# Kateridge/TransMF_AD

Hardware: AMD Instinct MI355X
Metric: volume-pairs/sec fwd+bwd(+Adam), 96^3 MRI+PET batch=8 per GPU (higher is better)
Workload: dtype f32

## Files before the change

include/tmf_hip.h:

```cpp
#ifndef TMF_HIP_H
#define TMF_HIP_H

#include <stddef.h>
#include <stdint.h>

#ifdef __cplusplus
extern "C" {
#endif

#define TMF_OK              0
#define TMF_E_NULL         -1
#define TMF_E_SHAPE        -2
#define TMF_E_ALIGN        -3
#define TMF_E_WORKSPACE    -4
#define TMF_E_ARG          -5

#define TMF_DW_TAPMAJOR  0
#define TMF_DW_REFERENCE 1

#define TMF_POOL_NONE 0
#define TMF_POOL_MAX2 1
#define TMF_POOL_AVG2 2

int         tmf_version(void);
const char* tmf_last_error_string(void);
int         tmf_set_option(const char* name, int value);

int  tmf_conv3d_fwd(const float* x, const float* w, float* z, float* stat_partial,
                    int B, int D, int H, int W, int cin, int cout, int ksize, void* stream);
int  tmf_conv3d_stat_blocks(int B, int D, int H, int W, int cin, int cout, int ksize);
const char* tmf_conv3d_fwd_kernel_name(int B, int D, int H, int W, int cin, int cout, int ksize);
const char* tmf_conv3d_wgrad_kernel_name(int B, int D, int H, int W, int cin, int cout, int ksize);
int  tmf_conv3d_fwd_affine(const float* x, const float* w, const float* scale, const float* shift, float* y,
                           int B, int D, int H, int W, int cin, int cout, int ksize, int pool, float slope, void* stream);

size_t tmf_conv3d_wgrad_workspace_bytes(int B, int D, int H, int W, int cin, int cout, int ksize);
int    tmf_conv3d_wgrad(const float* x, const float* dz, float* dw, void* workspace, size_t workspace_bytes,
                        int B, int D, int H, int W, int cin, int cout, int ksize, int dw_layout, void* stream);

int  tmf_conv3d_fwd_bf16(const float* x, const void* w_bf16, float* z, float* stat_partial,
                         int B, int D, int H, int W, int cin, int cout, void* stream);
int  tmf_conv3d_bf16_stat_blocks(int B, int D, int H, int W);
size_t tmf_conv3d_wgrad_bf16_workspace_bytes(int B, int D, int H, int W, int cin, int cout);
int    tmf_conv3d_wgrad_bf16(const float* x, const float* dz, float* dw, void* workspace, size_t workspace_bytes,
                             int B, int D, int H, int W, int cin, int cout, void* stream);
int    tmf_conv3d_fwd_bf16_t(const void* x, const void* w_bf16, void* z, float* stat_partial,
                             int B, int D, int H, int W, int cin, int cout, int io, void* stream);
const char* tmf_conv3d_fwd_bf16_kernel_name(int B, int D, int H, int W, int cin, int cout, int io);
const char* tmf_conv3d_wgrad_bf16_kernel_name(int B, int D, int H, int W, int cin, int cout, int io);
int    tmf_conv3d_wgrad_bf16_plan(int B, int D, int H, int W, int cin, int cout, int io, int* nsplit, int* tiles_per_split);
int    tmf_conv3d_wgrad_bf16_t(const void* x, const void* dz, float* dw, void* workspace, size_t workspace_bytes,
                               int B, int D, int H, int W, int cin, int cout, int io, int dw_layout, void* stream);
int  tmf_conv3d_fwd_split(const float* x, const void* w3_bf16, float* z, float* stat_partial,
                          int B, int D, int H, int W, int cin, int cout, void* stream);
int  tmf_conv3d_split_stat_blocks(int B, int D, int H, int W);
int    tmf_conv3d_fwd_wino(const float* x, const float* u, float* z, float* stat_partial,
                           int B, int D, int H, int W, int cin, int cout, void* stream);
int    tmf_conv3d_wino_ok(int cin, int cout);
int    tmf_conv3d_fwd_wino_affine(const float* x, const float* u, const float* scale, const float* shift, float* y,
                                  int B, int D, int H, int W, int cin, int cout, int pool, float slope, void* stream);
int    tmf_conv3d_wino_stat_blocks(int B, int D, int H, int W);
int    tmf_conv3d_wino_bricks(int B, int D, int H, int W);
int    tmf_conv3d_wino_bricks2(int B, int D, int H, int W, int cin, int cout);
int    tmf_conv3d_wino_grid(int B, int D, int H, int W, int cin, int cout);
int    tmf_xcd_slot(int block, int grid);
const char* tmf_conv3d_wino_kernel_name(int B, int D, int H, int W, int stats);
const char* tmf_conv3d_wgrad_wino_kernel_name(int B, int D, int H, int W, int cin, int cout);
long   tmf_conv3d_wgrad_wino_tiles(int B, int D, int H, int W, int cin, int cout);
const char* tmf_conv3d_wino_kernel_name2(int B, int D, int H, int W, int cin, int cout, int stats);
size_t tmf_conv3d_wino_weight_bytes(int cin, int cout);
int    tmf_wino_x_mode(void);
int    tmf_conv_wino_mode(void);
int    tmf_wino_p_mode(void);
int    tmf_conv3d_wgrad_wino_ok(int cin, int cout);
size_t tmf_conv3d_wgrad_wino_workspace_bytes(int B, int D, int H, int W, int cin, int cout);
int    tmf_conv3d_wgrad_wino(const float* x, const float* dz, float* dw, void* workspace, size_t workspace_bytes,
                             int B, int D, int H, int W, int cin, int cout, int dw_layout, void* stream);

int    tmf_conv3d_c1_fwd(const float* x, const float* w, float* z, float* stat_partial,
                         int B, int D, int H, int W, int cout, void* stream);
int    tmf_conv3d_c1_stat_blocks(int B, int D, int H, int W, int cout);
size_t tmf_conv3d_c1_wgrad_workspace_bytes(int B, int D, int H, int W, int cout);
int    tmf_conv3d_c1_wgrad(const float* x, const float* dz, float* dw, void* workspace, size_t workspace_bytes,
                           int B, int D, int H, int W, int cout, int dw_layout, void* stream);

int    tmf_c1_blocks(int B, int D, int H, int W, int C);
int    tmf_c1_stats(const float* x, const float* w, float* stat_partial, int B, int D, int H, int W, int C, void* stream);
size_t tmf_c1_gram_bytes(int B, int D, int H, int W, int C);
size_t tmf_c1_gram_bytes_bf16(int B, int D, int H, int W, int C);
int    tmf_c1_stats_g(const float* x, const float* w, float* stat_partial, void* gram, size_t gram_bytes,
                      int B, int D, int H, int W, int C, void* stream);
size_t tmf_c1_bwd_fused_workspace_bytes(int B, int D, int H, int W, int C);
int    tmf_c1_bwd_fused(const float* x, const float* w, const float* scale, const float* shift, const float* mean,
                        const float* invstd, const float* dpool, const void* gram, float* dw, float* dgamma, float* dbeta,
                        void* workspace, size_t workspace_bytes, int B, int D, int H, int W, int C, float slope,
                        int dw_layout, void* stream);
int    tmf_c1_stats_g_bf16(const float* x, const float* w, float* stat_partial, void* gram, size_t gram_bytes,
                           int B, int D, int H, int W, int C, void* stream);
int    tmf_c1_bwd_fused_bf16(const float* x, const float* w, const float* scale, const float* shift, const float* mean,
                             const float* invstd, const void* dpool, const void* gram, float* dw, float* dgamma, float* dbeta,
                             void* workspace, size_t workspace_bytes, int B, int D, int H, int W, int C, float slope,
                             int pooled_bf16, int dw_layout, void* stream);
int    tmf_c1_bn_pool_fwd(const float* x, const float* w, const float* scale, const float* shift, float* pooled,
                          int B, int D, int H, int W, int C, float slope, void* stream);
int    tmf_c1_bn_pool_fwd_route(const float* x, const float* w, const float* scale, const float* shift, float* pooled,
                                float* z_sel, unsigned char* arg, int B, int D, int H, int W, int C, float slope, void* stream);
int    tmf_c1_bwd_fused_route(const float* x, const float* w, const float* scale, const float* shift, const float* mean,
                              const float* invstd, const float* dpool, const float* z_sel, const unsigned char* arg,
                              const void* gram, float* dw, float* dgamma, float* dbeta, void* workspace, size_t workspace_bytes,
                              int B, int D, int H, int W, int C, float slope, int dw_layout, void* stream);
int    tmf_c1_bwd_fused_coef(const float* x, const float* w, const float* scale, const float* shift, const float* mean,
                             const float* invstd, const float* dpool, const float* z_sel, const unsigned char* arg,
                             const void* gram, float* dw, float* dgamma, float* dbeta, float* coef, void* workspace,
                             size_t workspace_bytes, int B, int D, int H, int W, int C, float slope, int dw_layout, void* stream);
int    tmf_c1_bwd_reduce(const float* x, const float* w, const float* scale, const float* shift,
                         const float* mean, const float* invstd, const float* dpool, float* partial,
                         int B, int D, int H, int W, int C, float slope, void* stream);
size_t tmf_c1_bwd_wgrad_workspace_bytes(int B, int D, int H, int W, int C);
int    tmf_c1_bwd_wgrad(const float* x, const float* w, const float* scale, const float* shift,
                        const float* mean, const float* invstd, const float* coef, const float* dpool,
                        float* dw, void* workspace, size_t workspace_bytes,
                        int B, int D, int H, int W, int C, float slope, int dw_layout, void* stream);
size_t tmf_c1_bwd_dgrad_workspace_bytes(int B, int D, int H, int W, int C);
int    tmf_c1_bwd_dgrad(const float* x, const float* w, const float* scale, const float* shift, const float* mean,
                        const float* invstd, const float* coef, const float* dpool, float* dx,
                        void* workspace, size_t workspace_bytes, int B, int D, int H, int W, int C, float slope, void* stream);
int    tmf_c1_stats_bf16(const float* x, const float* w, float* stat_partial, int B, int D, int H, int W, int C, void* stream);
int    tmf_c1_bn_pool_fwd_bf16(const float* x, const float* w, const float* scale, const float* shift, void* pooled,
                               int B, int D, int H, int W, int C, float slope, int pooled_bf16, void* stream);
int    tmf_c1_bwd_reduce_bf16(const float* x, const float* w, const float* scale, const float* shift,
                              const float* mean, const float* invstd, const void* dpool, float* partial,
                              int B, int D, int H, int W, int C, float slope, int pooled_bf16, void* stream);
int    tmf_c1_bwd_wgrad_bf16(const float* x, const float* w, const float* scale, const float* shift,
                             const float* mean, const float* invstd, const float* coef, const void* dpool,
                             float* dw, void* workspace, size_t workspace_bytes,
                             int B, int D, int H, int W, int C, float slope, int pooled_bf16, int dw_layout, void* stream);


int tmf_bn_finalize(const float* stat_partial, int nblk, int C, double count,
                    const float* gamma, const float* beta, const float* conv_bias,
                    float* running_mean, float* running_var, float momentum, float eps,
                    float* mean, float* invstd, float* scale, float* shift, void* stream);

int tmf_bn_eval_coeffs(const float* gamma, const float* beta, const float* conv_bias,
                       const float* running_mean, const float* running_var, float eps, int C,
                       float* scale, float* shift, void* stream);

int tmf_bn_act_pool_fwd(const float* z, const float* scale, const float* shift, float* out,
                        int B, int D, int H, int W, int C, int pool, float slope, void* stream);

int tmf_bn_act_pool_bwd_blocks(int B, int D, int H, int W, int C, int pool);
int tmf_bn_act_pool_bwd_reduce(const float* z, const float* dout, const float* scale, const float* shift,
                               const float* mean, const float* invstd, float* partial,
                               int B, int D, int H, int W, int C, int pool, float slope, void* stream);
int tmf_bn_bwd_finalize(const float* partial, int nblk, int C, double count,
                        float* dgamma, float* dbeta, float* coef, void* stream);
int tmf_bn_act_pool_bwd_apply(const float* z, const float* dout, const float* scale, const float* shift,
                              const float* mean, const float* invstd, const float* coef, float* dz,
                              int B, int D, int H, int W, int C, int pool, float slope, void* stream);

int tmf_bn_act_pool_fwd_t(const void* z, const float* scale, const float* shift, void* out,
                          int B, int D, int H, int W, int C, int pool, float slope, int io, void* stream);
int tmf_bn_act_pool_bwd_reduce_t(const void* z, const void* dout, const float* scale, const float* shift,
                                 const float* mean, const float* invstd, float* partial,
                                 int B, int D, int H, int W, int C, int pool, float slope, int io, void* stream);
int tmf_bn_act_pool_bwd_apply_t(const void* z, const void* dout, const float* scale, const float* shift,
                                const float* mean, const float* invstd, const float* coef, void* dz,
                                int B, int D, int H, int W, int C, int pool, float slope, int io, void* stream);

int tmf_bn_act_pool_fwd_route(const float* z, const float* scale, const float* shift, float* out, float* z_sel,
                              int B, int D, int H, int W, int C, float slope, void* stream);
int tmf_bn_act_pool_bwd_reduce_route(const float* z_sel, const float* dout, const float* scale, const float* shift,
                                     const float* mean, const float* invstd, float* partial,
                                     int B, int D, int H, int W, int C, float slope, void* stream);

int tmf_colsum_finalize(const float* partial, int nblk, int ncol, float* out, void* stream);

int tmf_xattn_fwd(const float* q, const float* k, const float* v, float* out, float* lse,
                  int B, int heads, int N, int M, int dh, int q_stride, int kv_stride, float scale,
                  void* stream);
int tmf_xattn_bwd(const float* q, const float* k, const float* v, const float* out, const float* lse,
                  const float* dout, float* dq, float* dk, float* dv,
                  int B, int heads, int N, int M, int dh, int q_stride, int kv_stride, int dkv_stride,
                  float scale, void* stream);
int tmf_xattn_fwd_cat(const float* q, const float* k1, const float* v1, const float* k2, const float* v2, float* out,
                      float* lse, int B, int heads, int N, int M1, int M2, int dh, int q_stride, int kv_stride, float scale,
                      void* stream);
int tmf_xattn_bwd_cat(const float* q, const float* k1, const float* v1, const float* k2, const float* v2, const float* out,
                      const float* lse, const float* dout, float* dq, float* dk1, float* dv1, float* dk2, float* dv2,
                      int B, int heads, int N, int M1, int M2, int dh, int q_stride, int kv_stride, int dkv_stride,
                      float scale, void* stream);
int tmf_xattn_probs(const float* q, const float* k1, const float* k2, const float* lse,
                    float* probs, float* recv, int B, int heads, int N, int M1, int M2, int dh,
                    int q_stride, int kv_stride, float scale, void* stream);

int tmf_layernorm_fwd(const float* x, const float* gamma, const float* beta, const float* residual, float* y,
                      float* mean, float* rstd, int rows, int dim, float eps, void* stream);
int tmf_layernorm_bwd_blocks(int rows, int dim);
int tmf_layernorm_bwd(const float* x, const float* gamma, const float* mean, const float* rstd,
                      const float* dy, float* dx, float* partial, int rows, int dim, void* stream);
int tmf_layernorm_bwd_masked(const float* x, const float* gamma, const float* mean, const float* rstd,
                             const float* dy, float* dx, float* partial, int rows, int dim,
                             const float* mask, float* dx_masked, void* stream);
int tmf_mask_mul(const float* x, const float* mask, float* y, long n, void* stream);

int tmf_tok_row_blocks(int R);
int tmf_tok_linear_fwd(const float* x, const float* w, const float* bias, const float* residual, float* y,
                       int R, int K, int Nout, const float* ln_gamma, const float* ln_beta, float eps,
                       float* ln_mean, float* ln_rstd, float* ln_out, float* gelu_pre, void* stream);
int tmf_tok_linear_bwd_input(const float* dy, const float* w, float* dx, int R, int Nout, int K,
                             const float* gelu_pre, const float* ln_x, const float* ln_mean, const float* ln_rstd,
                             const float* ln_gamma, const float* add1, const float* add2, float* ln_partial,
                             float* bias_partial, int partial_stride, void* stream);
int tmf_tok_linear_fwd_masked(const float* x, const float* w, const float* bias, const float* residual, float* y,
                              int R, int K, int Nout, const float* ln_gamma, const float* ln_beta, float eps,
                              float* ln_mean, float* ln_rstd, float* ln_out, float* gelu_pre, const float* mask, void* stream);
int tmf_tok_linear_bwd_input_masked(const float* dy, const float* w, float* dx, int R, int Nout, int K,
                                    const float* gelu_pre, const float* ln_x, const float* ln_mean, const float* ln_rstd,
                                    const float* ln_gamma, const float* add1, const float* add2, float* ln_partial,
                                    float* bias_partial, int partial_stride, const float* mask, float* dx_masked,
                                    void* stream);

int tmf_pack_conv_weights(const float* w, float* w_fwd, float* w_dgrad, int cout, int cin, int taps, void* stream);
int tmf_pack_conv_weights_bf16(const float* w, void* w_fwd_bf16, void* w_dgrad_bf16, int cout, int cin, int taps, void* stream);
int tmf_pack_conv_weights_split3(const float* w, void* w3_fwd, void* w3_dgrad, int cout, int cin, int taps, void* stream);
int tmf_pack_conv_weights_wino(const float* w, float* u_fwd, float* u_dgrad, int cout, int cin, void* stream);
int tmf_pack_conv_weights_wino_multi(int n, const float* const* w, float* const* u_fwd, float* const* u_dgrad,
                                     const int* cout, const int* cin, void* stream);

int tmf_layout_ncdhw_to_ndhwc(const float* src, float* dst, int B, int C, long voxels, void* stream);
int tmf_layout_ndhwc_to_ncdhw(const float* src, float* dst, int B, int C, long voxels, void* stream);

size_t tmf_tok_wgrad_multi_workspace_bytes(int nprob, const int* N, const int* K);
int    tmf_tok_wgrad_multi(int nprob, const float* const* dy, const float* const* x, float* const* dw,
                           const int* R, const int* N, const int* K, void* workspace, size_t workspace_bytes, void* stream);

int tmf_token_pool_fwd(const float* mri, const float* pet, float* cls, int32_t* argmax,
                       int B, int N, int dim, void* stream);
int tmf_token_pool_bwd(const float* dcls, const int32_t* argmax, float* dmri, float* dpet,
                       int B, int N, int dim, void* stream);

size_t tmf_scale_intensity_workspace_bytes(int B);
int    tmf_rotate_x(const float* src, float* dst, const float* cos_sin, const unsigned char* do_rot,
                    int B, int D, int H, int W, void* stream);
int    tmf_zoom_area(const float* src, float* dst, const int* out_size, const unsigned char* do_zoom,
                     int B, int D, int H, int W, void* stream);
int    tmf_volume_minmax(const float* vol, float* minmax, void* workspace, size_t workspace_bytes, int B, long voxels,
                         void* stream);
int    tmf_scale_flip(const float* src, float* dst, const float* minmax, const unsigned char* flip_d,
                      int B, int D, int H, int W, void* stream);

typedef struct tmf_augment_decision {
    int32_t index;
    int32_t flip;
    int32_t do_rot;
    float   cos_a, sin_a;
    int32_t od, oh, ow;
} tmf_augment_decision;
int    tmf_batch_augment(const float* store_mri, const float* store_pet, const int64_t* labels,
                         const tmf_augment_decision* decisions, float* out_mri, float* out_pet, int64_t* out_label,
                         int N, int B, int D, int H, int W, void* stream);

#define TMF_SNET_BLOCKS 7
#define TMF_PREC_FP32 0
#define TMF_PREC_BF16 1
#define TMF_PREC_FP32X 2
#define TMF_SNET_ALONE 1
#define TMF_SNET_ALGO          0x100
#define TMF_SNET_ALGO_WINO(m)  (((m) & 3) << 9)
#define TMF_SNET_ALGO_WINO_P   0x800
#define TMF_SNET_ALGO_WINO_X   0x1000
#define TMF_SNET_ALGO_C1_GRAM  0x2000
#define TMF_SNET_ALGO_C1_GRAM_BF16 0x4000
#define TMF_SNET_ALGO_C1_SPLIT 0x8000
#define TMF_SNET_ALGO_POOL_REC_C1 0x10000
#define TMF_SNET_ALGO_POOL_REC_BN 0x20000
int  tmf_snet_algo_flags(void);
int  tmf_c1_split_mode(void);
#define TMF_CONV_DIRECT 0
#define TMF_CONV_WINO   1
#define TMF_CONV_BF16   2
#define TMF_CONV_SPLIT  3
int  tmf_conv_block_algo(int precision, int cin, int cout, int ksize);
typedef struct tmf_snet_desc {
    int   B, D, H, W;
    int   dim;
    int   precision;
    int   storage_bf16;
    float momentum[TMF_SNET_BLOCKS];
    float eps[TMF_SNET_BLOCKS];
    float slope[TMF_SNET_BLOCKS];
    int   flags;
} tmf_snet_desc;
typedef struct tmf_snet_params {
    const float* weight[TMF_SNET_BLOCKS];
    const float* bias[TMF_SNET_BLOCKS];
    const float* gamma[TMF_SNET_BLOCKS];
    const float* beta[TMF_SNET_BLOCKS];
    float*       running_mean[TMF_SNET_BLOCKS];
    float*       running_var[TMF_SNET_BLOCKS];
} tmf_snet_params;
#define TMF_SNET_DEEP_FROM 3
typedef struct tmf_snet_grads {
    float* dweight[TMF_SNET_BLOCKS];
    float* dbias[TMF_SNET_BLOCKS];
    float* dgamma[TMF_SNET_BLOCKS];
    float* dbeta[TMF_SNET_BLOCKS];
    void*  deep_event;
} tmf_snet_grads;
size_t tmf_snet_saved_bytes(const tmf_snet_desc* d);
size_t tmf_snet_bwd_scratch_bytes(const tmf_snet_desc* d);
int    tmf_snet_train_fwd(const tmf_snet_desc* d, const float* vol, const tmf_snet_params* params,
                          void* saved, size_t saved_bytes, float* out, void* stream);
int    tmf_snet_train_bwd(const tmf_snet_desc* d, const float* vol, const void* saved, size_t saved_bytes,
                          const float* dout, const tmf_snet_grads* grads, void* scratch, size_t scratch_bytes, void* stream);
int    tmf_snet_train_bwd_input(const tmf_snet_desc* d, const float* vol, const void* saved, size_t saved_bytes,
                                const float* dout, const tmf_snet_grads* grads, void* scratch, size_t scratch_bytes, void* stream,
                                float* dvol);
size_t tmf_snet_eval_workspace_bytes(const tmf_snet_desc* d);
int    tmf_snet_eval_fwd(const tmf_snet_desc* d, const float* vol, const tmf_snet_params* params,
                         void* workspace, size_t workspace_bytes, float* out, void* stream);

#define TMF_FUSION_MAX_DEPTH 16
#define TMF_FUSION_PER_OP 1
typedef struct tmf_fusion_desc { int B, N, dim, heads, dim_head, mlp, depth, flags; } tmf_fusion_desc;
typedef struct tmf_xformer_params {
    const float *ln1_g, *ln1_b;
    const float *wq, *wkv, *wo, *bo;
    const float *ln2_g, *ln2_b;
    const float *w1, *b1, *w2, *b2;
    const float *lnf_g, *lnf_b;
    float eps1, eps2, epsf;
    const float *mask_o, *mask_g, *mask_f;
} tmf_xformer_params;
typedef struct tmf_xformer_grads {
    float *small, *lnf, *dwq, *dwkv, *dwo, *dw1, *dw2;
} tmf_xformer_grads;
void   tmf_debug_xf_trace(void* fwd, void* bwd_q, void* bwd_kv);
size_t tmf_fusion_saved_bytes(const tmf_fusion_desc* d);
int    tmf_fusion_uses_fused(const tmf_fusion_desc* d);
int    tmf_fusion_takes_masks(const tmf_fusion_desc* d);
size_t tmf_fusion_bwd_scratch_bytes(const tmf_fusion_desc* d);
int    tmf_fusion_train_fwd(const tmf_fusion_desc* d, const float* mri_tok, const float* pet_tok,
                            const tmf_xformer_params* inst, void* saved, size_t saved_bytes, float* cls, void* stream);
int    tmf_fusion_train_bwd(const tmf_fusion_desc* d, const float* mri_tok, const float* pet_tok,
                            const tmf_xformer_params* inst, const void* saved, size_t saved_bytes, const float* dcls,
                            const tmf_xformer_grads* grads, float* dmri_tok, float* dpet_tok,
                            void* scratch, size_t scratch_bytes, void* stream);
size_t tmf_fusion_infer_workspace_bytes(const tmf_fusion_desc* d);
int    tmf_fusion_infer_fwd(const tmf_fusion_desc* d, const float* mri_tok, const float* pet_tok,
                            const tmf_xformer_params* inst, void* workspace, size_t workspace_bytes,
                            float* cls, void* stream);
size_t tmf_fusion_attn_maps_workspace_bytes(const tmf_fusion_desc* d);
int    tmf_fusion_attn_maps(const tmf_fusion_desc* d, const float* mri_tok, const float* pet_tok,
                            const tmf_xformer_params* inst, void* workspace, size_t workspace_bytes,
                            float* cls, float* probs, float* recv, void* stream);

typedef struct tmf_heads_desc { int B, N, dim, H1, H2, HD, NC, training; float momentum[3], eps[3]; } tmf_heads_desc;
typedef struct tmf_heads_params {
    const float *fc0_w, *fc0_b, *bn1_g, *bn1_b, *fc4_w, *fc4_b, *bn5_g, *bn5_b, *fc8_w, *fc8_b;
    const float *d0_w, *d0_b, *dbn_g, *dbn_b, *d3_w, *d3_b;
    float *bn1_rm, *bn1_rv, *bn5_rm, *bn5_rv, *dbn_rm, *dbn_rv;
} tmf_heads_params;
typedef struct tmf_heads_grads {
    float *fc0_w, *fc0_b, *bn1_g, *bn1_b, *fc4_w, *fc4_b, *bn5_g, *bn5_b, *fc8_w, *fc8_b, *d0_w, *d0_b, *dbn_g, *dbn_b, *d3_w, *d3_b;
} tmf_heads_grads;
size_t tmf_heads_saved_bytes(const tmf_heads_desc* d);
size_t tmf_heads_bwd_scratch_bytes(const tmf_heads_desc* d);
int    tmf_heads_fwd(const tmf_heads_desc* d, const float* cls, const float* mri_tok, const float* pet_tok,
                     const float* mask1, const float* mask2, const tmf_heads_params* params, float* logits,
                     float* d_mri_logits, float* d_pet_logits, void* saved, size_t saved_bytes, void* stream);
int    tmf_heads_bwd(const tmf_heads_desc* d, const float* cls, const float* mask1, const float* mask2,
                     const tmf_heads_params* params, const void* saved, size_t saved_bytes, const float* d_logits,
                     const float* d_d_mri_logits, const float* d_d_pet_logits, const tmf_heads_grads* grads,
                     float* d_cls, float* d_mri_tok, float* d_pet_tok, float revgrad_alpha,
                     void* scratch, size_t scratch_bytes, void* stream);

#define TMF_MASK_SEGMENTS 20
int    tmf_dropout_keep_masks(int nseg, float* const* out, const long* numel, const float* keep,
                              unsigned long long seed, unsigned long long offset, void* stream);

typedef struct tmf_heads_cnn_desc { int B, N, dim, M, H, HD, NC, training; float momentum, eps; } tmf_heads_cnn_desc;
typedef struct tmf_heads_cnn_params {
    const float *fc0_w, *fc0_b, *fc2_w, *fc2_b;
    const float *d0_w, *d0_b, *dbn_g, *dbn_b;
    float *dbn_rm, *dbn_rv;
    const float *d3_w, *d3_b;
} tmf_heads_cnn_params;
typedef struct tmf_heads_cnn_grads { float *fc0_w, *fc0_b, *fc2_w, *fc2_b, *d0_w, *d0_b, *dbn_g, *dbn_b, *d3_w, *d3_b; } tmf_heads_cnn_grads;
size_t tmf_heads_cnn_saved_bytes(const tmf_heads_cnn_desc* d);
size_t tmf_heads_cnn_bwd_scratch_bytes(const tmf_heads_cnn_desc* d);
int    tmf_heads_cnn_fwd(const tmf_heads_cnn_desc* d, const float* mri_tok, const float* pet_tok,
                         const tmf_heads_cnn_params* params, float* logits, float* d_mri_logits, float* d_pet_logits,
                         void* saved, size_t saved_bytes, void* stream);
// ... 94 lines not shown
```

transmf_ad_amd/csrc/conv1_fused.hip:

```cpp
#include <type_traits>
#include "conv1_z.h"

namespace {
using namespace c1z;

enum { MODE_STATS = 0, MODE_FWD = 1, MODE_REDUCE = 2, MODE_WGRAD = 3, MODE_RD = 4 };
#ifndef TMF_C1X_LAZY
#define TMF_C1X_LAZY 0x12
#endif

struct Args {
    const float* x;
    const float* w;
    const float* scale;
    const float* shift;
    const float* mean;
    const float* invstd;
    const float* coef;
    const void* dpool;
    void* pooled;
    float* zsel;
    unsigned char* parg;
    float* partial;
    float* partial2;
// ... 400 lines not shown
}
extern "C" int tmf_c1_stats(const float* x, const float* w, float* stat_partial,
                            int B, int D, int H, int W, int C, void* stream) {
    return c1_stats(false, x, w, stat_partial, B, D, H, W, C, stream);
}
extern "C" int tmf_c1_stats_bf16(const float* x, const float* w, float* stat_partial,
                                 int B, int D, int H, int W, int C, void* stream) {
    return c1_stats(true, x, w, stat_partial, B, D, H, W, C, stream);
}

static int c1_bn_pool_fwd(bool bf16, bool p16, const float* x, const float* w, const float* scale, const float* shift,
                          void* pooled, int B, int D, int H, int W, int C, float slope, void* stream,
                          float* z_sel = nullptr, unsigned char* arg = nullptr) {
    TMF_REQUIRE_PTR(x); TMF_REQUIRE_PTR(w); TMF_REQUIRE_PTR(scale); TMF_REQUIRE_PTR(shift); TMF_REQUIRE_PTR(pooled);
    int rc = check("tmf_c1_bn_pool_fwd", B, D, H, W, C);
    if (rc) return rc;
    const Plan p = make_plan(B, D, H, W, C, tmf_opt(TMF_OPT_C1_FWD_MULT) * SLAB_BLOCKS);
    Args a = base_args(x, w, D, H, W, C, p, slope);
    a.scale = scale; a.shift = shift; a.pooled = pooled; a.zsel = z_sel; a.parg = arg;
    TMF_REQUIRE(bf16 || !p16, TMF_E_ARG, "tmf_c1_bn_pool_fwd: bf16 tensors only with the bf16 kernels");
    if (z_sel != nullptr) {
        if (c1_split_mode()) hipLaunchKernelGGL((conv1_fused_kernel<MODE_FWD, false, false, true, true>), dim3(p.nblk, p.nby), dim3(256), 0, (hipStream_t)stream, a);
        else                 hipLaunchKernelGGL((conv1_fused_kernel<MODE_FWD, false, false, false, true>), dim3(p.nblk, p.nby), dim3(256), 0, (hipStream_t)stream, a);
        return tmf_launch_result("tmf_c1_bn_pool_fwd_route");
    }
    if (bf16 && p16) hipLaunchKernelGGL((conv1_fused_kernel<MODE_FWD, true, true>), dim3(p.nblk, p.nby), dim3(256), 0, (hipStream_t)stream, a);
    else if (bf16)   hipLaunchKernelGGL((conv1_fused_kernel<MODE_FWD, true>), dim3(p.nblk, p.nby), dim3(256), 0, (hipStream_t)stream, a);
    else if (c1_split_mode()) hipLaunchKernelGGL((conv1_fused_kernel<MODE_FWD, false, false, true>), dim3(p.nblk, p.nby), dim3(256), 0, (hipStream_t)stream, a);
    else             hipLaunchKernelGGL((conv1_fused_kernel<MODE_FWD, false>), dim3(p.nblk, p.nby), dim3(256), 0, (hipStream_t)stream, a);
    return tmf_launch_result("tmf_c1_bn_pool_fwd");
}
extern "C" int tmf_c1_bn_pool_fwd(const float* x, const float* w, const float* scale, const float* shift,
                                  float* pooled, int B, int D, int H, int W, int C, float slope, void* stream) {
    return c1_bn_pool_fwd(false, false, x, w, scale, shift, pooled, B, D, H, W, C, slope, stream);
}
extern "C" int tmf_c1_bn_pool_fwd_route(const float* x, const float* w, const float* scale, const float* shift, float* pooled,
                                        float* z_sel, unsigned char* arg, int B, int D, int H, int W, int C, float slope, void* stream) {
    TMF_REQUIRE_PTR(z_sel); TMF_REQUIRE_PTR(arg);
    return c1_bn_pool_fwd(false, false, x, w, scale, shift, pooled, B, D, H, W, C, slope, stream, z_sel, arg);
}
extern "C" int tmf_c1_bn_pool_fwd_bf16(const float* x, const float* w, const float* scale, const float* shift,
                                       void* pooled, int B, int D, int H, int W, int C, float slope, int pooled_bf16,
                                       void* stream) {
    return c1_bn_pool_fwd(true, pooled_bf16 != 0, x, w, scale, shift, pooled, B, D, H, W, C, slope, stream);
}

static int c1_bwd_reduce(bool bf16, bool p16, const float* x, const float* w, const float* scale, const float* shift,
                         const float* mean, const float* invstd, const void* dpool, float* partial,
                         int B, int D, int H, int W, int C, float slope, void* stream) {
    TMF_REQUIRE_PTR(x); TMF_REQUIRE_PTR(w); TMF_REQUIRE_PTR(scale); TMF_REQUIRE_PTR(shift);
    TMF_REQUIRE_PTR(mean); TMF_REQUIRE_PTR(invstd); TMF_REQUIRE_PTR(dpool); TMF_REQUIRE_PTR(partial);
    int rc = check("tmf_c1_bwd_reduce", B, D, H, W, C);
    if (rc) return rc;
    const Plan p = make_plan(B, D, H, W, C, SLAB_BLOCKS);
    Args a = base_args(x, w, D, H, W, C, p, slope);
    a.scale = scale; a.shift = shift; a.mean = mean; a.invstd = invstd; a.dpool = dpool; a.partial = partial;
    TMF_REQUIRE(bf16 || !p16, TMF_E_ARG, "tmf_c1_bwd_reduce: bf16 tensors only with the bf16 kernels");
    if (bf16 && p16) hipLaunchKernelGGL((conv1_fused_kernel<MODE_REDUCE, true, true>), dim3(p.nblk, p.nby), dim3(256), 0, (hipStream_t)stream, a);
    else if (bf16)   hipLaunchKernelGGL((conv1_fused_kernel<MODE_REDUCE, true>), dim3(p.nblk, p.nby), dim3(256), 0, (hipStream_t)stream, a);
    else if (c1_split_mode()) hipLaunchKernelGGL((conv1_fused_kernel<MODE_REDUCE, false, false, true>), dim3(p.nblk, p.nby), dim3(256), 0, (hipStream_t)stream, a);
    else             hipLaunchKernelGGL((conv1_fused_kernel<MODE_REDUCE, false>), dim3(p.nblk, p.nby), dim3(256), 0, (hipStream_t)stream, a);
    return tmf_launch_result("tmf_c1_bwd_reduce");
}
extern "C" int tmf_c1_bwd_reduce(const float* x, const float* w, const float* scale, const float* shift,
                                 const float* mean, const float* invstd, const float* dpool, float* partial,
                                 int B, int D, int H, int W, int C, float slope, void* stream) {
    return c1_bwd_reduce(false, false, x, w, scale, shift, mean, invstd, dpool, partial, B, D, H, W, C, slope, stream);
}
extern "C" int tmf_c1_bwd_reduce_bf16(const float* x, const float* w, const float* scale, const float* shift,
                                      const float* mean, const float* invstd, const void* dpool, float* partial,
                                      int B, int D, int H, int W, int C, float slope, int pooled_bf16, void* stream) {
    return c1_bwd_reduce(true, pooled_bf16 != 0, x, w, scale, shift, mean, invstd, dpool, partial, B, D, H, W, C, slope, stream);
}

extern "C" size_t tmf_c1_bwd_wgrad_workspace_bytes(int B, int D, int H, int W, int C) {
    if (B <= 0 || D <= 0 || H <= 0 || W <= 0 || C <= 0) return 0;
    const Plan p = make_plan(B, D, H, W, C, SLAB_BLOCKS);
    return (size_t)(p.nblk + tmf_reduce_groups(p.nblk)) * 27 * C * 4;
}

static int c1_bwd_wgrad(bool bf16, bool p16, const float* x, const float* w, const float* scale, const float* shift,
                        const float* mean, const float* invstd, const float* coef, const void* dpool,
                        float* dw, void* workspace, size_t workspace_bytes,
                        int B, int D, int H, int W, int C, float slope, int dw_layout, void* stream) {
    TMF_REQUIRE(dw_layout == TMF_DW_TAPMAJOR || dw_layout == TMF_DW_REFERENCE, TMF_E_ARG,
                "tmf_c1_bwd_wgrad: unknown dw_layout %d", dw_layout);
    TMF_REQUIRE_PTR(x); TMF_REQUIRE_PTR(w); TMF_REQUIRE_PTR(scale); TMF_REQUIRE_PTR(shift); TMF_REQUIRE_PTR(mean);
    TMF_REQUIRE_PTR(invstd); TMF_REQUIRE_PTR(coef); TMF_REQUIRE_PTR(dpool); TMF_REQUIRE_PTR(dw); TMF_REQUIRE_PTR(workspace);
    int rc = check("tmf_c1_bwd_wgrad", B, D, H, W, C);
    if (rc) return rc;
    const size_t need = tmf_c1_bwd_wgrad_workspace_bytes(B, D, H, W, C);
    TMF_REQUIRE(workspace_bytes >= need, TMF_E_WORKSPACE, "tmf_c1_bwd_wgrad: workspace %zu B < required %zu B",
                workspace_bytes, need);
    const Plan p = make_plan(B, D, H, W, C, SLAB_BLOCKS);
    Args a = base_args(x, w, D, H, W, C, p, slope);
    a.scale = scale; a.shift = shift; a.mean = mean; a.invstd = invstd; a.coef = coef; a.dpool = dpool;
    a.partial = (float*)workspace;
    hipStream_t s = (hipStream_t)stream;
    TMF_REQUIRE(bf16 || !p16, TMF_E_ARG, "tmf_c1_bwd_wgrad: bf16 tensors only with the bf16 kernels");
    if (bf16 && p16) hipLaunchKernelGGL((conv1_fused_kernel<MODE_WGRAD, true, true>), dim3(p.nblk, p.nby), dim3(256), 0, s, a);
    else if (bf16)   hipLaunchKernelGGL((conv1_fused_kernel<MODE_WGRAD, true>), dim3(p.nblk, p.nby), dim3(256), 0, s, a);
    else if (c1_split_mode()) hipLaunchKernelGGL((conv1_fused_kernel<MODE_WGRAD, false, false, true>), dim3(p.nblk, p.nby), dim3(256), 0, s, a);
    else             hipLaunchKernelGGL((conv1_fused_kernel<MODE_WGRAD, false>), dim3(p.nblk, p.nby), dim3(256), 0, s, a);
    if ((rc = tmf_launch_result("tmf_c1_bwd_wgrad"))) return rc;
    const long n = 27L * C;
    return tmf_reduce_slabs((const float*)workspace, p.nblk, n, (float*)workspace + (size_t)p.nblk * n, dw, s,
                            "tmf_c1_bwd_wgrad(reduce)", dw_layout == TMF_DW_REFERENCE ? 1 : 0, C);
}

extern "C" int tmf_c1_bwd_wgrad(const float* x, const float* w, const float* scale, const float* shift,
                                const float* mean, const float* invstd, const float* coef, const float* dpool,
                                float* dw, void* workspace, size_t workspace_bytes,
                                int B, int D, int H, int W, int C, float slope, int dw_layout, void* stream) {
    return c1_bwd_wgrad(false, false, x, w, scale, shift, mean, invstd, coef, dpool, dw, workspace, workspace_bytes, B, D, H, W,
                        C, slope, dw_layout, stream);
}
extern "C" int tmf_c1_bwd_wgrad_bf16(const float* x, const float* w, const float* scale, const float* shift,
                                     const float* mean, const float* invstd, const float* coef, const void* dpool,
                                     float* dw, void* workspace, size_t workspace_bytes,
                                     int B, int D, int H, int W, int C, float slope, int pooled_bf16, int dw_layout,
                                     void* stream) {
    return c1_bwd_wgrad(true, pooled_bf16 != 0, x, w, scale, shift, mean, invstd, coef, dpool, dw, workspace, workspace_bytes,
                        B, D, H, W, C, slope, dw_layout, stream);
}

int tmf_c1_bwd_fused_finish(const float* part, int nblk, const float* dred, const float* w, const void* gram, const float* scale,
                            const float* mean, const float* invstd, double count, float* dgamma, float* dbeta, float* dw, int C,
                            int dw_ref, int round16, void* stream, float* coef);
extern "C" size_t tmf_c1_bwd_fused_workspace_bytes(int B, int D, int H, int W, int C) {
    if (B <= 0 || D <= 0 || H <= 0 || W <= 0 || C <= 0) return 0;
    const Plan p = make_plan(B, D, H, W, C, SLAB_BLOCKS);
    return ((size_t)p.nblk * 2 * C + (size_t)(p.nblk + tmf_reduce_groups(p.nblk) + 1) * 27 * C) * 4;
}
static int c1_bwd_fused(bool bf16, bool p16, const float* x, const float* w, const float* scale, const float* shift, const float* mean,
                        const float* invstd, const void* dpool, const void* gram, float* dw, float* dgamma, float* dbeta,
                        void* workspace, size_t workspace_bytes, int B, int D, int H, int W, int C, float slope,
                        int dw_layout, void* stream, const float* z_sel = nullptr, const unsigned char* arg = nullptr,
                        float* coef = nullptr) {
    TMF_REQUIRE(dw_layout == TMF_DW_TAPMAJOR || dw_layout == TMF_DW_REFERENCE, TMF_E_ARG, "tmf_c1_bwd_fused: unknown dw_layout %d", dw_layout);
    TMF_REQUIRE_PTR(x); TMF_REQUIRE_PTR(w); TMF_REQUIRE_PTR(scale); TMF_REQUIRE_PTR(shift); TMF_REQUIRE_PTR(mean); TMF_REQUIRE_PTR(invstd);
    TMF_REQUIRE_PTR(dpool); TMF_REQUIRE_PTR(gram); TMF_REQUIRE_PTR(dw); TMF_REQUIRE_PTR(workspace);
    int rc = check("tmf_c1_bwd_fused", B, D, H, W, C);
    if (rc) return rc;
    TMF_REQUIRE(C <= 64, TMF_E_SHAPE, "tmf_c1_bwd_fused: C = %d > 64", C);
    const size_t need = tmf_c1_bwd_fused_workspace_bytes(B, D, H, W, C);
    TMF_REQUIRE(workspace_bytes >= need, TMF_E_WORKSPACE, "tmf_c1_bwd_fused: workspace %zu B < required %zu B", workspace_bytes, need);
    const Plan p = make_plan(B, D, H, W, C, SLAB_BLOCKS);
    Args a = base_args(x, w, D, H, W, C, p, slope);
    a.scale = scale; a.shift = shift; a.mean = mean; a.invstd = invstd; a.dpool = dpool;
    float* part = (float*)workspace;
    float* slabs = part + (size_t)p.nblk * 2 * C;
    const long n = 27L * C;
    float* scratch = slabs + (size_t)p.nblk * n;
    float* dred = scratch + (size_t)tmf_reduce_groups(p.nblk) * n;
    a.partial = part; a.partial2 = slabs;
    a.zsel = const_cast<float*>(z_sel); a.parg = const_cast<unsigned char*>(arg);
    hipStream_t s = (hipStream_t)stream;
    TMF_REQUIRE(bf16 || !p16, TMF_E_ARG, "tmf_c1_bwd_fused: bf16 tensors only with the bf16 kernels");
    if (z_sel != nullptr) hipLaunchKernelGGL((conv1_fused_kernel<MODE_RD, false, false, false, true>), dim3(p.nblk, p.nby), dim3(256), 0, s, a);
    else if (bf16 && p16) hipLaunchKernelGGL((conv1_fused_kernel<MODE_RD, true, true>), dim3(p.nblk, p.nby), dim3(256), 0, s, a);
    else if (bf16)   hipLaunchKernelGGL((conv1_fused_kernel<MODE_RD, true>), dim3(p.nblk, p.nby), dim3(256), 0, s, a);
    else if (c1_split_mode()) hipLaunchKernelGGL((conv1_fused_kernel<MODE_RD, false, false, true>), dim3(p.nblk, p.nby), dim3(256), 0, s, a);
    else             hipLaunchKernelGGL((conv1_fused_kernel<MODE_RD, false>), dim3(p.nblk, p.nby), dim3(256), 0, s, a);
    if ((rc = tmf_launch_result("tmf_c1_bwd_fused"))) return rc;
    if ((rc = tmf_reduce_slabs(slabs, p.nblk, n, scratch, dred, s, "tmf_c1_bwd_fused(reduce)"))) return rc;
    return tmf_c1_bwd_fused_finish(part, p.nblk, dred, w, gram, scale, mean, invstd, (double)B * D * H * W, dgamma, dbeta, dw, C,
                                   dw_layout == TMF_DW_REFERENCE ? 1 : 0, bf16 ? 1 : 0, stream, coef);
}
extern "C" int tmf_c1_bwd_fused(const float* x, const float* w, const float* scale, const float* shift, const float* mean,
                                const float* invstd, const float* dpool, const void* gram, float* dw, float* dgamma, float* dbeta,
                                void* workspace, size_t workspace_bytes, int B, int D, int H, int W, int C, float slope,
                                int dw_layout, void* stream) {
    return c1_bwd_fused(false, false, x, w, scale, shift, mean, invstd, dpool, gram, dw, dgamma, dbeta, workspace, workspace_bytes,
                        B, D, H, W, C, slope, dw_layout, stream);
}
extern "C" int tmf_c1_bwd_fused_route(const float* x, const float* w, const float* scale, const float* shift, const float* mean,
                                      const float* invstd, const float* dpool, const float* z_sel, const unsigned char* arg,
                                      const void* gram, float* dw, float* dgamma, float* dbeta, void* workspace, size_t workspace_bytes,
                                      int B, int D, int H, int W, int C, float slope, int dw_layout, void* stream) {
    TMF_REQUIRE_PTR(z_sel); TMF_REQUIRE_PTR(arg);
    return c1_bwd_fused(false, false, x, w, scale, shift, mean, invstd, dpool, gram, dw, dgamma, dbeta, workspace, workspace_bytes,
                        B, D, H, W, C, slope, dw_layout, stream, z_sel, arg);
}
extern "C" int tmf_c1_bwd_fused_coef(const float* x, const float* w, const float* scale, const float* shift, const float* mean,
                                     const float* invstd, const float* dpool, const float* z_sel, const unsigned char* arg,
                                     const void* gram, float* dw, float* dgamma, float* dbeta, float* coef, void* workspace,
                                     size_t workspace_bytes, int B, int D, int H, int W, int C, float slope, int dw_layout, void* stream) {
    TMF_REQUIRE_PTR(coef);
    TMF_REQUIRE((z_sel == nullptr) == (arg == nullptr), TMF_E_NULL, "tmf_c1_bwd_fused_coef: z_sel and arg go together");
    return c1_bwd_fused(false, false, x, w, scale, shift, mean, invstd, dpool, gram, dw, dgamma, dbeta, workspace, workspace_bytes,
// ... 10 lines not shown
```

transmf_ad_amd/csrc/conv3d_mfma.hip:

```cpp
#include <type_traits>
#include "tmf_device.h"

#ifndef TMF_CONV_ACC
#define TMF_CONV_ACC 1
#endif
#ifndef TMF_CONV_BUF
#define TMF_CONV_BUF 1
#endif

namespace {

template <int KS_, int CINC_, int MT_, int NT_, int WM_, int WN_, int TD_, int TH_, int TW_, int TPS_>
struct FwdCfg {
    static constexpr int KS = KS_, CINC = CINC_, MT = MT_, NT = NT_, WM = WM_, WN = WN_;
    static constexpr int TD = TD_, TH = TH_, TW = TW_, TPS = TPS_;
    static constexpr int PAD = KS / 2;
    static constexpr int HD = TD + 2 * PAD, HH = TH + 2 * PAD, HW = TW + 2 * PAD;
    static constexpr int NHALO = HD * HH * HW;
    static constexpr int CP = CINC + 4;
    static constexpr int NPOS = TD * TH * TW;
    static constexpr int NB = 32 * NT * WN;
    static constexpr int NTAPS = KS * KS * KS;
    static constexpr int NSTAGES = NTAPS / TPS;
    static constexpr int BSTAGE = TPS * CINC * NB;
// ... 1402 lines not shown
}

extern "C" const char* tmf_conv3d_fwd_kernel_name(int B, int D, int H, int W, int cin, int cout, int ksize) {
    if (B <= 0 || D <= 0 || H <= 0 || W <= 0 || cin <= 0 || cout <= 0 || (ksize != 1 && ksize != 3)) return "?";
    const FwdPlan p = plan_fwd(B, D, H, W, cin, cout, ksize);
    return ksize == 3 ? fwd_kernel_name<3>(p) : fwd_kernel_name<1>(p);
}

extern "C" const char* tmf_conv3d_wgrad_kernel_name(int B, int D, int H, int W, int cin, int cout, int ksize) {
    if (B <= 0 || D <= 0 || H <= 0 || W <= 0 || cin <= 0 || cout <= 0) return "?";
    if (ksize != 3) return "conv1x1_wgrad_kernel";
    const WgPlan p = plan_wgrad(B, D, H, W, cin, cout);
    const bool vec = (cin % 4 == 0) && (cout % 4 == 0);
    const bool w8 = vec && conv_waves() >= 8;
    static thread_local char buf[64];
    const int edge = p.small ? 4 : 8;
    const int nt = (w8 && p.pack) ? 1 : p.nt;
    snprintf(buf, sizeof buf, "WgCfg<%d, 4, %d, %d, %d, %d>", nt, edge, edge, w8 ? 8 : 4, (w8 && p.pack) ? 16 : 32);
    return buf;
}

extern "C" int tmf_conv3d_stat_blocks(int B, int D, int H, int W, int cin, int cout, int ksize) {
    return tmf_conv3d_stat_blocks_mode(B, D, H, W, cin, cout, ksize, 0);
}
int tmf_conv3d_stat_blocks_mode(int B, int D, int H, int W, int cin, int cout, int ksize, int rt_min) {
    if (B <= 0 || D <= 0 || H <= 0 || W <= 0 || cin <= 0 || cout <= 0) return 0;
    return plan_fwd(B, D, H, W, cin, cout, ksize, true, rt_min).ntiles;
}

extern "C" int tmf_conv3d_fwd(const float* x, const float* w, float* z, float* stat_partial,
                              int B, int D, int H, int W, int cin, int cout, int ksize, void* stream) {
    return tmf_conv3d_fwd_mode(x, w, z, stat_partial, B, D, H, W, cin, cout, ksize, 0, stream);
}
int tmf_conv3d_fwd_mode(const float* x, const float* w, float* z, float* stat_partial,
                        int B, int D, int H, int W, int cin, int cout, int ksize, int rt_min, void* stream) {
    TMF_REQUIRE_PTR(x); TMF_REQUIRE_PTR(w); TMF_REQUIRE_PTR(z);
    TMF_REQUIRE(B > 0 && D > 0 && H > 0 && W > 0 && cin > 0 && cout > 0, TMF_E_SHAPE,
                "tmf_conv3d_fwd: non-positive dimension (B=%d D=%d H=%d W=%d cin=%d cout=%d)", B, D, H, W, cin, cout);
    TMF_REQUIRE(ksize == 1 || ksize == 3, TMF_E_ARG, "tmf_conv3d_fwd: ksize must be 1 or 3, got %d", ksize);
    TMF_REQUIRE((long)D * H * W * (cin > cout ? cin : cout) < (1L << 29), TMF_E_SHAPE,
                "tmf_conv3d_fwd: one sample exceeds 2^29 elements (32-bit byte offsets inside a sample)");
    TMF_REQUIRE((long)ksize * ksize * ksize * cin * cout < (1L << 29), TMF_E_SHAPE, "tmf_conv3d_fwd: weight tensor exceeds 2^29 elements");
    TMF_REQUIRE_ALIGNED(x); TMF_REQUIRE_ALIGNED(w); TMF_REQUIRE_ALIGNED(z);
    const FwdPlan p = plan_fwd(B, D, H, W, cin, cout, ksize, true, rt_min);
    hipStream_t s = (hipStream_t)stream;
    return ksize == 3 ? launch_fwd<3>(p, x, w, z, stat_partial, D, H, W, cin, cout, s)
                      : launch_fwd<1>(p, x, w, z, stat_partial, D, H, W, cin, cout, s);
}

extern "C" int tmf_conv3d_fwd_affine(const float* x, const float* w, const float* scale, const float* shift, float* y,
                                     int B, int D, int H, int W, int cin, int cout, int ksize, int pool, float slope,
                                     void* stream) {
    TMF_REQUIRE_PTR(x); TMF_REQUIRE_PTR(w); TMF_REQUIRE_PTR(scale); TMF_REQUIRE_PTR(shift); TMF_REQUIRE_PTR(y);
    TMF_REQUIRE(B > 0 && D > 0 && H > 0 && W > 0 && cin > 0 && cout > 0, TMF_E_SHAPE,
                "tmf_conv3d_fwd_affine: non-positive dimension (B=%d D=%d H=%d W=%d cin=%d cout=%d)", B, D, H, W, cin, cout);
    TMF_REQUIRE(ksize == 1 || ksize == 3, TMF_E_ARG, "tmf_conv3d_fwd_affine: ksize must be 1 or 3, got %d", ksize);
    TMF_REQUIRE(pool == TMF_POOL_NONE || pool == TMF_POOL_MAX2 || pool == TMF_POOL_AVG2, TMF_E_ARG,
                "tmf_conv3d_fwd_affine: unknown pool mode %d", pool);
    TMF_REQUIRE((long)D * H * W * (cin > cout ? cin : cout) < (1L << 29), TMF_E_SHAPE,
                "tmf_conv3d_fwd_affine: one sample exceeds 2^29 elements (32-bit byte offsets inside a sample)");
    TMF_REQUIRE((long)ksize * ksize * ksize * cin * cout < (1L << 29), TMF_E_SHAPE, "tmf_conv3d_fwd_affine: weight tensor exceeds 2^29 elements");
    TMF_REQUIRE_ALIGNED(x); TMF_REQUIRE_ALIGNED(w); TMF_REQUIRE_ALIGNED(y);
    if (pool != TMF_POOL_NONE && (D / 2 == 0 || H / 2 == 0 || W / 2 == 0)) return TMF_OK;
    const FwdPlan p = plan_fwd(B, D, H, W, cin, cout, ksize, false);
    const Affine aff = {scale, shift, slope, pool};
    hipStream_t s = (hipStream_t)stream;
    return ksize == 3 ? launch_fwd<3>(p, x, w, y, nullptr, D, H, W, cin, cout, s, &aff)
                      : launch_fwd<1>(p, x, w, y, nullptr, D, H, W, cin, cout, s, &aff);
}

extern "C" size_t tmf_conv3d_wgrad_workspace_bytes(int B, int D, int H, int W, int cin, int cout, int ksize) {
    if (B <= 0 || D <= 0 || H <= 0 || W <= 0 || cin <= 0 || cout <= 0) return 0;
    if (ksize == 3) {
        const WgPlan p = plan_wgrad(B, D, H, W, cin, cout);
        return (size_t)(p.nsplit + tmf_reduce_groups(p.nsplit)) * 27 * cin * cout * 4;
    }
    const Wg1Plan p = plan_wgrad1((long)B * D * H * W, cin, cout);
    return (size_t)(p.nsplit + tmf_reduce_groups(p.nsplit)) * cin * cout * 4;
}

extern "C" int tmf_conv3d_wgrad(const float* x, const float* dz, float* dw, void* workspace,
                                size_t workspace_bytes, int B, int D, int H, int W, int cin, int cout,
                                int ksize, int dw_layout, void* stream) {
    TMF_REQUIRE(dw_layout == TMF_DW_TAPMAJOR || dw_layout == TMF_DW_REFERENCE, TMF_E_ARG,
                "tmf_conv3d_wgrad: unknown dw_layout %d", dw_layout);
    TMF_REQUIRE_PTR(x); TMF_REQUIRE_PTR(dz); TMF_REQUIRE_PTR(dw); TMF_REQUIRE_PTR(workspace);
    TMF_REQUIRE(B > 0 && D > 0 && H > 0 && W > 0 && cin > 0 && cout > 0, TMF_E_SHAPE,
                "tmf_conv3d_wgrad: non-positive dimension");
    TMF_REQUIRE(ksize == 1 || ksize == 3, TMF_E_ARG, "tmf_conv3d_wgrad: ksize must be 1 or 3, got %d", ksize);
    TMF_REQUIRE((long)(D > 6 ? D : 6) * H * W * (cin > cout ? cin : cout) < (1L << 29), TMF_E_SHAPE,
                "tmf_conv3d_wgrad: one sample exceeds 2^29 elements (32-bit byte offsets inside a sample)");
    TMF_REQUIRE_ALIGNED(x); TMF_REQUIRE_ALIGNED(dz); TMF_REQUIRE_ALIGNED(dw); TMF_REQUIRE_ALIGNED(workspace);
    const size_t need = tmf_conv3d_wgrad_workspace_bytes(B, D, H, W, cin, cout, ksize);
    TMF_REQUIRE(workspace_bytes >= need, TMF_E_WORKSPACE, "tmf_conv3d_wgrad: workspace %zu B < required %zu B",
                workspace_bytes, need);
    hipStream_t s = (hipStream_t)stream;
    float* partial = (float*)workspace;
    const bool vec = (cin % 4 == 0) && (cout % 4 == 0);
    int rc;
    long nelem;
    int nsplit;
    if (ksize == 3) {
        const WgPlan p = plan_wgrad(B, D, H, W, cin, cout);
        dim3 grid(p.nsplit, p.gy, p.gz);
#define TMF_WG_LAUNCH(CFG, V)                                                                       \
    do {                                                                                            \
        auto k = conv3d_wgrad_kernel<CFG, V>;                                                       \
        if ((rc = tmf_allow_lds(k, CFG::LDS_BYTES, "tmf_conv3d_wgrad"))) return rc;                 \
        hipLaunchKernelGGL(k, grid, dim3(CFG::NTHR), CFG::LDS_BYTES, s, x, dz, partial, D, H, W, cin, cout,   \
                           p.tilesD, p.tilesH, p.tilesW, p.ntiles, p.tps, tmf_opt(TMF_OPT_DEBUG));  \
    } while (0)
        using L1 = WgCfg<1, 4, 8, 8>;
        using L2 = WgCfg<2, 4, 8, 8>;
        using S1 = WgCfg<1, 4, 4, 4>;
        using S2 = WgCfg<2, 4, 4, 4>;
        using L1w8 = WgCfg<1, 4, 8, 8, 8>;
        using L2w8 = WgCfg<2, 4, 8, 8, 8>;
        using S1w8 = WgCfg<1, 4, 4, 4, 8>;
        using S2w8 = WgCfg<2, 4, 4, 4, 8>;
        using L1w8p = WgCfg<1, 4, 8, 8, 8, 16>;
        using S1w8p = WgCfg<1, 4, 4, 4, 8, 16>;
        const bool w8 = vec && conv_waves() >= 8;
        if (w8 && p.pack) {
            if (!p.small) TMF_WG_LAUNCH(L1w8p, true);
            else          TMF_WG_LAUNCH(S1w8p, true);
        } else if (w8) {
            if (!p.small && p.nt == 1) TMF_WG_LAUNCH(L1w8, true);
            else if (!p.small)         TMF_WG_LAUNCH(L2w8, true);
            else if (p.nt == 1)        TMF_WG_LAUNCH(S1w8, true);
            else                       TMF_WG_LAUNCH(S2w8, true);
        }
        else if (!p.small && p.nt == 1) { if (vec) TMF_WG_LAUNCH(L1, true); else TMF_WG_LAUNCH(L1, false); }
        else if (!p.small)         { if (vec) TMF_WG_LAUNCH(L2, true); else TMF_WG_LAUNCH(L2, false); }
        else if (p.nt == 1)        { if (vec) TMF_WG_LAUNCH(S1, true); else TMF_WG_LAUNCH(S1, false); }
        else                       { if (vec) TMF_WG_LAUNCH(S2, true); else TMF_WG_LAUNCH(S2, false); }
#undef TMF_WG_LAUNCH
        if ((rc = tmf_launch_result("tmf_conv3d_wgrad"))) return rc;
        nelem = 27L * cin * cout;
        nsplit = p.nsplit;
    } else {
        const long npos = (long)B * D * H * W;
        const Wg1Plan p = plan_wgrad1(npos, cin, cout);
        dim3 grid(p.nblk, p.gy, p.gz), block(256);
        if (p.nt == 1) hipLaunchKernelGGL(conv1x1_wgrad_kernel<1>, grid, block, 0, s, x, dz, partial, npos, cin, cout, p.spb);
        else           hipLaunchKernelGGL(conv1x1_wgrad_kernel<2>, grid, block, 0, s, x, dz, partial, npos, cin, cout, p.spb);
        if ((rc = tmf_launch_result("tmf_conv3d_wgrad(1x1)"))) return rc;
        nelem = (long)cin * cout;
        nsplit = p.nsplit;
    }
    return tmf_reduce_slabs(partial, nsplit, nelem, partial + (size_t)nsplit * nelem, dw, s, "tmf_conv3d_wgrad(reduce)",
                            dw_layout == TMF_DW_REFERENCE ? cin : 0, cout);
}

extern "C" int tmf_conv3d_c1_stat_blocks(int B, int D, int H, int W, int cout) {
    if (B <= 0 || D <= 0 || H <= 0 || W <= 0 || cout <= 0) return 0;
    return plan_c1(B, D, H, W, cout).ntiles;
}

extern "C" int tmf_conv3d_c1_fwd(const float* x, const float* w, float* z, float* stat_partial,
                                 int B, int D, int H, int W, int cout, void* stream) {
    TMF_REQUIRE_PTR(x); TMF_REQUIRE_PTR(w); TMF_REQUIRE_PTR(z);
    TMF_REQUIRE(B > 0 && D > 0 && H > 0 && W > 0 && cout > 0, TMF_E_SHAPE, "tmf_conv3d_c1_fwd: non-positive dimension");
    TMF_REQUIRE((long)D * H * W * cout < (1L << 31), TMF_E_SHAPE, "tmf_conv3d_c1_fwd: one sample exceeds 2^31 elements");
    const C1Plan p = plan_c1(B, D, H, W, cout);
    hipLaunchKernelGGL(conv3d_c1_fwd_kernel, dim3(p.ntiles, p.nby), dim3(256), 0, (hipStream_t)stream,
                       x, w, z, stat_partial, D, H, W, cout, p.tilesD, p.tilesH, p.tilesW, p.ntiles);
    return tmf_launch_result("tmf_conv3d_c1_fwd");
}

extern "C" size_t tmf_conv3d_c1_wgrad_workspace_bytes(int B, int D, int H, int W, int cout) {
    if (B <= 0 || D <= 0 || H <= 0 || W <= 0 || cout <= 0) return 0;
    const C1Plan p = plan_c1(B, D, H, W, cout);
    return (size_t)(p.nblk * 4 + tmf_reduce_groups(p.nblk * 4)) * 27 * cout * 4;
}

extern "C" int tmf_conv3d_c1_wgrad(const float* x, const float* dz, float* dw, void* workspace,
                                   size_t workspace_bytes, int B, int D, int H, int W, int cout, int dw_layout,
                                   void* stream) {
    TMF_REQUIRE(dw_layout == TMF_DW_TAPMAJOR || dw_layout == TMF_DW_REFERENCE, TMF_E_ARG,
                "tmf_conv3d_c1_wgrad: unknown dw_layout %d", dw_layout);
    TMF_REQUIRE_PTR(x); TMF_REQUIRE_PTR(dz); TMF_REQUIRE_PTR(dw); TMF_REQUIRE_PTR(workspace);
    TMF_REQUIRE(B > 0 && D > 0 && H > 0 && W > 0 && cout > 0, TMF_E_SHAPE, "tmf_conv3d_c1_wgrad: non-positive dimension");
    const size_t need = tmf_conv3d_c1_wgrad_workspace_bytes(B, D, H, W, cout);
    TMF_REQUIRE(workspace_bytes >= need, TMF_E_WORKSPACE, "tmf_conv3d_c1_wgrad: workspace %zu B < required %zu B",
                workspace_bytes, need);
    const C1Plan p = plan_c1(B, D, H, W, cout);
    hipStream_t s = (hipStream_t)stream;
    float* partial = (float*)workspace;
    const size_t lds = (size_t)C1_TD * C1_TH * C1_TW * 32 * 4;
    hipLaunchKernelGGL(conv3d_c1_wgrad_kernel, dim3(p.nblk, p.nby), dim3(256), lds, s, x, dz, partial,
                       D, H, W, cout, p.tilesD, p.tilesH, p.tilesW, p.ntiles, p.tps);
    int rc;
    if ((rc = tmf_launch_result("tmf_conv3d_c1_wgrad"))) return rc;
    const long nelem = 27L * cout;
    return tmf_reduce_slabs(partial, p.nblk * 4, nelem, partial + (size_t)p.nblk * 4 * nelem, dw, s,
                            "tmf_conv3d_c1_wgrad(reduce)", dw_layout == TMF_DW_REFERENCE ? 1 : 0, cout);
}
```

transmf_ad_amd/csrc/conv3d_wino.hip:

```cpp
#include <type_traits>
#include "tmf_device.h"

namespace {

constexpr int TD = 4, TH = 8, TW = 8;
constexpr int CK = 8;
constexpr int NTHR = 512;
constexpr int GROUPS = 768, SLOTS = 2 * GROUPS;
constexpr int RAW_BYTES = SLOTS * 16;
constexpr int NDMA = SLOTS / NTHR;
constexpr int B_OFF = 2 * RAW_BYTES;
constexpr int B_BYTES = 8 * 8 * 64 * 16;
constexpr int EX_FLOATS = 8 * 8 * 2 * 64 * 4;
constexpr int RED_OFF = EX_FLOATS;
constexpr int LDS_FLOATS = RED_OFF + 8 * 32 * 2;
constexpr size_t LDS_BYTES = (size_t)LDS_FLOATS * 4;
static_assert(B_OFF + B_BYTES <= EX_FLOATS * 4, "LDS carving");

__device__ __forceinline__ constexpr int ogd(int dd) { return (dd & 1) * 384 + (dd >> 1) * 32; }
__device__ __forceinline__ constexpr int ogh(int i) { return (i & 1) * 192 + (i >> 1) * 6; }
__device__ __forceinline__ constexpr int ogw(int k) { return (k & 1) * 96 + (k >> 1); }

#ifdef TMF_WINO_TRACE
__device__ long long g_wino_blocks[8192 * 4];
// ... 1628 lines not shown
    if (B <= 0 || D <= 0 || H <= 0 || W <= 0) return "conv3d_wino_wgrad_p_kernel<0>";
    return plan_wino_wgrad(B, D, H, W, cin, cout).geom ? "conv3d_wino_wgrad_p_kernel<1>" : "conv3d_wino_wgrad_p_kernel<0>";
}

extern "C" size_t tmf_conv3d_wino_weight_bytes(int cin, int cout) { return (size_t)64 * cin * cout * (4 + 6); }

extern "C" int tmf_pack_conv_weights_wino(const float* w, float* u_fwd, float* u_dgrad, int cout, int cin, void* stream) {
    TMF_REQUIRE_PTR(w);
    TMF_REQUIRE(u_fwd != nullptr || u_dgrad != nullptr, TMF_E_NULL, "tmf_pack_conv_weights_wino: both outputs are NULL");
    TMF_REQUIRE(cout > 0 && cin > 0, TMF_E_SHAPE, "tmf_pack_conv_weights_wino: cout=%d cin=%d", cout, cin);
    TMF_REQUIRE(u_fwd == nullptr || tmf_conv3d_wino_ok(cin, cout), TMF_E_SHAPE,
                "tmf_pack_conv_weights_wino: forward form needs cin %% 8 == 0 and cout %% 32 == 0 (cin=%d cout=%d)", cin, cout);
    TMF_REQUIRE(u_dgrad == nullptr || tmf_conv3d_wino_ok(cout, cin), TMF_E_SHAPE,
                "tmf_pack_conv_weights_wino: data-gradient form needs cout %% 8 == 0 and cin %% 32 == 0 (cin=%d cout=%d)", cin, cout);
    hipLaunchKernelGGL(wino_pack_kernel, dim3((unsigned)tmf_cdiv((long)cout * cin, 256L)), dim3(256), 0, (hipStream_t)stream,
                       w, u_fwd, u_dgrad, cout, cin);
    return tmf_launch_result("tmf_pack_conv_weights_wino");
}

extern "C" int tmf_pack_conv_weights_wino_multi(int n, const float* const* w, float* const* u_fwd, float* const* u_dgrad,
                                                const int* cout, const int* cin, void* stream) {
    TMF_REQUIRE(n > 0 && n <= 8, TMF_E_ARG, "tmf_pack_conv_weights_wino_multi: %d layers (1 .. 8)", n);
    TMF_REQUIRE_PTR(w); TMF_REQUIRE_PTR(u_fwd); TMF_REQUIRE_PTR(u_dgrad); TMF_REQUIRE_PTR(cout); TMF_REQUIRE_PTR(cin);
    WinoPackMulti a;
    long most = 0;
    for (int l = 0; l < n; ++l) {
        TMF_REQUIRE(w[l] != nullptr && (u_fwd[l] != nullptr || u_dgrad[l] != nullptr), TMF_E_NULL,
                    "tmf_pack_conv_weights_wino_multi: layer %d: weight or both outputs NULL", l);
        TMF_REQUIRE(cout[l] > 0 && cin[l] > 0 && (u_fwd[l] == nullptr || tmf_conv3d_wino_ok(cin[l], cout[l])) &&
                    (u_dgrad[l] == nullptr || tmf_conv3d_wino_ok(cout[l], cin[l])), TMF_E_SHAPE,
                    "tmf_pack_conv_weights_wino_multi: layer %d: cin=%d cout=%d", l, cin[l], cout[l]);
        a.w[l] = w[l]; a.fwd[l] = u_fwd[l]; a.dgrad[l] = u_dgrad[l]; a.cout[l] = cout[l]; a.cin[l] = cin[l];
        if ((long)cout[l] * cin[l] > most) most = (long)cout[l] * cin[l];
    }
    for (int l = n; l < 8; ++l) { a.w[l] = nullptr; a.fwd[l] = nullptr; a.dgrad[l] = nullptr; a.cout[l] = 0; a.cin[l] = 0; }
    hipLaunchKernelGGL(wino_pack_multi_kernel, dim3((unsigned)tmf_cdiv(most, 256L), n), dim3(256), 0, (hipStream_t)stream, a);
    return tmf_launch_result("tmf_pack_conv_weights_wino_multi");
}

extern "C" int tmf_conv3d_fwd_wino(const float* x, const float* u, float* z, float* stat_partial,
                                   int B, int D, int H, int W, int cin, int cout, void* stream) {
    TMF_REQUIRE_PTR(x); TMF_REQUIRE_PTR(u); TMF_REQUIRE_PTR(z);
    TMF_REQUIRE(B > 0 && D > 0 && H > 0 && W > 0, TMF_E_SHAPE, "tmf_conv3d_fwd_wino: non-positive dimension (B=%d D=%d H=%d W=%d)", B, D, H, W);
    TMF_REQUIRE(tmf_conv3d_wino_ok(cin, cout), TMF_E_SHAPE,
                "tmf_conv3d_fwd_wino: needs cin %% 8 == 0 and cout %% 32 == 0 (cin=%d cout=%d)", cin, cout);
    TMF_REQUIRE((long)D * H * W * (cin > cout ? cin : cout) < (1L << 29), TMF_E_SHAPE,
                "tmf_conv3d_fwd_wino: one sample exceeds 2^29 elements (32-bit byte offsets inside a sample)");
    TMF_REQUIRE((long)64 * cin * cout < (1L << 29), TMF_E_SHAPE, "tmf_conv3d_fwd_wino: weight tensor exceeds 2^29 elements");
    TMF_REQUIRE_ALIGNED(x); TMF_REQUIRE_ALIGNED(u); TMF_REQUIRE_ALIGNED(z);
    if (wino_p_mode()) {
        if (stat_partial != nullptr)
            return launch_wino_p<1>("tmf_conv3d_fwd_wino", x, u, z, stat_partial, B, D, H, W, cin, cout, nullptr, nullptr, 0.f, 0, (hipStream_t)stream);
        return launch_wino_p<0>("tmf_conv3d_fwd_wino", x, u, z, nullptr, B, D, H, W, cin, cout, nullptr, nullptr, 0.f, 0, (hipStream_t)stream);
    }
    const int tilesD = tmf_cdiv(D, TD), tilesH = tmf_cdiv(H, TH), tilesW = tmf_cdiv(W, TW);
    const int ntiles = B * tilesD * tilesH * tilesW;
    dim3 grid(ntiles, cout / 32), block(NTHR);
    int rc;
    if (stat_partial != nullptr) {
        auto k = conv3d_wino_kernel<1>;
        if ((rc = tmf_allow_lds(k, LDS_BYTES, "tmf_conv3d_fwd_wino"))) return rc;
        hipLaunchKernelGGL(k, grid, block, LDS_BYTES, (hipStream_t)stream, x, u, z, stat_partial, D, H, W, cin, cout,
                           tilesD, tilesH, tilesW, ntiles, (const float*)nullptr, (const float*)nullptr, 0.f, 0);
    } else {
        auto k = conv3d_wino_kernel<0>;
        if ((rc = tmf_allow_lds(k, LDS_BYTES, "tmf_conv3d_fwd_wino"))) return rc;
        hipLaunchKernelGGL(k, grid, block, LDS_BYTES, (hipStream_t)stream, x, u, z, stat_partial, D, H, W, cin, cout,
                           tilesD, tilesH, tilesW, ntiles, (const float*)nullptr, (const float*)nullptr, 0.f, 0);
    }
    return tmf_launch_result("tmf_conv3d_fwd_wino");
}

extern "C" int tmf_conv3d_wgrad_wino_ok(int cin, int cout) { return cin > 0 && cout > 0 && cin % 32 == 0 && cout % 32 == 0; }

extern "C" size_t tmf_conv3d_wgrad_wino_workspace_bytes(int B, int D, int H, int W, int cin, int cout) {
    if (B <= 0 || D <= 0 || H <= 0 || W <= 0 || !tmf_conv3d_wgrad_wino_ok(cin, cout)) return 0;
    const WinoWgPlan p = plan_wino_wgrad(B, D, H, W, cin, cout);
    if (wino_p_mode())
        return (size_t)(p.nsplit + tmf_reduce_groups(p.nsplit)) * 27 * cin * cout * 4;
    const size_t n = (size_t)p.nblk * 64 * 1024;
    return (size_t)(p.nsplit + tmf_reduce_groups(p.nsplit) + 1) * n * 4;
}

extern "C" int tmf_conv3d_wgrad_wino(const float* x, const float* dz, float* dw, void* workspace, size_t workspace_bytes,
                                     int B, int D, int H, int W, int cin, int cout, int dw_layout, void* stream) {
    TMF_REQUIRE(dw_layout == TMF_DW_TAPMAJOR || dw_layout == TMF_DW_REFERENCE, TMF_E_ARG,
                "tmf_conv3d_wgrad_wino: unknown dw_layout %d", dw_layout);
    TMF_REQUIRE_PTR(x); TMF_REQUIRE_PTR(dz); TMF_REQUIRE_PTR(dw); TMF_REQUIRE_PTR(workspace);
    TMF_REQUIRE(B > 0 && D > 0 && H > 0 && W > 0, TMF_E_SHAPE, "tmf_conv3d_wgrad_wino: non-positive dimension");
    TMF_REQUIRE(tmf_conv3d_wgrad_wino_ok(cin, cout), TMF_E_SHAPE,
                "tmf_conv3d_wgrad_wino: needs cin %% 32 == 0 and cout %% 32 == 0 (cin=%d cout=%d)", cin, cout);
    TMF_REQUIRE((long)(D + 2) * (H + 2) * (W + 2) * (cin > cout ? cin : cout) < (1L << 29), TMF_E_SHAPE,
                "tmf_conv3d_wgrad_wino: one sample exceeds 2^29 elements (32-bit byte offsets inside a sample)");
    TMF_REQUIRE_ALIGNED(x); TMF_REQUIRE_ALIGNED(dz); TMF_REQUIRE_ALIGNED(dw); TMF_REQUIRE_ALIGNED(workspace);
    const size_t need = tmf_conv3d_wgrad_wino_workspace_bytes(B, D, H, W, cin, cout);
    TMF_REQUIRE(workspace_bytes >= need, TMF_E_WORKSPACE, "tmf_conv3d_wgrad_wino: workspace %zu B < required %zu B", workspace_bytes, need);
    const WinoWgPlan p = plan_wino_wgrad(B, D, H, W, cin, cout);
    hipStream_t s = (hipStream_t)stream;
    float* partial = (float*)workspace;
    const long n = (long)p.nblk * 64 * 1024;
    int rc;
    if (wino_p_mode()) {
        auto k = p.geom ? conv3d_wino_wgrad_p_kernel<1> : conv3d_wino_wgrad_p_kernel<0>;
        const size_t lds = p.geom ? WGeomP<1>::LDS_BYTES : WGeomP<0>::LDS_BYTES;
        if ((rc = tmf_allow_lds(k, lds, "tmf_conv3d_wgrad_wino"))) return rc;
        hipLaunchKernelGGL(k, dim3(p.nsplit, p.nblk), dim3(WPN), lds, s, x, dz, partial, B, D, H, W, cin, cout,
                           p.tilesD, p.tilesH, p.tilesW, p.nbricks, p.per, p.ncob);
        if ((rc = tmf_launch_result("tmf_conv3d_wgrad_wino"))) return rc;
        const long nw = (long)27 * cin * cout;
        const bool ref = dw_layout == TMF_DW_REFERENCE;
        return tmf_reduce_slabs(partial, p.nsplit, nw, partial + (size_t)p.nsplit * nw, dw, s, "tmf_conv3d_wgrad_wino(reduce)",
                                ref ? cin : 0, ref ? cout : 0);
    }
    auto k = conv3d_wino_wgrad_kernel;
    if ((rc = tmf_allow_lds(k, WG_LDS_BYTES, "tmf_conv3d_wgrad_wino"))) return rc;
    hipLaunchKernelGGL(k, dim3(p.nsplit, p.nblk), dim3(NTHR), WG_LDS_BYTES, s, x, dz, partial, D, H, W, cin, cout,
                       p.tilesD, p.tilesH, p.tilesW, p.nbricks, p.per, p.ncob);
    if ((rc = tmf_launch_result("tmf_conv3d_wgrad_wino"))) return rc;
    float* scratch = partial + (size_t)p.nsplit * n;
    float* du = scratch + (size_t)tmf_reduce_groups(p.nsplit) * n;
    if ((rc = tmf_reduce_slabs(partial, p.nsplit, n, scratch, du, s, "tmf_conv3d_wgrad_wino(reduce)"))) return rc;
    hipLaunchKernelGGL(wino_wgrad_finish_kernel, dim3((unsigned)tmf_cdiv((long)cin * cout, 256L)), dim3(256), 0, s,
                       (const float*)du, dw, cin, cout, p.ncob, dw_layout == TMF_DW_REFERENCE ? 1 : 0);
    return tmf_launch_result("tmf_conv3d_wgrad_wino(finish)");
}

extern "C" int tmf_conv3d_fwd_wino_affine(const float* x, const float* u, const float* scale, const float* shift, float* y,
                                          int B, int D, int H, int W, int cin, int cout, int pool, float slope, void* stream) {
    TMF_REQUIRE_PTR(x); TMF_REQUIRE_PTR(u); TMF_REQUIRE_PTR(scale); TMF_REQUIRE_PTR(shift); TMF_REQUIRE_PTR(y);
    TMF_REQUIRE(B > 0 && D > 0 && H > 0 && W > 0, TMF_E_SHAPE, "tmf_conv3d_fwd_wino_affine: non-positive dimension");
    TMF_REQUIRE(tmf_conv3d_wino_ok(cin, cout), TMF_E_SHAPE,
                "tmf_conv3d_fwd_wino_affine: needs cin %% 8 == 0 and cout %% 32 == 0 (cin=%d cout=%d)", cin, cout);
    TMF_REQUIRE(pool == TMF_POOL_NONE || pool == TMF_POOL_MAX2, TMF_E_ARG, "tmf_conv3d_fwd_wino_affine: pool must be none or max, got %d", pool);
    TMF_REQUIRE((long)D * H * W * (cin > cout ? cin : cout) < (1L << 29), TMF_E_SHAPE,
                "tmf_conv3d_fwd_wino_affine: one sample exceeds 2^29 elements (32-bit byte offsets inside a sample)");
    TMF_REQUIRE((long)64 * cin * cout < (1L << 29), TMF_E_SHAPE, "tmf_conv3d_fwd_wino_affine: weight tensor exceeds 2^29 elements");
    TMF_REQUIRE_ALIGNED(x); TMF_REQUIRE_ALIGNED(u); TMF_REQUIRE_ALIGNED(y);
    if (pool != TMF_POOL_NONE && (D / 2 == 0 || H / 2 == 0 || W / 2 == 0)) return TMF_OK;
    if (wino_p_mode())
        return launch_wino_p<2>("tmf_conv3d_fwd_wino_affine", x, u, y, nullptr, B, D, H, W, cin, cout, scale, shift, slope, pool, (hipStream_t)stream);
    const int tilesD = tmf_cdiv(D, TD), tilesH = tmf_cdiv(H, TH), tilesW = tmf_cdiv(W, TW);
    const int ntiles = B * tilesD * tilesH * tilesW;
    auto k = conv3d_wino_kernel<2>;
    int rc;
    if ((rc = tmf_allow_lds(k, LDS_BYTES, "tmf_conv3d_fwd_wino_affine"))) return rc;
    hipLaunchKernelGGL(k, dim3(ntiles, cout / 32), dim3(NTHR), LDS_BYTES, (hipStream_t)stream, x, u, y, (float*)nullptr, D, H, W, cin, cout,
                       tilesD, tilesH, tilesW, ntiles, scale, shift, slope, pool);
    return tmf_launch_result("tmf_conv3d_fwd_wino_affine");
}
```

transmf_ad_amd/csrc/options.hip:

```cpp
#include "tmf_common.h"
#include <atomic>
#include <climits>

namespace {

constexpr int UNSET = INT_MIN;

int nonzero(int v) { return v != 0; }
int clamp02(int v) { return v <= 0 ? 0 : (v >= 2 ? 2 : 1); }
bool in02(int v) { return v >= 0 && v <= 2; }

struct Row {
    TmfOpt opt;
    const char* name;
    const char* env;
    int def;
    const char* accepts;
    bool (*ok)(int);
    int (*set)(int);
    int (*from_env)(int);
    int call[3];
};

constexpr Row kRows[] = {
    {TMF_OPT_CONV_WINO, "conv_wino", "TMF_CONV_WINO", 3, "0, 1, 2 or 3", [](int v) { return v >= 0 && v <= 3; }, nullptr,
     [](int v) { return v >= 0 && v <= 2 ? v : 3; }, {TMF_SNET_ALGO_WINO(1), TMF_SNET_ALGO_WINO(2), TMF_SNET_ALGO_WINO(3)}},
    {TMF_OPT_WINO_P, "wino_p", "TMF_WINO_P", 1, nullptr, nullptr, nonzero, nonzero, {TMF_SNET_ALGO_WINO_P}},
    {TMF_OPT_WINO_X, "wino_x", "TMF_WINO_X", 1, nullptr, nullptr, nonzero, nonzero, {TMF_SNET_ALGO_WINO_X}},
    {TMF_OPT_C1_GRAM, "c1_gram", "TMF_C1_GRAM", 1, nullptr, nullptr, clamp02, clamp02,
     {TMF_SNET_ALGO_C1_GRAM, TMF_SNET_ALGO_C1_GRAM | TMF_SNET_ALGO_C1_GRAM_BF16}},
    {TMF_OPT_C1_SPLIT, "c1_split", "TMF_C1_SPLIT", 1, nullptr, nullptr, nonzero, nonzero, {TMF_SNET_ALGO_C1_SPLIT}},
    {TMF_OPT_POOL_RECOMPUTE, "pool_recompute", "TMF_POOL_RECOMPUTE", 0, "0, 1, 2 or 3", [](int v) { return v >= 0 && v <= 3; }, nullptr,
     [](int v) { return v >= 0 && v <= 3 ? v : 0; },
     {TMF_SNET_ALGO_POOL_REC_C1 | TMF_SNET_ALGO_POOL_REC_BN, TMF_SNET_ALGO_POOL_REC_C1, TMF_SNET_ALGO_POOL_REC_BN}},
    {TMF_OPT_WINO_CUS, "wino_cus", "TMF_WINO_CUS", 0, ">= 0", [](int v) { return v >= 0; }, [](int v) { return v ? v : UNSET; },
     nullptr, {}},
    {TMF_OPT_CONV_RT, "conv_rt", "TMF_CONV_RT", 0, "0, 1 or 2", in02, nullptr, [](int v) { return v == 1 || v == 2 ? v : 0; }, {}},
    {TMF_OPT_CONV_WAVES, "conv_waves", "TMF_CONV_WAVES", 16, "2, 4, 8 or 16", [](int v) { return v == 2 || v == 4 || v == 8 || v == 16; },
     nullptr, [](int v) { return v == 2 || v == 4 || v == 8 ? v : 16; }, {}},
    {TMF_OPT_BF16_V2, "bf16_v2", "TMF_BF_V2", 1, "0, 1 or 2", in02, nullptr, [](int v) { return v == 0 || v == 2 ? v : 1; }, {}},
    {TMF_OPT_BF16_DMA, "bf16_dma", nullptr, 1, "0 or 1", [](int v) { return v == 0 || v == 1; }, nullptr, nullptr, {}},
    {TMF_OPT_WGRAD_TR, "wgrad_tr", nullptr, 1, "0, 1 or 2", in02, nullptr, nullptr, {}},
    {TMF_OPT_DEBUG, "debug", nullptr, 0, nullptr, nullptr, nullptr, nullptr, {}},
    {TMF_OPT_WINO_EVEN, nullptr, "TMF_WINO_EVEN", 1, nullptr, nullptr, nullptr, nonzero, {}},
    {TMF_OPT_WINOX_SWAP, nullptr, "TMF_WINOX_SWAP", 1, nullptr, nullptr, nullptr, nonzero, {}},
    {TMF_OPT_BF_NT2, nullptr, "TMF_BF_NT2", 1, nullptr, nullptr, nullptr, nonzero, {}},
    {TMF_OPT_CONV_AUTO, nullptr, "TMF_CONV_AUTO", 1, nullptr, nullptr, nullptr, nonzero, {}},
    {TMF_OPT_C1_BLOCKS, nullptr, "TMF_C1_BLOCKS", 1024, nullptr, nullptr, nullptr, [](int v) { return v < 64 ? 1024 : v; }, {}},
    {TMF_OPT_C1_FWD_MULT, nullptr, "TMF_C1_FWD_MULT", 4, nullptr, nullptr, nullptr, nullptr, {}},
};
constexpr bool rows_in_order() {
    for (int o = 0; o < TMF_OPT_COUNT; ++o)
        if (kRows[o].opt != o) return false;
    return sizeof kRows / sizeof kRows[0] == TMF_OPT_COUNT;
}
static_assert(rows_in_order(), "kRows: one row per TmfOpt, in the enum's order");

struct Values {
    int env[TMF_OPT_COUNT];
    std::atomic<int> set[TMF_OPT_COUNT];
    Values() {
        for (const Row& r : kRows) {
            const char* e = r.env ? getenv(r.env) : nullptr;
            env[r.opt] = e == nullptr ? r.def : (r.from_env ? r.from_env(atoi(e)) : atoi(e));
            set[r.opt].store(UNSET, std::memory_order_relaxed);
        }
    }
};
Values& values() {
    static Values v;
    return v;
}

thread_local int t_algo = 0;

}

TmfAlgoScope::TmfAlgoScope(int flags) : prev(t_algo) { if (flags & TMF_SNET_ALGO) t_algo = flags; }
TmfAlgoScope::~TmfAlgoScope() { t_algo = prev; }

int tmf_opt(TmfOpt o) {
    const Row& r = kRows[o];
    if (r.call[0]) {
        if (const int f = t_algo) {
            const int bits = f & (r.call[0] | r.call[1] | r.call[2]);
            for (int i = 0; i < 3; ++i)
                if (r.call[i] && bits == r.call[i]) return i + 1;
            return 0;
        }
    }
    Values& v = values();
    const int s = v.set[o].load(std::memory_order_relaxed);
    return s != UNSET ? s : v.env[o];
}

extern "C" int tmf_set_option(const char* name, int value) {
    TMF_REQUIRE_PTR(name);
    for (const Row& r : kRows) {
        if (r.name == nullptr || strcmp(name, r.name) != 0) continue;
        TMF_REQUIRE(r.ok == nullptr || r.ok(value), TMF_E_ARG, "tmf_set_option: %s must be %s, got %d", r.name, r.accepts, value);
        values().set[r.opt].store(r.set ? r.set(value) : value, std::memory_order_relaxed);
        return TMF_OK;
    }
    tmf_set_error("tmf_set_option: unknown option '%s'", name);
    return TMF_E_ARG;
}

extern "C" int tmf_snet_algo_flags(void) {
    int flags = TMF_SNET_ALGO;
    for (const Row& r : kRows)
        if (const int v = r.call[0] ? tmf_opt(r.opt) : 0) flags |= r.call[v - 1];
    return flags;
}

extern "C" int tmf_conv_wino_mode(void) { return tmf_opt(TMF_OPT_CONV_WINO); }
extern "C" int tmf_wino_p_mode(void) { return tmf_opt(TMF_OPT_WINO_P); }
extern "C" int tmf_wino_x_mode(void) { return tmf_opt(TMF_OPT_WINO_X); }
extern "C" int tmf_c1_split_mode(void) { return tmf_opt(TMF_OPT_C1_SPLIT); }
```

transmf_ad_amd/csrc/reduce.hip:

```cpp
#include "tmf_common.h"

#define TMF_RED_LANES 16
static __global__ __launch_bounds__(64 * TMF_RED_LANES) void tmf_slab_reduce_kernel(
    const float* __restrict__ partial, float* __restrict__ out, int nsplit, long n, int slabs_per_group,
    int tcin = 0, int tcout = 0) {
    __shared__ double red[TMF_RED_LANES][64];
    const int tx = threadIdx.x & 63, ty = threadIdx.x >> 6;
    const long e = (long)blockIdx.x * 64 + tx;
    const int g = blockIdx.y;
    const int s0 = g * slabs_per_group;
    int s1 = s0 + slabs_per_group;
    if (s1 > nsplit) s1 = nsplit;
    double a = 0.0;
    if (e < n) {
        int s = s0 + ty;
        for (; s + 3 * TMF_RED_LANES < s1; s += 4 * TMF_RED_LANES) {
            const float v0 = partial[(size_t)s * n + e];
            const float v1 = partial[(size_t)(s + TMF_RED_LANES) * n + e];
            const float v2 = partial[(size_t)(s + 2 * TMF_RED_LANES) * n + e];
            const float v3 = partial[(size_t)(s + 3 * TMF_RED_LANES) * n + e];
            a += ((double)v0 + (double)v1) + ((double)v2 + (double)v3);
        }
        for (; s < s1; s += TMF_RED_LANES) a += (double)partial[(size_t)s * n + e];
    }
    red[ty][tx] = a;
    __syncthreads();
    if (ty == 0 && e < n) {
#pragma unroll
        for (int k = 1; k < TMF_RED_LANES; ++k) a += red[k][tx];
        size_t o = (size_t)g * n + e;
        if (tcin > 0) {
            const int co = (int)(e % tcout), ci = (int)((e / tcout) % tcin), t = (int)(e / ((long)tcout * tcin));
            const int T = (int)(n / ((long)tcin * tcout));
            o = ((size_t)co * tcin + ci) * T + t;
        }
        out[o] = (float)a;
    }
}

static __global__ __launch_bounds__(64 * TMF_RED_LANES) void tmf_slab_reduce4_kernel(
    const float* __restrict__ partial, float* __restrict__ out, int nsplit, long n, int slabs_per_group,
    int tcin = 0, int tcout = 0) {
    typedef float f4 __attribute__((ext_vector_type(4)));
    __shared__ double red[TMF_RED_LANES][64][4];
    const int tx = threadIdx.x & 63, ty = threadIdx.x >> 6;
    const long e = ((long)blockIdx.x * 64 + tx) * 4;
    const int g = blockIdx.y;
    const int s0 = g * slabs_per_group;
    int s1 = s0 + slabs_per_group;
    if (s1 > nsplit) s1 = nsplit;
    double a[4] = {0.0, 0.0, 0.0, 0.0};
    if (e < n) {
        int s = s0 + ty;
        for (; s + 3 * TMF_RED_LANES < s1; s += 4 * TMF_RED_LANES) {
            const f4 v0 = *reinterpret_cast<const f4*>(partial + (size_t)s * n + e);
            const f4 v1 = *reinterpret_cast<const f4*>(partial + (size_t)(s + TMF_RED_LANES) * n + e);
            const f4 v2 = *reinterpret_cast<const f4*>(partial + (size_t)(s + 2 * TMF_RED_LANES) * n + e);
            const f4 v3 = *reinterpret_cast<const f4*>(partial + (size_t)(s + 3 * TMF_RED_LANES) * n + e);
#pragma unroll
            for (int c = 0; c < 4; ++c) a[c] += ((double)v0[c] + (double)v1[c]) + ((double)v2[c] + (double)v3[c]);
        }
        for (; s < s1; s += TMF_RED_LANES) {
            const f4 v = *reinterpret_cast<const f4*>(partial + (size_t)s * n + e);
#pragma unroll
            for (int c = 0; c < 4; ++c) a[c] += (double)v[c];
        }
    }
#pragma unroll
    for (int c = 0; c < 4; ++c) red[ty][tx][c] = a[c];
    __syncthreads();
    if (ty == 0 && e < n) {
#pragma unroll
        for (int k = 1; k < TMF_RED_LANES; ++k)
#pragma unroll
            for (int c = 0; c < 4; ++c) a[c] += red[k][tx][c];
        if (tcin > 0) {
            const int T = (int)(n / ((long)tcin * tcout));
#pragma unroll
            for (int c = 0; c < 4; ++c) {
                const long ec = e + c;
                const int co = (int)(ec % tcout), ci = (int)((ec / tcout) % tcin), t = (int)(ec / ((long)tcout * tcin));
                out[((size_t)co * tcin + ci) * T + t] = (float)a[c];
            }
        } else {
            *reinterpret_cast<f4*>(out + (size_t)g * n + e) = f4{(float)a[0], (float)a[1], (float)a[2], (float)a[3]};
        }
    }
}

int tmf_reduce_slabs(const float* partial, int nsplit, long n, float* scratch, float* out, hipStream_t s, const char* what,
                     int tcin, int tcout) {
    const int G = tmf_reduce_groups(nsplit);
    const dim3 block(64 * TMF_RED_LANES);
    const bool v4 = n % 4 == 0 && n >= 1024 && ((size_t)partial & 15) == 0 && ((size_t)out & 15) == 0 &&
                    (G == 1 || ((size_t)scratch & 15) == 0);
    const int gx = v4 ? (int)((n / 4 + 63) / 64) : (int)((n + 63) / 64);
    auto k = v4 ? tmf_slab_reduce4_kernel : tmf_slab_reduce_kernel;
    if (G == 1) {
        hipLaunchKernelGGL(k, dim3(gx, 1), block, 0, s, partial, out, nsplit, n, nsplit, tcin, tcout);
        return tmf_launch_result(what);
    }
    const int spg = (nsplit + G - 1) / G;
    hipLaunchKernelGGL(k, dim3(gx, G), block, 0, s, partial, scratch, nsplit, n, spg, 0, 0);
    int rc = tmf_launch_result(what);
    if (rc) return rc;
    hipLaunchKernelGGL(k, dim3(gx, 1), block, 0, s, (const float*)scratch, out, G, n, G, tcin, tcout);
    return tmf_launch_result(what);
}

extern "C" int tmf_colsum_finalize(const float* partial, int nblk, int ncol, float* out, void* stream) {
    TMF_REQUIRE_PTR(partial); TMF_REQUIRE_PTR(out);
    TMF_REQUIRE(nblk > 0 && ncol > 0, TMF_E_SHAPE, "tmf_colsum_finalize: nblk=%d ncol=%d", nblk, ncol);
    const dim3 block(64 * TMF_RED_LANES);
    hipLaunchKernelGGL(tmf_slab_reduce_kernel, dim3(tmf_cdiv(ncol, 64), 1), block, 0, (hipStream_t)stream,
                       partial, out, nblk, (long)ncol, nblk, 0, 0);
    return tmf_launch_result("tmf_colsum_finalize");
}
```

transmf_ad_amd/csrc/snet_path.hip:

```cpp
#include "tmf_common.h"

namespace {

constexpr int NL = TMF_SNET_BLOCKS;

struct LayerPlan {
    int cin, cout, k, pool;
    int D, H, W;
    int oD, oH, oW;
    int fwd, dgr, wgr;
    bool x16, z16, o16;
    size_t off_z, off_out, off_vec, off_wf, off_wd;
    bool route;
    size_t off_zsel, off_arg;
    size_t x_bytes, z_bytes, out_bytes;
    int cpad;
};

struct Plan {
    LayerPlan L[NL];
    size_t off_part;
    size_t off_c1gram = 0, c1gram_bytes = 0;
    size_t saved_bytes;
    size_t off_bpart, off_coef, off_dz, off_gA, off_gB, off_ws, scratch_bytes, ws_bytes;
    size_t off_dgws, dgws_bytes;
};

int check_desc(const char* fn, const tmf_snet_desc* d) {
    TMF_REQUIRE_PTR(d);
    TMF_REQUIRE(d->B > 0 && d->D >= 16 && d->H >= 16 && d->W >= 16, TMF_E_SHAPE,
                "%s: volume %dx%dx%d (batch %d): every edge must be >= 16 (four 2x2x2 pools)", fn, d->D, d->H, d->W, d->B);
    TMF_REQUIRE(d->dim >= 32 && d->dim % 32 == 0, TMF_E_SHAPE, "%s: dim=%d must be a positive multiple of 32", fn, d->dim);
    TMF_REQUIRE(d->precision == TMF_PREC_FP32 || d->precision == TMF_PREC_BF16 || d->precision == TMF_PREC_FP32X, TMF_E_ARG,
                "%s: unknown precision %d", fn, d->precision);
    TMF_REQUIRE(!d->storage_bf16 || d->precision == TMF_PREC_BF16, TMF_E_ARG,
                "%s: bf16 activation storage needs the bf16 precision", fn);
    return TMF_OK;
}


inline int rt_min_of(const tmf_snet_desc& d) { return (d.flags & TMF_SNET_ALONE) ? 1 : 0; }

int stat_rows(const tmf_snet_desc& d, const LayerPlan& L) {
    switch (L.fwd) {
    case TMF_CONV_BF16:  return tmf_conv3d_bf16_stat_blocks(d.B, L.D, L.H, L.W);
    case TMF_CONV_SPLIT: return tmf_conv3d_split_stat_blocks(d.B, L.D, L.H, L.W);
    case TMF_CONV_WINO:  return tmf_conv3d_wino_stat_blocks(d.B, L.D, L.H, L.W);
    default:             return tmf_conv3d_stat_blocks_mode(d.B, L.D, L.H, L.W, L.cin, L.cout, L.k, rt_min_of(d));
    }
}

size_t wgrad_workspace_bytes(const tmf_snet_desc& d, const LayerPlan& L) {
    switch (L.wgr) {
    case TMF_CONV_BF16: return tmf_conv3d_wgrad_bf16_workspace_bytes(d.B, L.D, L.H, L.W, L.cin, L.cout);
    case TMF_CONV_WINO: return tmf_conv3d_wgrad_wino_workspace_bytes(d.B, L.D, L.H, L.W, L.cin, L.cout);
    default:            return tmf_conv3d_wgrad_workspace_bytes(d.B, L.D, L.H, L.W, L.cin, L.cout, L.k);
    }
}

size_t weight_bytes(const LayerPlan& L, int family) {
    const size_t wn = (size_t)L.k * L.k * L.k * L.cin * L.cout;
    switch (family) {
    case TMF_CONV_WINO:  return tmf_conv3d_wino_weight_bytes(L.cin, L.cout);
    case TMF_CONV_SPLIT: return wn * 6;
    case TMF_CONV_BF16:  return wn * 2;
    default:             return wn * 4;
    }
}

int pack_weights(const LayerPlan& L, const float* w, void* wf, void* wd, void* stream) {
    const bool uf = L.fwd == TMF_CONV_WINO, ud = L.dgr == TMF_CONV_WINO;
    switch (L.fwd) {
    case TMF_CONV_BF16:  return tmf_pack_conv_weights_bf16(w, wf, wd, L.cout, L.cin, 27, stream);
    case TMF_CONV_SPLIT: return tmf_pack_conv_weights_split3(w, wf, wd, L.cout, L.cin, 27, stream);
    default:
        if (uf && ud) return TMF_OK;
        return tmf_pack_conv_weights(w, uf ? nullptr : (float*)wf, ud ? nullptr : (float*)wd, L.cout, L.cin, L.k * L.k * L.k, stream);
    }
}

int launch_fwd(const tmf_snet_desc& d, const LayerPlan& L, const void* x, const void* wf, void* z, float* part, void* stream) {
    switch (L.fwd) {
    case TMF_CONV_BF16:
        return tmf_conv3d_fwd_bf16_t(x, wf, z, part, d.B, L.D, L.H, L.W, L.cin, L.cout, (L.x16 ? 1 : 0) | (L.z16 ? 2 : 0), stream);
    case TMF_CONV_SPLIT:
        return tmf_conv3d_fwd_split((const float*)x, wf, (float*)z, part, d.B, L.D, L.H, L.W, L.cin, L.cout, stream);
    case TMF_CONV_WINO:
        return tmf_conv3d_fwd_wino((const float*)x, (const float*)wf, (float*)z, part, d.B, L.D, L.H, L.W, L.cin, L.cout, stream);
    default:
        return tmf_conv3d_fwd_mode((const float*)x, (const float*)wf, (float*)z, part, d.B, L.D, L.H, L.W, L.cin, L.cout, L.k,
                                   rt_min_of(d), stream);
    }
}

int launch_dgrad(const tmf_snet_desc& d, const LayerPlan& L, const void* dz, const void* wd, void* dx, void* stream) {
    switch (L.dgr) {
    case TMF_CONV_BF16:
        return tmf_conv3d_fwd_bf16_t(dz, wd, dx, nullptr, d.B, L.D, L.H, L.W, L.cout, L.cin, (L.z16 ? 1 : 0) | (L.x16 ? 2 : 0), stream);
    case TMF_CONV_SPLIT:
        return tmf_conv3d_fwd_split((const float*)dz, wd, (float*)dx, nullptr, d.B, L.D, L.H, L.W, L.cout, L.cin, stream);
    case TMF_CONV_WINO:
        return tmf_conv3d_fwd_wino((const float*)dz, (const float*)wd, (float*)dx, nullptr, d.B, L.D, L.H, L.W, L.cout, L.cin, stream);
    default:
        return tmf_conv3d_fwd_mode((const float*)dz, (const float*)wd, (float*)dx, nullptr, d.B, L.D, L.H, L.W, L.cout, L.cin, L.k,
                                   rt_min_of(d), stream);
    }
}

int launch_wgrad(const tmf_snet_desc& d, const LayerPlan& L, const void* x, const void* dz, float* dw, void* ws, size_t ws_bytes,
                 void* stream) {
    switch (L.wgr) {
    case TMF_CONV_BF16:
        return tmf_conv3d_wgrad_bf16_t(x, dz, dw, ws, ws_bytes, d.B, L.D, L.H, L.W, L.cin, L.cout, L.x16 ? 1 : 0, TMF_DW_REFERENCE, stream);
    case TMF_CONV_WINO:
        return tmf_conv3d_wgrad_wino((const float*)x, (const float*)dz, dw, ws, ws_bytes, d.B, L.D, L.H, L.W, L.cin, L.cout,
                                     TMF_DW_REFERENCE, stream);
    default:
        return tmf_conv3d_wgrad((const float*)x, (const float*)dz, dw, ws, ws_bytes, d.B, L.D, L.H, L.W, L.cin, L.cout, L.k,
                                TMF_DW_REFERENCE, stream);
    }
}

Plan make_plan(const tmf_snet_desc& d, bool train = true) {
    Plan p;
    const int rec = tmf_opt(TMF_OPT_POOL_RECOMPUTE);
    const int q = d.dim / 4, h = d.dim / 2, dm = d.dim, d2 = d.dim * 2;
    const int cin[NL] = {1, q, q, h, h, dm, d2}, cout[NL] = {q, q, h, h, dm, d2, dm};
    const int ks[NL] = {3, 3, 3, 3, 3, 3, 1};
    const int pool[NL] = {TMF_POOL_MAX2, TMF_POOL_NONE, TMF_POOL_MAX2, TMF_POOL_NONE, TMF_POOL_MAX2, TMF_POOL_NONE, TMF_POOL_AVG2};
    const bool b16 = d.precision == TMF_PREC_BF16, s16 = b16 && d.storage_bf16;
    int D = d.D, H = d.H, W = d.W;
    size_t off = 0;
    size_t part_max = 0, bpart_max = 0, z_max = 0, x_max = 0, ws_max = 0;
    for (int l = 0; l < NL; ++l) {
        LayerPlan& L = p.L[l];
        L.cin = cin[l]; L.cout = cout[l]; L.k = ks[l]; L.pool = pool[l];
        L.D = D; L.H = H; L.W = W;
        if (pool[l] != TMF_POOL_NONE) { D /= 2; H /= 2; W /= 2; }
        L.oD = D; L.oH = H; L.oW = W;
        const int algo = tmf_conv_block_algo(d.precision, cin[l], cout[l], ks[l]);
        L.fwd = algo & 15; L.dgr = (algo >> 4) & 15; L.wgr = (algo >> 8) & 15;
    }
    for (int l = 0; l < NL; ++l) {
        LayerPlan& L = p.L[l];
        const bool mine = l == 0 ? b16 : L.fwd == TMF_CONV_BF16;
        L.o16 = s16 && l + 1 < NL && mine && p.L[l + 1].fwd == TMF_CONV_BF16;
        L.z16 = s16 && L.fwd == TMF_CONV_BF16;
        L.x16 = l > 0 && p.L[l - 1].o16;
        const size_t vox = (size_t)d.B * L.D * L.H * L.W, ovox = (size_t)d.B * L.oD * L.oH * L.oW;
        L.x_bytes = vox * L.cin * (L.x16 ? 2 : 4);
        L.z_bytes = l == 0 ? 0 : vox * L.cout * (L.z16 ? 2 : 4);
        L.out_bytes = l == NL - 1 ? 0 : ovox * L.cout * (L.o16 ? 2 : 4);
        L.cpad = (int)(up256((size_t)L.cout * 4) / 4);
        L.off_z = off; off += up256(L.z_bytes);
        L.off_out = off; off += up256(L.out_bytes);
        L.route = train && d.precision == TMF_PREC_FP32 && L.pool == TMF_POOL_MAX2 && ovox > 0 &&
                  (l == 0 ? rec != 1 && rec != 2 && tmf_c1_gram_bytes(d.B, L.D, L.H, L.W, L.cout) > 0 : rec != 1 && rec != 3);
        L.off_zsel = off; off += L.route ? up256(ovox * L.cout * 4) : 0;
        L.off_arg = off; off += L.route && l == 0 ? up256(ovox * L.cout) : 0;
        L.off_vec = off; off += (size_t)4 * L.cpad * 4;
        L.off_wf = off; off += up256(weight_bytes(L, L.fwd));
        L.off_wd = off; off += l == 0 ? 0 : up256(weight_bytes(L, L.dgr));
        int nblk, nb2;
        size_t ws;
        if (l == 0) {
            nblk = tmf_c1_blocks(d.B, L.D, L.H, L.W, L.cout);
            nb2 = nblk;
            ws = tmf_c1_bwd_wgrad_workspace_bytes(d.B, L.D, L.H, L.W, L.cout);
            p.c1gram_bytes = d.precision == TMF_PREC_FP32 ? tmf_c1_gram_bytes(d.B, L.D, L.H, L.W, L.cout)
                             : b16 ? tmf_c1_gram_bytes_bf16(d.B, L.D, L.H, L.W, L.cout) : 0;
            if (p.c1gram_bytes) {
                const size_t wf_ = tmf_c1_bwd_fused_workspace_bytes(d.B, L.D, L.H, L.W, L.cout);
                if (wf_ > ws) ws = wf_;
            }
        } else {
            nblk = stat_rows(d, L);
            nb2 = tmf_bn_act_pool_bwd_blocks(d.B, L.D, L.H, L.W, L.cout, L.pool);
            ws = wgrad_workspace_bytes(d, L);
        }
        const size_t pb = (size_t)nblk * 2 * L.cout * 4, pb2 = (size_t)nb2 * 2 * L.cout * 4;
        if (pb > part_max) part_max = pb;
        if (pb2 > bpart_max) bpart_max = pb2;
        if (L.z_bytes > z_max) z_max = L.z_bytes;
        if (l > 0 && L.x_bytes > x_max) x_max = L.x_bytes;
        if (ws > ws_max) ws_max = ws;
    }
    p.off_part = off; off += up256(part_max);
    p.off_c1gram = off; off += up256(p.c1gram_bytes);
    p.saved_bytes = off;
    size_t so = 0;
    p.off_bpart = so; so += up256(bpart_max);
    p.off_coef = so; so += up256((size_t)2 * 2 * d.dim * 4);
    p.off_dz = so; so += up256(z_max);
    p.off_gA = so; so += up256(x_max);
    p.off_gB = so; so += up256(x_max);
    p.off_ws = so; so += up256(ws_max > 16 ? ws_max : 16);
    p.ws_bytes = ws_max > 16 ? ws_max : 16;
    p.dgws_bytes = tmf_c1_bwd_dgrad_workspace_bytes(d.B, p.L[0].D, p.L[0].H, p.L[0].W, p.L[0].cout);
    p.off_dgws = so; so += up256(p.dgws_bytes);
    p.scratch_bytes = so;
    return p;
}

struct Vecs { float *mean, *invstd, *scale, *shift; };
inline Vecs vecs_of(char* base, const LayerPlan& L) {
    float* v = (float*)(base + L.off_vec);
    return Vecs{v, v + L.cpad, v + 2 * L.cpad, v + 3 * L.cpad};
}

}

extern "C" int tmf_conv_block_algo(int precision, int cin, int cout, int ksize) {
    if (precision != TMF_PREC_FP32 && precision != TMF_PREC_BF16 && precision != TMF_PREC_FP32X) return -1;
    int fwd = TMF_CONV_DIRECT, dgr = TMF_CONV_DIRECT, wgr = TMF_CONV_DIRECT;
    if (ksize == 3 && cin > 1) {
        if (precision == TMF_PREC_FP32) {
            const int wino = tmf_opt(TMF_OPT_CONV_WINO);
            if (wino >= 2 && tmf_conv3d_wino_ok(cin, cout)) fwd = TMF_CONV_WINO;
            if (wino >= 1 && tmf_conv3d_wino_ok(cout, cin)) dgr = TMF_CONV_WINO;
            if (wino >= 3 && tmf_conv3d_wgrad_wino_ok(cin, cout)) wgr = TMF_CONV_WINO;
        } else if (cin % 8 == 0) {
            fwd = precision == TMF_PREC_BF16 ? TMF_CONV_BF16 : TMF_CONV_SPLIT;
            if (cout % 8 == 0) dgr = fwd;
            if (precision == TMF_PREC_BF16) wgr = TMF_CONV_BF16;
        }
    }
    return fwd | (dgr << 4) | (wgr << 8);
}

extern "C" size_t tmf_snet_saved_bytes(const tmf_snet_desc* d) {
    if (check_desc("tmf_snet_saved_bytes", d) != TMF_OK) return 0;
    const TmfAlgoScope algo_scope(d->flags);
    return make_plan(*d).saved_bytes;
}

extern "C" size_t tmf_snet_bwd_scratch_bytes(const tmf_snet_desc* d) {
    if (check_desc("tmf_snet_bwd_scratch_bytes", d) != TMF_OK) return 0;
    const TmfAlgoScope algo_scope(d->flags);
    return make_plan(*d).scratch_bytes;
}

extern "C" int tmf_snet_train_fwd(const tmf_snet_desc* d, const float* vol, const tmf_snet_params* prm,
                                  void* saved, size_t saved_bytes, float* out, void* stream) {
    TMF_TRY(check_desc("tmf_snet_train_fwd", d));
    const TmfAlgoScope algo_scope(d->flags);
    TMF_REQUIRE_PTR(vol); TMF_REQUIRE_PTR(prm); TMF_REQUIRE_PTR(saved); TMF_REQUIRE_PTR(out);
    TMF_REQUIRE_ALIGNED(vol); TMF_REQUIRE_ALIGNED(saved); TMF_REQUIRE_ALIGNED(out);
    const Plan p = make_plan(*d);
    TMF_REQUIRE(saved_bytes >= p.saved_bytes, TMF_E_WORKSPACE, "tmf_snet_train_fwd: saved workspace %zu B < required %zu B",
                saved_bytes, p.saved_bytes);
    for (int l = 0; l < NL; ++l) {
        TMF_REQUIRE(prm->weight[l] && prm->gamma[l] && prm->beta[l], TMF_E_NULL,
                    "tmf_snet_train_fwd: weight / gamma / beta of block %d is NULL", l);
    }
    char* base = (char*)saved;
    float* part = (float*)(base + p.off_part);
    const bool b16 = d->precision == TMF_PREC_BF16;
    const void* x = vol;
    {
        const float* pw[8]; float* pf[8]; float* pd[8]; int pco[8], pci[8];
        int n = 0;
        for (int l = 0; l < NL; ++l) {
            const LayerPlan& L = p.L[l];
            const bool uf = L.fwd == TMF_CONV_WINO, ud = L.dgr == TMF_CONV_WINO;
            if (!(uf || ud)) continue;
            pw[n] = prm->weight[l]; pf[n] = uf ? (float*)(base + L.off_wf) : nullptr; pd[n] = ud ? (float*)(base + L.off_wd) : nullptr;
            pco[n] = L.cout; pci[n] = L.cin; ++n;
        }
        if (n > 0) TMF_TRY(tmf_pack_conv_weights_wino_multi(n, pw, pf, pd, pco, pci, stream));
    }
    for (int l = 0; l < NL; ++l) {
        const LayerPlan& L = p.L[l];
        const Vecs v = vecs_of(base, L);
        void* o = l == NL - 1 ? (void*)out : (void*)(base + L.off_out);
        void* wf = base + L.off_wf;
        void* wd = base + L.off_wd;
        void* z = base + L.off_z;
        const double count = (double)d->B * L.D * L.H * L.W;
        const bool has_out = (size_t)L.oD * L.oH * L.oW > 0;
        int nblk;
        if (l == 0) {
            TMF_TRY(tmf_pack_conv_weights(prm->weight[l], (float*)wf, nullptr, L.cout, 1, 27, stream));
            nblk = tmf_c1_blocks(d->B, L.D, L.H, L.W, L.cout);
            if (p.c1gram_bytes) {
                if (b16) TMF_TRY(tmf_c1_stats_g_bf16(vol, (const float*)wf, part, base + p.off_c1gram, p.c1gram_bytes, d->B, L.D, L.H, L.W,
                                                     L.cout, stream));
                else     TMF_TRY(tmf_c1_stats_g(vol, (const float*)wf, part, base + p.off_c1gram, p.c1gram_bytes, d->B, L.D, L.H, L.W, L.cout,
                                                stream));
                nblk = 2;
            } else if (b16) TMF_TRY(tmf_c1_stats_bf16(vol, (const float*)wf, part, d->B, L.D, L.H, L.W, L.cout, stream));
            else     TMF_TRY(tmf_c1_stats(vol, (const float*)wf, part, d->B, L.D, L.H, L.W, L.cout, stream));
        } else {
            TMF_TRY(pack_weights(L, prm->weight[l], wf, wd, stream));
            nblk = stat_rows(*d, L);
            TMF_TRY(launch_fwd(*d, L, x, wf, z, part, stream));
        }
        TMF_TRY(tmf_bn_finalize(part, nblk, L.cout, count, prm->gamma[l], prm->beta[l], prm->bias[l], prm->running_mean[l],
                                prm->running_var[l], d->momentum[l], d->eps[l], v.mean, v.invstd, v.scale, v.shift, stream));
        if (has_out) {
            if (l == 0) {
                if (b16) TMF_TRY(tmf_c1_bn_pool_fwd_bf16(vol, (const float*)wf, v.scale, v.shift, o, d->B, L.D, L.H, L.W, L.cout,
                                                         d->slope[l], L.o16 ? 1 : 0, stream));
                else if (L.route) TMF_TRY(tmf_c1_bn_pool_fwd_route(vol, (const float*)wf, v.scale, v.shift, (float*)o, (float*)(base + L.off_zsel),
                                                                   (unsigned char*)(base + L.off_arg), d->B, L.D, L.H, L.W, L.cout, d->slope[l],
                                                                   stream));
                else     TMF_TRY(tmf_c1_bn_pool_fwd(vol, (const float*)wf, v.scale, v.shift, (float*)o, d->B, L.D, L.H, L.W,
                                                    L.cout, d->slope[l], stream));
            } else if (L.route) {
                TMF_TRY(tmf_bn_act_pool_fwd_route((const float*)z, v.scale, v.shift, (float*)o, (float*)(base + L.off_zsel), d->B, L.D, L.H,
                                                  L.W, L.cout, d->slope[l], stream));
            } else {
                TMF_TRY(tmf_bn_act_pool_fwd_t(z, v.scale, v.shift, o, d->B, L.D, L.H, L.W, L.cout, L.pool, d->slope[l],
                                              (L.z16 ? 1 : 0) | (L.o16 ? 2 : 0), stream));
            }
        }
        x = o;
    }
    return TMF_OK;
}

extern "C" size_t tmf_snet_eval_workspace_bytes(const tmf_snet_desc* d) {
    if (check_desc("tmf_snet_eval_workspace_bytes", d) != TMF_OK) return 0;
// ... 19 lines not shown
                    "tmf_snet_eval_fwd: weight / gamma / beta / running statistics of block %d is NULL", l);
    char* base = (char*)workspace;
    const bool b16 = d->precision == TMF_PREC_BF16;
    const void* x = vol;
    for (int l = 0; l < NL; ++l) {
        const LayerPlan& L = p.L[l];
        const Vecs v = vecs_of(base, L);
        void* o = l == NL - 1 ? (void*)out : (void*)(base + L.off_out);
        void* wf = base + L.off_wf;
        const int fam = (L.fwd == TMF_CONV_WINO && L.pool == TMF_POOL_AVG2) ? TMF_CONV_DIRECT : L.fwd;
        switch (fam) {
        case TMF_CONV_BF16: TMF_TRY(tmf_pack_conv_weights_bf16(prm->weight[l], wf, nullptr, L.cout, L.cin, 27, stream)); break;
        case TMF_CONV_WINO: TMF_TRY(tmf_pack_conv_weights_wino(prm->weight[l], (float*)wf, nullptr, L.cout, L.cin, stream)); break;
        default:            TMF_TRY(tmf_pack_conv_weights(prm->weight[l], (float*)wf, nullptr, L.cout, L.cin, L.k * L.k * L.k, stream));
        }
        TMF_TRY(tmf_bn_eval_coeffs(prm->gamma[l], prm->beta[l], prm->bias[l], prm->running_mean[l], prm->running_var[l],
                                   d->eps[l], L.cout, v.scale, v.shift, stream));
        if ((size_t)L.oD * L.oH * L.oW == 0) continue;
        if (l == 0) {
            if (b16) TMF_TRY(tmf_c1_bn_pool_fwd_bf16(vol, (const float*)wf, v.scale, v.shift, o, d->B, L.D, L.H, L.W, L.cout,
                                                     d->slope[l], L.o16 ? 1 : 0, stream));
            else     TMF_TRY(tmf_c1_bn_pool_fwd(vol, (const float*)wf, v.scale, v.shift, (float*)o, d->B, L.D, L.H, L.W, L.cout,
                                                d->slope[l], stream));
        } else if (b16) {
            void* z = base + L.off_z;
            if (fam == TMF_CONV_BF16) TMF_TRY(launch_fwd(*d, L, x, wf, z, nullptr, stream));
            else TMF_TRY(tmf_conv3d_fwd((const float*)x, (const float*)wf, (float*)z, nullptr, d->B, L.D, L.H, L.W, L.cin, L.cout, L.k, stream));
            TMF_TRY(tmf_bn_act_pool_fwd_t(z, v.scale, v.shift, o, d->B, L.D, L.H, L.W, L.cout, L.pool, d->slope[l],
                                          (L.z16 ? 1 : 0) | (L.o16 ? 2 : 0), stream));
        } else if (fam == TMF_CONV_WINO) {
            TMF_TRY(tmf_conv3d_fwd_wino_affine((const float*)x, (const float*)wf, v.scale, v.shift, (float*)o, d->B, L.D, L.H, L.W,
                                               L.cin, L.cout, L.pool, d->slope[l], stream));
        } else {
            TMF_TRY(tmf_conv3d_fwd_affine((const float*)x, (const float*)wf, v.scale, v.shift, (float*)o, d->B, L.D, L.H, L.W,
                                          L.cin, L.cout, L.k, L.pool, d->slope[l], stream));
        }
        x = o;
    }
    return TMF_OK;
}

extern "C" int tmf_snet_train_bwd_input(const tmf_snet_desc* d, const float* vol, const void* saved, size_t saved_bytes,
                                        const float* dout, const tmf_snet_grads* g, void* scratch, size_t scratch_bytes,
                                        void* stream, float* dvol) {
    TMF_TRY(check_desc("tmf_snet_train_bwd", d));
    TMF_REQUIRE(dvol == nullptr || d->precision != TMF_PREC_BF16, TMF_E_ARG,
                "tmf_snet_train_bwd_input: the input gradient needs the fp32 or fp32x precision");
    if (dvol != nullptr) TMF_REQUIRE_ALIGNED(dvol);
    const TmfAlgoScope algo_scope(d->flags);
    TMF_REQUIRE_PTR(vol); TMF_REQUIRE_PTR(saved); TMF_REQUIRE_PTR(dout); TMF_REQUIRE_PTR(g); TMF_REQUIRE_PTR(scratch);
    TMF_REQUIRE_ALIGNED(vol); TMF_REQUIRE_ALIGNED(saved); TMF_REQUIRE_ALIGNED(dout); TMF_REQUIRE_ALIGNED(scratch);
    const Plan p = make_plan(*d);
    TMF_REQUIRE(saved_bytes >= p.saved_bytes, TMF_E_WORKSPACE, "tmf_snet_train_bwd: saved workspace %zu B < required %zu B",
                saved_bytes, p.saved_bytes);
    TMF_REQUIRE(scratch_bytes >= p.scratch_bytes, TMF_E_WORKSPACE, "tmf_snet_train_bwd: scratch %zu B < required %zu B",
                scratch_bytes, p.scratch_bytes);
    char* base = (char*)saved;
    char* sc = (char*)scratch;
    float* part = (float*)(sc + p.off_bpart);
    float* coef = (float*)(sc + p.off_coef);
    void* dz = sc + p.off_dz;
    void* ws = sc + p.off_ws;
    hipStream_t s = (hipStream_t)stream;
    const bool b16 = d->precision == TMF_PREC_BF16;
    bool bias_filled = false;
    {
        float* first = nullptr;
        const float* expect = nullptr;
        size_t total = 0;
        bool contiguous = true;
        for (int l = 0; l < NL; ++l) {
            if (g->dbias[l] == nullptr) continue;
            if (first == nullptr) first = g->dbias[l];
            else if (g->dbias[l] != expect) contiguous = false;
            expect = g->dbias[l] + p.L[l].cout;
            total += (size_t)p.L[l].cout;
        }
        if (first != nullptr && contiguous) {
            hipError_t e = hipMemsetAsync(first, 0, total * 4, s);
            TMF_REQUIRE(e == hipSuccess, (int)e, "tmf_snet_train_bwd: memset failed: %s", hipGetErrorString(e));
            bias_filled = true;
        }
    }
    const void* go = dout;
    for (int l = NL - 1; l >= 0; --l) {
        const LayerPlan& L = p.L[l];
        const Vecs v = vecs_of(base, L);
        const void* x = l == 0 ? (const void*)vol : (const void*)(base + p.L[l - 1].off_out);
        const void* wf = base + L.off_wf;
        const void* wd = base + L.off_wd;
        const void* z = base + L.off_z;
        const double count = (double)d->B * L.D * L.H * L.W;
        if (g->dbias[l] != nullptr && !bias_filled) {
            hipError_t e = hipMemsetAsync(g->dbias[l], 0, (size_t)L.cout * 4, s);
            TMF_REQUIRE(e == hipSuccess, (int)e, "tmf_snet_train_bwd: memset failed: %s", hipGetErrorString(e));
        }
        if ((size_t)L.oD * L.oH * L.oW == 0) continue;
        if (l == 0 && p.c1gram_bytes && g->dweight[l] != nullptr) {
            if (dvol != nullptr) {
                TMF_TRY(tmf_c1_bwd_fused_coef(vol, (const float*)wf, v.scale, v.shift, v.mean, v.invstd, (const float*)go,
                                              L.route ? (const float*)(base + L.off_zsel) : nullptr,
                                              L.route ? (const unsigned char*)(base + L.off_arg) : nullptr, base + p.off_c1gram,
                                              g->dweight[l], g->dgamma[l], g->dbeta[l], coef, ws, p.ws_bytes, d->B, L.D, L.H, L.W, L.cout,
                                              d->slope[l], TMF_DW_REFERENCE, stream));
                TMF_TRY(tmf_c1_bwd_dgrad(vol, (const float*)wf, v.scale, v.shift, v.mean, v.invstd, coef, (const float*)go, dvol,
                                         sc + p.off_dgws, p.dgws_bytes, d->B, L.D, L.H, L.W, L.cout, d->slope[l], stream));
                break;
            }
            if (b16) TMF_TRY(tmf_c1_bwd_fused_bf16(vol, (const float*)wf, v.scale, v.shift, v.mean, v.invstd, go, base + p.off_c1gram,
                                                   g->dweight[l], g->dgamma[l], g->dbeta[l], ws, p.ws_bytes, d->B, L.D, L.H, L.W, L.cout,
                                                   d->slope[l], L.o16 ? 1 : 0, TMF_DW_REFERENCE, stream));
            else if (L.route) TMF_TRY(tmf_c1_bwd_fused_route(vol, (const float*)wf, v.scale, v.shift, v.mean, v.invstd, (const float*)go,
                                                             (const float*)(base + L.off_zsel), (const unsigned char*)(base + L.off_arg),
                                                             base + p.off_c1gram, g->dweight[l], g->dgamma[l], g->dbeta[l], ws, p.ws_bytes,
                                                             d->B, L.D, L.H, L.W, L.cout, d->slope[l], TMF_DW_REFERENCE, stream));
            else     TMF_TRY(tmf_c1_bwd_fused(vol, (const float*)wf, v.scale, v.shift, v.mean, v.invstd, (const float*)go,
                                              base + p.off_c1gram, g->dweight[l], g->dgamma[l], g->dbeta[l], ws, p.ws_bytes, d->B, L.D,
                                              L.H, L.W, L.cout, d->slope[l], TMF_DW_REFERENCE, stream));
            break;
        }
        if (l == 0) {
            const int nblk = tmf_c1_blocks(d->B, L.D, L.H, L.W, L.cout);
            if (b16) TMF_TRY(tmf_c1_bwd_reduce_bf16(vol, (const float*)wf, v.scale, v.shift, v.mean, v.invstd, go, part, d->B, L.D,
                                                    L.H, L.W, L.cout, d->slope[l], L.o16 ? 1 : 0, stream));
            else     TMF_TRY(tmf_c1_bwd_reduce(vol, (const float*)wf, v.scale, v.shift, v.mean, v.invstd, (const float*)go, part,
                                               d->B, L.D, L.H, L.W, L.cout, d->slope[l], stream));
            TMF_TRY(tmf_bn_bwd_finalize(part, nblk, L.cout, count, g->dgamma[l], g->dbeta[l], coef, stream));
            if (g->dweight[l] != nullptr) {
                if (b16) TMF_TRY(tmf_c1_bwd_wgrad_bf16(vol, (const float*)wf, v.scale, v.shift, v.mean, v.invstd, coef, go,
                                                       g->dweight[l], ws, p.ws_bytes, d->B, L.D, L.H, L.W, L.cout, d->slope[l],
                                                       L.o16 ? 1 : 0, TMF_DW_REFERENCE, stream));
                else     TMF_TRY(tmf_c1_bwd_wgrad(vol, (const float*)wf, v.scale, v.shift, v.mean, v.invstd, coef,
                                                  (const float*)go, g->dweight[l], ws, p.ws_bytes, d->B, L.D, L.H, L.W, L.cout,
                                                  d->slope[l], TMF_DW_REFERENCE, stream));
            }
            if (dvol != nullptr)
                TMF_TRY(tmf_c1_bwd_dgrad(vol, (const float*)wf, v.scale, v.shift, v.mean, v.invstd, coef, (const float*)go, dvol,
                                         sc + p.off_dgws, p.dgws_bytes, d->B, L.D, L.H, L.W, L.cout, d->slope[l], stream));
            break;
        }
        const int io = (L.z16 ? 1 : 0) | (L.o16 ? 2 : 0);
        const int nblk = tmf_bn_act_pool_bwd_blocks(d->B, L.D, L.H, L.W, L.cout, L.pool);
        if (L.route) TMF_TRY(tmf_bn_act_pool_bwd_reduce_route((const float*)(base + L.off_zsel), (const float*)go, v.scale, v.shift, v.mean,
                                                              v.invstd, part, d->B, L.D, L.H, L.W, L.cout, d->slope[l], stream));
        else TMF_TRY(tmf_bn_act_pool_bwd_reduce_t(z, go, v.scale, v.shift, v.mean, v.invstd, part, d->B, L.D, L.H, L.W, L.cout, L.pool,
                                                  d->slope[l], io, stream));
        TMF_TRY(tmf_bn_bwd_finalize(part, nblk, L.cout, count, g->dgamma[l], g->dbeta[l], coef, stream));
        TMF_TRY(tmf_bn_act_pool_bwd_apply_t(z, go, v.scale, v.shift, v.mean, v.invstd, coef, dz, d->B, L.D, L.H, L.W, L.cout,
                                            L.pool, d->slope[l], io, stream));
        void* dx = sc + ((l & 1) ? p.off_gA : p.off_gB);
        if (g->dweight[l] != nullptr) TMF_TRY(launch_wgrad(*d, L, x, dz, g->dweight[l], ws, p.ws_bytes, stream));
        TMF_TRY(launch_dgrad(*d, L, dz, wd, dx, stream));
        go = dx;
        if (l == TMF_SNET_DEEP_FROM && g->deep_event != nullptr) {
            hipError_t e = hipEventRecord((hipEvent_t)g->deep_event, s);
            TMF_REQUIRE(e == hipSuccess, (int)e, "tmf_snet_train_bwd: hipEventRecord failed: %s", hipGetErrorString(e));
        }
    }
    return TMF_OK;
}

extern "C" int tmf_snet_train_bwd(const tmf_snet_desc* d, const float* vol, const void* saved, size_t saved_bytes,
                                  const float* dout, const tmf_snet_grads* g, void* scratch, size_t scratch_bytes,
                                  void* stream) {
    return tmf_snet_train_bwd_input(d, vol, saved, saved_bytes, dout, g, scratch, scratch_bytes, stream, nullptr);
}
```

transmf_ad_amd/csrc/tmf_common.h:

```cpp
#pragma once
#include <hip/hip_runtime.h>
#include <stdarg.h>
#include <stdio.h>
#include <stdlib.h>
#include <string.h>
#include "../../include/tmf_hip.h"

typedef float f32x16 __attribute__((ext_vector_type(16)));
typedef float f32x4 __attribute__((ext_vector_type(4)));
#ifdef __HIPCC__
typedef __bf16 tmf_bf16x2 __attribute__((ext_vector_type(2)));
typedef __bf16 tmf_bf16x8 __attribute__((ext_vector_type(8)));
__device__ __forceinline__ unsigned int tmf_pack_bf16(float a, float b) {
    const tmf_bf16x2 v = {(__bf16)a, (__bf16)b};
    return __builtin_bit_cast(unsigned int, v);
}
typedef unsigned short tmf_bf16_t;
typedef unsigned int tmf_u32x2 __attribute__((ext_vector_type(2)));
typedef float tmf_f32x1 __attribute__((ext_vector_type(1)));
template <typename T, int VEC> struct TmfIO;
template <> struct TmfIO<float, 4> {
    static __device__ __forceinline__ f32x4 ld(const float* p) { return *reinterpret_cast<const f32x4*>(p); }
    static __device__ __forceinline__ void st(float* p, f32x4 v) { *reinterpret_cast<f32x4*>(p) = v; }
    static __device__ __forceinline__ f32x4 ld_nt(const float* p) { return __builtin_nontemporal_load(reinterpret_cast<const f32x4*>(p)); }
    static __device__ __forceinline__ void st_nt(float* p, f32x4 v) { __builtin_nontemporal_store(v, reinterpret_cast<f32x4*>(p)); }
};
template <> struct TmfIO<float, 1> {
    static __device__ __forceinline__ tmf_f32x1 ld(const float* p) { return *reinterpret_cast<const tmf_f32x1*>(p); }
    static __device__ __forceinline__ void st(float* p, tmf_f32x1 v) { *p = v[0]; }
};
template <> struct TmfIO<tmf_bf16_t, 4> {
    static __device__ __forceinline__ f32x4 ld(const tmf_bf16_t* p) {
        const tmf_u32x2 r = *reinterpret_cast<const tmf_u32x2*>(p);
        return f32x4{__builtin_bit_cast(float, r[0] << 16), __builtin_bit_cast(float, r[0] & 0xFFFF0000u),
                     __builtin_bit_cast(float, r[1] << 16), __builtin_bit_cast(float, r[1] & 0xFFFF0000u)};
    }
    static __device__ __forceinline__ void st(tmf_bf16_t* p, f32x4 v) {
        *reinterpret_cast<tmf_u32x2*>(p) = tmf_u32x2{tmf_pack_bf16(v[0], v[1]), tmf_pack_bf16(v[2], v[3])};
    }
};
typedef float tmf_f32x8 __attribute__((ext_vector_type(8)));
typedef unsigned int tmf_u32x4 __attribute__((ext_vector_type(4)));
template <> struct TmfIO<float, 8> {
    static __device__ __forceinline__ tmf_f32x8 ld(const float* p) {
        const f32x4 a = *reinterpret_cast<const f32x4*>(p), b = *reinterpret_cast<const f32x4*>(p + 4);
        return tmf_f32x8{a[0], a[1], a[2], a[3], b[0], b[1], b[2], b[3]};
    }
    static __device__ __forceinline__ void st(float* p, tmf_f32x8 v) {
        *reinterpret_cast<f32x4*>(p) = f32x4{v[0], v[1], v[2], v[3]};
        *reinterpret_cast<f32x4*>(p + 4) = f32x4{v[4], v[5], v[6], v[7]};
    }
};
template <> struct TmfIO<tmf_bf16_t, 8> {
    static __device__ __forceinline__ tmf_f32x8 ld(const tmf_bf16_t* p) {
        const tmf_u32x4 r = *reinterpret_cast<const tmf_u32x4*>(p);
        tmf_f32x8 v;
#pragma unroll
        for (int i = 0; i < 4; ++i) {
            v[2 * i] = __builtin_bit_cast(float, r[i] << 16);
            v[2 * i + 1] = __builtin_bit_cast(float, r[i] & 0xFFFF0000u);
        }
        return v;
    }
    static __device__ __forceinline__ void st(tmf_bf16_t* p, tmf_f32x8 v) {
        *reinterpret_cast<tmf_u32x4*>(p) = tmf_u32x4{tmf_pack_bf16(v[0], v[1]), tmf_pack_bf16(v[2], v[3]),
                                                      tmf_pack_bf16(v[4], v[5]), tmf_pack_bf16(v[6], v[7])};
    }
};
template <> struct TmfIO<tmf_bf16_t, 1> {
    static __device__ __forceinline__ tmf_f32x1 ld(const tmf_bf16_t* p) {
        return tmf_f32x1{__builtin_bit_cast(float, (unsigned int)(*p) << 16)};
    }
    static __device__ __forceinline__ void st(tmf_bf16_t* p, tmf_f32x1 v) {
        *p = (tmf_bf16_t)(tmf_pack_bf16(v[0], 0.f) & 0xFFFFu);
    }
};
#endif

void tmf_set_error(const char* fmt, ...);
int tmf_conv3d_fwd_mode(const float* x, const float* w, float* z, float* stat_partial, int B, int D, int H, int W, int cin,
                        int cout, int ksize, int rt_min, void* stream);
int tmf_conv3d_stat_blocks_mode(int B, int D, int H, int W, int cin, int cout, int ksize, int rt_min);
enum TmfOpt {
    TMF_OPT_CONV_WINO, TMF_OPT_WINO_P, TMF_OPT_WINO_X, TMF_OPT_C1_GRAM, TMF_OPT_C1_SPLIT, TMF_OPT_POOL_RECOMPUTE,
    TMF_OPT_WINO_CUS, TMF_OPT_CONV_RT, TMF_OPT_CONV_WAVES, TMF_OPT_BF16_V2, TMF_OPT_BF16_DMA, TMF_OPT_WGRAD_TR, TMF_OPT_DEBUG,
    TMF_OPT_WINO_EVEN, TMF_OPT_WINOX_SWAP, TMF_OPT_BF_NT2, TMF_OPT_CONV_AUTO, TMF_OPT_C1_BLOCKS, TMF_OPT_C1_FWD_MULT,
    TMF_OPT_COUNT
};
int tmf_opt(TmfOpt o);
struct TmfAlgoScope {
    int prev;
    explicit TmfAlgoScope(int flags);
    ~TmfAlgoScope();
    TmfAlgoScope(const TmfAlgoScope&) = delete;
    TmfAlgoScope& operator=(const TmfAlgoScope&) = delete;
};
int tmf_winox_takes(int B, int D, int H, int W, int cin, int cout, int geom);
long tmf_winox_items(int D, int H, int W, int* swap);
int tmf_winox_first_grid(long nitems, int ncu);
int tmf_winox_launch(const char* what, const float* x, const unsigned short* u3, float* z, float* stat_partial, int B, int D, int H,
                     int W, int cin, int cout, int ncu, hipStream_t stream, const float* scale = nullptr, const float* shift = nullptr,
                     float slope = 0.f, int pool = 0);
#define TMF_INTERNAL __attribute__((visibility("hidden")))
TMF_INTERNAL
int tmf_tok_linear_fwd_impl(const float* x, const float* w, const float* bias, const float* residual, float* y, int R, int K,
                            int Nout, const float* ln_gamma, const float* ln_beta, float eps, float* ln_mean, float* ln_rstd,
                            float* ln_out, float* gelu_pre, const float* mask, void* stream);
TMF_INTERNAL
int tmf_tok_linear_bwd_input_impl(const float* dy, const float* w, float* dx, int R, int Nout, int K, const float* gelu_pre,
                                 const float* ln_x, const float* ln_mean, const float* ln_rstd, const float* ln_gamma,
                                 const float* add1, const float* add2, float* ln_partial, float* bias_partial,
                                 int partial_stride, const float* mask, float* dx_masked, void* stream);
TMF_INTERNAL
int tmf_layernorm_bwd_impl(const float* x, const float* gamma, const float* mean, const float* rstd, const float* dy, float* dx,
                          float* partial, int rows, int dim, const float* mask, float* dx_masked, void* stream);

#define TMF_REQUIRE_PTR(p)                                                     \
    do {                                                                       \
        if ((p) == nullptr) {                                                  \
            tmf_set_error("%s: argument '%s' is NULL", __func__, #p);          \
            return TMF_E_NULL;                                                 \
        }                                                                      \
    } while (0)

#define TMF_REQUIRE_ALIGNED(p)                                                 \
    do {                                                                       \
        if ((reinterpret_cast<uintptr_t>(p) & 15u) != 0) {                     \
            tmf_set_error("%s: argument '%s' is not 16-byte aligned", __func__, #p); \
            return TMF_E_ALIGN;                                                \
        }                                                                      \
    } while (0)

#define TMF_REQUIRE(cond, code, ...)                                           \
    do {                                                                       \
        if (!(cond)) {                                                         \
            tmf_set_error(__VA_ARGS__);                                        \
            return (code);                                                     \
        }                                                                      \
    } while (0)

#define TMF_REQUIRE_PTR_FN(fn, p) TMF_REQUIRE((p) != nullptr, TMF_E_NULL, "%s: argument '%s' is NULL", (fn), #p)
#define TMF_REQUIRE_ALIGNED_FN(fn, p) \
    TMF_REQUIRE((reinterpret_cast<uintptr_t>(p) & 15u) == 0, TMF_E_ALIGN, "%s: argument '%s' is not 16-byte aligned", (fn), #p)

#define TMF_TRY(call) do { int rc__ = (call); if (rc__ != TMF_OK) return rc__; } while (0)

static inline int tmf_launch_result(const char* what, const char* tag = "") {
    hipError_t e = hipGetLastError();
    if (e != hipSuccess) {
        tmf_set_error("%s%s: launch failed: %s", what, tag, hipGetErrorString(e));
        return (int)e;
    }
    return TMF_OK;
}

template <typename K>
static inline int tmf_allow_lds(K kernel, size_t bytes, const char* what) {
    static thread_local const void* last_fn[8] = {};
    static thread_local size_t last_sz[8] = {};
    static thread_local int last_dev[8] = {-1, -1, -1, -1, -1, -1, -1, -1};
    const void* fn = reinterpret_cast<const void*>(kernel);
    const unsigned slot = (unsigned)((reinterpret_cast<uintptr_t>(fn) >> 4) & 7u);
    int dev = 0;
    (void)hipGetDevice(&dev);
    if (last_fn[slot] == fn && last_dev[slot] == dev && last_sz[slot] >= bytes) return TMF_OK;
    hipError_t e = hipFuncSetAttribute(fn, hipFuncAttributeMaxDynamicSharedMemorySize, (int)bytes);
    if (e != hipSuccess) {
        tmf_set_error("%s: cannot reserve %zu B of LDS: %s", what, bytes, hipGetErrorString(e));
        return (int)e;
    }
    last_fn[slot] = fn;
    last_sz[slot] = bytes;
    last_dev[slot] = dev;
    return TMF_OK;
}

static inline int tmf_cdiv(long a, long b) { return (int)((a + b - 1) / b); }
static inline size_t up256(size_t n) { return (n + 255) & ~(size_t)255; }

static inline int tmf_wino_window_grid(long n, int ncu, int even) {
    if (n <= ncu) return (int)n;
    if (!even) return ncu;
    const long rounds = (n + ncu - 1) / ncu;
    return (int)((n + rounds - 1) / rounds);
}

static inline int tmf_reduce_groups(int nsplit) {
    if (nsplit <= 64) return 1;
    int g = nsplit / 16;
    return g > 32 ? 32 : g;
}
int tmf_reduce_slabs(const float* partial, int nsplit, long n, float* scratch, float* out, hipStream_t s, const char* what,
                     int tcin = 0, int tcout = 0);

#ifdef __HIPCC__
__host__ __device__ __forceinline__ int xcd_contiguous(int bid, int n) {
    const int q = n >> 3, r = n & 7;
    const int xcd = bid & 7, idx = bid >> 3;
    const int start = xcd < r ? xcd * (q + 1) : r * (q + 1) + (xcd - r) * q;
    return start + idx;
}

__device__ __forceinline__ float wave_sum(float v) {
#pragma unroll
    for (int o = 32; o > 0; o >>= 1) v += __shfl_xor(v, o);
    return v;
}
__device__ __forceinline__ float wave_max(float v) {
#pragma unroll
    for (int o = 32; o > 0; o >>= 1) v = fmaxf(v, __shfl_xor(v, o));
    return v;
}
#endif
```

transmf_ad_amd/ops.py:

```python
from __future__ import annotations

import ctypes
import math
import os

import torch
from torch.autograd.function import once_differentiable

from . import _lib

_f32 = torch.float32


def _stream():
    return torch._C._cuda_getCurrentRawStream(torch._C._cuda_getDevice())


def _chk(t: torch.Tensor, name: str, allow_bf16: bool = False) -> torch.Tensor:
    if not t.is_cuda:
        raise _lib.TmfError(
            f"{name} is on {t.device}: transmf_ad_amd runs only on a HIP device (MI355X); there is no CPU fallback")
    if t.device.index != torch._C._cuda_getDevice():
        raise _lib.TmfError(
            f"{name} is on {t.device} but the current HIP device is cuda:{torch._C._cuda_getDevice()}: "
# ... 496 lines not shown
    if out.numel() > 0:
        if conv_block_algo("fp32", cin, cout, k)[0] == _lib.CONV_WINO and pool != "avg":
            uf, _ = pack_weights_wino(weight, True, False)
            _lib.call("tmf_conv3d_fwd_wino_affine", x.data_ptr(), uf.data_ptr(), scale.data_ptr(), shift.data_ptr(),
                      out.data_ptr(), B, D, H, W, cin, cout, pc, float(slope), s)
        else:
            _lib.call("tmf_conv3d_fwd_affine", x.data_ptr(), pack_weight(weight).data_ptr(), scale.data_ptr(),
                      shift.data_ptr(), out.data_ptr(), B, D, H, W, cin, cout, k, pc, float(slope), s)
    return out


FUSE_EVAL_BLOCKS = os.environ.get("TMF_FUSE_EVAL", "1") != "0"


def conv_bn_act_pool(x, weight, bias, gamma, beta, running_mean, running_var, training,
                     momentum=0.1, eps=1e-5, slope=0.01, pool=None, out_bf16=False, precision=None):
    precision = resolve_precision(precision)
    mode, act16 = precision
    needs_graph = torch.is_grad_enabled() and (x.requires_grad or weight.requires_grad or gamma.requires_grad)
    if (FUSE_EVAL_BLOCKS and not training and not needs_graph and mode == "fp32" and weight.shape[1] > 1
            and weight.shape[1] % 4 == 0 and weight.shape[0] % 4 == 0):
        return conv_bn_act_pool_eval_fused(x, weight, bias, gamma, beta, running_mean, running_var, eps, slope, pool)
    if (weight.shape[1] == 1 and weight.shape[2] == 3 and pool == "max"
            and (not x.requires_grad or (mode != "bf16" and not out_bf16))):
        if out_bf16 and mode != "bf16":
            raise _lib.TmfError("a bf16 block output needs conv precision 'bf16'")
        return Conv1BnPool.apply(x, weight, bias, gamma, beta, running_mean, running_var,
                                 training, momentum, eps, slope, out_bf16 and mode == "bf16", precision)
    can16 = out_bf16 and act16 and bf16_conv_capable(weight.shape[1], weight.shape[2])
    y = ConvBnActPool.apply(x, weight, bias, gamma, beta, running_mean, running_var,
                            training, momentum, eps, slope, pool, can16, precision)
    return y.to(_b16) if (out_bf16 and not can16) else y



SNET_ONE_CALL = os.environ.get("TMF_SNET_C", "1") != "0"


def snet_one_call_supported(B, D, H, W, dim, precision=None):
    return (SNET_ONE_CALL and resolve_precision(precision)[0] in ("fp32", "bf16", "fp32x") and dim >= 32 and dim % 32 == 0
            and min(D, H, W) >= 16 and B > 0)


def snet_eval_one_call(vol, dim, eps, slope, blocks, precision=None, algo=None):
    import ctypes as C
    vol = _chk(vol, "vol")
    B, _, D, H, W = vol.shape
    mode, act16 = resolve_precision(precision)
    desc = _lib.SnetDesc(B=B, D=D, H=H, W=W, dim=dim, precision=_lib.PRECISION[mode], storage_bf16=int(act16),
                         flags=snet_algo_flags(algo))
    prm = _lib.SnetParams()
    for l, (w, b, g, be, rm, rv) in enumerate(blocks):
        desc.eps[l], desc.slope[l], desc.momentum[l] = eps[l], slope[l], 0.0
        prm.weight[l], prm.bias[l], prm.gamma[l], prm.beta[l] = w.data_ptr(), _ptr(b), g.data_ptr(), be.data_ptr()
        prm.running_mean[l], prm.running_var[l] = rm.data_ptr(), rv.data_ptr()
    nws = _lib.query("tmf_snet_eval_workspace_bytes", C.byref(desc))
    ws = torch.empty(nws, device=vol.device, dtype=torch.uint8)
    out = torch.empty((B, D // 16, H // 16, W // 16, dim), device=vol.device, dtype=_f32)
    _lib.call("tmf_snet_eval_fwd", C.byref(desc), vol.data_ptr(), C.byref(prm), ws.data_ptr(), nws, out.data_ptr(), _stream())
    return out


import weakref

_FLAT_GRAD_CONSUMERS = weakref.WeakSet()


def add_flat_grad_consumer(consumer) -> None:
    _FLAT_GRAD_CONSUMERS.add(consumer)


def remove_flat_grad_consumer(consumer) -> None:
    _FLAT_GRAD_CONSUMERS.discard(consumer)


def _publish_flat_grads(flat, param_ptrs, views, segments) -> None:
    for c in list(_FLAT_GRAD_CONSUMERS):
        c.tmf_flat_grads(flat, param_ptrs, views, segments)


def snet_algo_flags(algo=None) -> int:
    f = _lib.query("tmf_snet_algo_flags")
    if algo:
        bad = set(algo) - {"conv_wino", "wino_p", "wino_x", "c1_gram", "c1_split", "pool_recompute"}
        if bad:
            raise ValueError(f"unknown algorithm option(s) {sorted(bad)}")
        if "conv_wino" in algo:
            if algo["conv_wino"] not in (0, 1, 2, 3):
                raise ValueError("conv_wino must be 0, 1, 2 or 3")
            f = (f & ~_lib.snet_algo_wino(3)) | _lib.snet_algo_wino(int(algo["conv_wino"]))
        for key, bit in (("wino_p", _lib.SNET_ALGO_WINO_P), ("wino_x", _lib.SNET_ALGO_WINO_X), ("c1_gram", _lib.SNET_ALGO_C1_GRAM),
                         ("c1_split", _lib.SNET_ALGO_C1_SPLIT)):
            if key in algo:
                f = (f | bit) if algo[key] else (f & ~bit)
        if "c1_gram" in algo:
            f = (f | _lib.SNET_ALGO_C1_GRAM_BF16) if algo["c1_gram"] == 2 else (f & ~_lib.SNET_ALGO_C1_GRAM_BF16)
        if "pool_recompute" in algo:
            if algo["pool_recompute"] not in (0, 1, 2, 3):
                raise ValueError("pool_recompute must be 0, 1, 2 or 3")
            c1, bn = _lib.SNET_ALGO_POOL_REC_C1, _lib.SNET_ALGO_POOL_REC_BN
            f = (f & ~(c1 | bn)) | {0: 0, 1: c1 | bn, 2: c1, 3: bn}[int(algo["pool_recompute"])]
    return f


class SNetTrain(torch.autograd.Function):

    @staticmethod
    def forward(ctx, vol, cfg, buffers, *params):
        import ctypes as C
        vol = _chk(vol, "vol")
        dim, momentum, eps, slope = cfg[:4]
        mode, act16 = resolve_precision(cfg[4] if len(cfg) > 4 else None)
        B, _, D, H, W = vol.shape
        desc = _lib.SnetDesc(B=B, D=D, H=H, W=W, dim=dim, precision=_lib.PRECISION[mode], storage_bf16=int(act16),
                             flags=(_lib.SNET_ALONE if (len(cfg) > 5 and cfg[5]) else 0) | snet_algo_flags(cfg[6] if len(cfg) > 6 else None))
        if not any(ctx.needs_input_grad):
            desc.flags |= _lib.SNET_ALGO_POOL_REC_C1 | _lib.SNET_ALGO_POOL_REC_BN
        prm = _lib.SnetParams()
        for l in range(7):
            desc.momentum[l], desc.eps[l], desc.slope[l] = momentum[l], eps[l], slope[l]
            w, b, g, be = params[4 * l:4 * l + 4]
            rm, rv = buffers[l]
            for t, name in ((w, "conv weight"), (g, "BatchNorm weight"), (be, "BatchNorm bias")):
                if not (t.is_cuda and t.dtype == _f32 and t.is_contiguous()):
                    raise _lib.TmfError(f"sNet block {l}: {name} must be a contiguous float32 tensor on the HIP device")
            prm.weight[l], prm.bias[l], prm.gamma[l], prm.beta[l] = w.data_ptr(), _ptr(b), g.data_ptr(), be.data_ptr()
            prm.running_mean[l], prm.running_var[l] = _ptr(rm), _ptr(rv)
        nsaved = _lib.query("tmf_snet_saved_bytes", C.byref(desc))
        if nsaved == 0:
            raise _lib.TmfError("tmf_snet_saved_bytes: " + (_lib.load().tmf_last_error_string() or b"").decode())
        saved = torch.empty(nsaved, device=vol.device, dtype=torch.uint8)
        out = torch.empty((B, D // 16, H // 16, W // 16, dim), device=vol.device, dtype=_f32)
        _lib.call("tmf_snet_train_fwd", C.byref(desc), vol.data_ptr(), C.byref(prm), saved.data_ptr(), nsaved,
                  out.data_ptr(), _stream())
        ctx.save_for_backward(vol, saved)
        ctx.desc = desc
        ctx.shapes = [None if p is None else p.shape for p in params]
        ctx.param_ptrs = [None if p is None else p.data_ptr() for p in params]
        ctx.bwd = SNetTrain._prepare_backward(ctx.shapes, ctx.needs_input_grad, vol.device) if any(ctx.needs_input_grad[3:]) else None
        return out

    @staticmethod
    def _prepare_backward(shapes, need, dev):
        sizes = [0 if s is None else s.numel() for s in shapes]
        flat = torch.empty(sum(sizes), device=dev, dtype=_f32)
        shallow = [i for i in range(4 * _lib.SNET_DEEP_FROM) if i % 4 != 1]
        order = shallow + [i for i in range(4 * _lib.SNET_DEEP_FROM, len(sizes)) if i % 4 != 1] + \
            [i for i in range(len(sizes)) if i % 4 == 1]
        parts = dict(zip(order, flat.split([sizes[i] for i in order])))
        o_deep = sum(sizes[i] for i in shallow)
        grads = [None if s is None else (parts[i] if len(s) == 1 else parts[i].view(s)) for i, s in enumerate(shapes)]
        ptr = [parts[i].data_ptr() for i in range(len(sizes))]
        g = _lib.SnetGrads()
        for l in range(7):
            g.dweight[l] = ptr[4 * l] if need[3 + 4 * l] else None
            g.dbias[l] = None if shapes[4 * l + 1] is None else ptr[4 * l + 1]
            g.dgamma[l], g.dbeta[l] = ptr[4 * l + 2], ptr[4 * l + 3]
        ev = torch.cuda.Event()
        ev.record(torch.cuda.current_stream(dev))
        g.deep_event = ev.cuda_event
        return flat, grads, g, ev, o_deep

    @staticmethod
    @once_differentiable
    def backward(ctx, dout):
        import ctypes as C
        vol, saved = ctx.saved_tensors
        desc = ctx.desc
        dout = _chk(dout, "grad_output")
        prep = ctx.bwd if ctx.bwd is not None else SNetTrain._prepare_backward(ctx.shapes, ctx.needs_input_grad, vol.device)
        ctx.bwd = None
        flat, grads, g, ev, o_deep = prep
        nscr = _lib.query("tmf_snet_bwd_scratch_bytes", C.byref(desc))
        scratch = torch.empty(nscr, device=vol.device, dtype=torch.uint8)
        dvol = None
        if ctx.needs_input_grad[0]:
            dvol = torch.empty_like(vol)
            _lib.call("tmf_snet_train_bwd_input", C.byref(desc), vol.data_ptr(), saved.data_ptr(), saved.numel(), dout.data_ptr(),
                      C.byref(g), scratch.data_ptr(), nscr, _stream(), dvol.data_ptr())
        else:
            _lib.call("tmf_snet_train_bwd", C.byref(desc), vol.data_ptr(), saved.data_ptr(), saved.numel(), dout.data_ptr(),
                      C.byref(g), scratch.data_ptr(), nscr, _stream())
        out = [dvol, None, None]
        for i, gr in enumerate(grads):
            out.append(gr if (gr is not None and ctx.needs_input_grad[3 + i]) else None)
        if _FLAT_GRAD_CONSUMERS and all(ctx.needs_input_grad[3 + i] for i, gr in enumerate(grads) if gr is not None):
            _publish_flat_grads(flat, ctx.param_ptrs, grads, [(o_deep, flat.numel(), ev, "now"), (0, o_deep, None, "end")])
        return tuple(out)



class CrossAttention(torch.autograd.Function):

    @staticmethod
    def forward(ctx, q, kv, heads, scale):
        q, kv = _chk(q, "q"), _chk(kv, "kv")
        B, N, inner = q.shape
        M = kv.shape[1]
        if kv.shape[2] != 2 * inner or inner % heads:
            raise _lib.TmfError(f"attention shapes: q {tuple(q.shape)} kv {tuple(kv.shape)} heads {heads}")
        dh = inner // heads
        out = torch.empty((B, N, inner), device=q.device, dtype=_f32)
        lse = torch.empty((B, heads, N), device=q.device, dtype=_f32)
        _lib.call("tmf_xattn_fwd", q.data_ptr(), kv.data_ptr(), kv.data_ptr() + inner * 4, out.data_ptr(),
                  lse.data_ptr(), B, heads, N, M, dh, inner, 2 * inner, float(scale), _stream())
        ctx.save_for_backward(q, kv, out, lse)
        ctx.cfg = (heads, float(scale))
        return out

    @staticmethod
    def backward(ctx, dout):
        q, kv, out, lse = ctx.saved_tensors
        heads, scale = ctx.cfg
        B, N, inner = q.shape
        M = kv.shape[1]
        dh = inner // heads
        dout = _chk(dout, "grad_output")
        dq = torch.empty_like(q)
        dkv = torch.empty_like(kv)
        _lib.call("tmf_xattn_bwd", q.data_ptr(), kv.data_ptr(), kv.data_ptr() + inner * 4, out.data_ptr(),
                  lse.data_ptr(), dout.data_ptr(), dq.data_ptr(), dkv.data_ptr(), dkv.data_ptr() + inner * 4,
                  B, heads, N, M, dh, inner, 2 * inner, 2 * inner, scale, _stream())
        return dq, dkv, None, None


def cross_attention(q, kv, heads, scale):
    return CrossAttention.apply(q, kv, heads, scale)



class LayerNorm(torch.autograd.Function):
    @staticmethod
    def forward(ctx, x, gamma, beta, eps, residual):
        x = _chk(x, "x")
        dim = x.shape[-1]
        rows = x.numel() // dim
        y = torch.empty_like(x)
        mean = torch.empty(rows, device=x.device, dtype=_f32)
        rstd = torch.empty(rows, device=x.device, dtype=_f32)
        res = _chk(residual, "residual") if residual is not None else None
        _lib.call("tmf_layernorm_fwd", x.data_ptr(), gamma.data_ptr(), beta.data_ptr(), _ptr(res), y.data_ptr(),
                  mean.data_ptr(), rstd.data_ptr(), rows, dim, float(eps), _stream())
        ctx.save_for_backward(x, gamma, mean, rstd)
        ctx.has_res = residual is not None
        return y

    @staticmethod
    def backward(ctx, dy):
        x, gamma, mean, rstd = ctx.saved_tensors
        dim = x.shape[-1]
        rows = x.numel() // dim
        dy = _chk(dy, "grad_output")
        dx = torch.empty_like(x)
        nblk = _lib.query("tmf_layernorm_bwd_blocks", rows, dim)
        part = torch.empty((nblk, 2, dim), device=x.device, dtype=_f32)
        s = _stream()
        _lib.call("tmf_layernorm_bwd", x.data_ptr(), gamma.data_ptr(), mean.data_ptr(), rstd.data_ptr(),
                  dy.data_ptr(), dx.data_ptr(), part.data_ptr(), rows, dim, s)
        gb = torch.empty((2, dim), device=x.device, dtype=_f32)
        _lib.call("tmf_colsum_finalize", part.data_ptr(), nblk, 2 * dim, gb.data_ptr(), s)
        return dx, gb[0], gb[1], None, (dy if ctx.has_res else None)


def layer_norm(x, gamma, beta, eps=1e-5, residual=None):
    return LayerNorm.apply(x, gamma, beta, eps, residual)



def tok_linear_fwd(x, w, bias=None, residual=None, ln=None, gelu=False, keep_ln_out=False, mask=None):
# ... 1234 lines not shown
```

Baseline: 1066.

## Batch per-layer weight-gradient slab reductions into one multi-problem kernel launch

Weight-gradient kernels in the SNet backward no longer launch their own split-K slab reduction. They record a deferred problem, each with a dedicated workspace region in the enlarged backward scratch, and a single multi-problem reduce kernel handles all of them at the deep-event point and at the end. This is meant to remove many small reduce launches and their serialization in the backward pass. The cost is more scratch memory, since partials must persist until the batched reduce, and dW becomes available later, which could delay overlap with gradient consumers.

```diff
diff --git a/include/tmf_hip.h b/include/tmf_hip.h
--- a/include/tmf_hip.h
+++ b/include/tmf_hip.h
@@ -74,6 +74,7 @@
 int    tmf_wino_p_mode(void);
 int    tmf_conv3d_wgrad_wino_ok(int cin, int cout);
 size_t tmf_conv3d_wgrad_wino_workspace_bytes(int B, int D, int H, int W, int cin, int cout);
+int    tmf_conv3d_wgrad_wino_splits(int B, int D, int H, int W, int cin, int cout);
 int    tmf_conv3d_wgrad_wino(const float* x, const float* dz, float* dw, void* workspace, size_t workspace_bytes,
                              int B, int D, int H, int W, int cin, int cout, int dw_layout, void* stream);
 
@@ -176,6 +177,14 @@
 
 int tmf_colsum_finalize(const float* partial, int nblk, int ncol, float* out, void* stream);
 
+#define TMF_SLAB_MULTI_MAX 64
+int tmf_reduce_slabs_groups(int nsplit);
+int tmf_reduce_slabs_plan(const float* partial, int nsplit, long long n, float* scratch, float* out, int tcin, int tcout,
+                          void* stream);
+int tmf_reduce_slabs_multi_ptrs(int nproblems, const float* const* partial, float* const* out, const long long* n,
+                                const int* nsplit, const int* tcin, const int* tcout, void* stream);
+int tmf_slab_multi_mode(void);
+
 int tmf_xattn_fwd(const float* q, const float* k, const float* v, float* out, float* lse,
                   int B, int heads, int N, int M, int dh, int q_stride, int kv_stride, float scale,
                   void* stream);
@@ -275,6 +284,7 @@
 #define TMF_SNET_ALGO_C1_SPLIT 0x8000
 #define TMF_SNET_ALGO_POOL_REC_C1 0x10000
 #define TMF_SNET_ALGO_POOL_REC_BN 0x20000
+#define TMF_SNET_ALGO_SLAB_PER_LAYER 0x40000
 int  tmf_snet_algo_flags(void);
 int  tmf_c1_split_mode(void);
 #define TMF_CONV_DIRECT 0
@@ -310,6 +320,7 @@
 } tmf_snet_grads;
 size_t tmf_snet_saved_bytes(const tmf_snet_desc* d);
 size_t tmf_snet_bwd_scratch_bytes(const tmf_snet_desc* d);
+size_t tmf_snet_bwd_scratch_bytes_multi(const tmf_snet_desc* d);
 int    tmf_snet_train_fwd(const tmf_snet_desc* d, const float* vol, const tmf_snet_params* params,
                           void* saved, size_t saved_bytes, float* out, void* stream);
 int    tmf_snet_train_bwd(const tmf_snet_desc* d, const float* vol, const void* saved, size_t saved_bytes,
diff --git a/transmf_ad_amd/csrc/conv1_fused.hip b/transmf_ad_amd/csrc/conv1_fused.hip
--- a/transmf_ad_amd/csrc/conv1_fused.hip
+++ b/transmf_ad_amd/csrc/conv1_fused.hip
@@ -506,7 +506,7 @@
 static int c1_bwd_wgrad(bool bf16, bool p16, const float* x, const float* w, const float* scale, const float* shift,
                         const float* mean, const float* invstd, const float* coef, const void* dpool,
                         float* dw, void* workspace, size_t workspace_bytes,
-                        int B, int D, int H, int W, int C, float slope, int dw_layout, void* stream) {
+                        int B, int D, int H, int W, int C, float slope, int dw_layout, void* stream, TmfSlabProblem* defer = nullptr) {
     TMF_REQUIRE(dw_layout == TMF_DW_TAPMAJOR || dw_layout == TMF_DW_REFERENCE, TMF_E_ARG,
                 "tmf_c1_bwd_wgrad: unknown dw_layout %d", dw_layout);
     TMF_REQUIRE_PTR(x); TMF_REQUIRE_PTR(w); TMF_REQUIRE_PTR(scale); TMF_REQUIRE_PTR(shift); TMF_REQUIRE_PTR(mean);
@@ -528,8 +528,19 @@
     else             hipLaunchKernelGGL((conv1_fused_kernel<MODE_WGRAD, false>), dim3(p.nblk, p.nby), dim3(256), 0, s, a);
     if ((rc = tmf_launch_result("tmf_c1_bwd_wgrad"))) return rc;
     const long n = 27L * C;
+    if (defer != nullptr) {
+        *defer = TmfSlabProblem{(const float*)workspace, dw, n, p.nblk, dw_layout == TMF_DW_REFERENCE ? 1 : 0, C};
+        return TMF_OK;
+    }
     return tmf_reduce_slabs((const float*)workspace, p.nblk, n, (float*)workspace + (size_t)p.nblk * n, dw, s,
                             "tmf_c1_bwd_wgrad(reduce)", dw_layout == TMF_DW_REFERENCE ? 1 : 0, C);
+}
+int tmf_c1_bwd_wgrad_slabs(bool bf16, bool pooled_bf16, const float* x, const float* w, const float* scale, const float* shift,
+                           const float* mean, const float* invstd, const float* coef, const void* dpool, float* dw, void* workspace,
+                           size_t workspace_bytes, int B, int D, int H, int W, int C, float slope, int dw_layout, void* stream,
+                           TmfSlabProblem* defer) {
+    return c1_bwd_wgrad(bf16, pooled_bf16, x, w, scale, shift, mean, invstd, coef, dpool, dw, workspace, workspace_bytes, B, D, H, W,
+                        C, slope, dw_layout, stream, defer);
 }
 
 extern "C" int tmf_c1_bwd_wgrad(const float* x, const float* w, const float* scale, const float* shift,
diff --git a/transmf_ad_amd/csrc/conv3d_mfma.hip b/transmf_ad_amd/csrc/conv3d_mfma.hip
--- a/transmf_ad_amd/csrc/conv3d_mfma.hip
+++ b/transmf_ad_amd/csrc/conv3d_mfma.hip
@@ -1508,6 +1508,11 @@
 extern "C" int tmf_conv3d_wgrad(const float* x, const float* dz, float* dw, void* workspace,
                                 size_t workspace_bytes, int B, int D, int H, int W, int cin, int cout,
                                 int ksize, int dw_layout, void* stream) {
+    return tmf_conv3d_wgrad_slabs(x, dz, dw, workspace, workspace_bytes, B, D, H, W, cin, cout, ksize, dw_layout, stream, nullptr);
+}
+
+int tmf_conv3d_wgrad_slabs(const float* x, const float* dz, float* dw, void* workspace, size_t workspace_bytes, int B, int D, int H,
+                           int W, int cin, int cout, int ksize, int dw_layout, void* stream, TmfSlabProblem* defer) {
     TMF_REQUIRE(dw_layout == TMF_DW_TAPMAJOR || dw_layout == TMF_DW_REFERENCE, TMF_E_ARG,
                 "tmf_conv3d_wgrad: unknown dw_layout %d", dw_layout);
     TMF_REQUIRE_PTR(x); TMF_REQUIRE_PTR(dz); TMF_REQUIRE_PTR(dw); TMF_REQUIRE_PTR(workspace);
@@ -1574,6 +1579,10 @@
         nelem = (long)cin * cout;
         nsplit = p.nsplit;
     }
+    if (defer != nullptr) {
+        *defer = TmfSlabProblem{partial, dw, nelem, nsplit, dw_layout == TMF_DW_REFERENCE ? cin : 0, cout};
+        return TMF_OK;
+    }
     return tmf_reduce_slabs(partial, nsplit, nelem, partial + (size_t)nsplit * nelem, dw, s, "tmf_conv3d_wgrad(reduce)",
                             dw_layout == TMF_DW_REFERENCE ? cin : 0, cout);
 }
diff --git a/transmf_ad_amd/csrc/conv3d_wino.hip b/transmf_ad_amd/csrc/conv3d_wino.hip
--- a/transmf_ad_amd/csrc/conv3d_wino.hip
+++ b/transmf_ad_amd/csrc/conv3d_wino.hip
@@ -1734,8 +1734,18 @@
     return (size_t)(p.nsplit + tmf_reduce_groups(p.nsplit) + 1) * n * 4;
 }
 
+extern "C" int tmf_conv3d_wgrad_wino_splits(int B, int D, int H, int W, int cin, int cout) {
+    if (B <= 0 || D <= 0 || H <= 0 || W <= 0 || !tmf_conv3d_wgrad_wino_ok(cin, cout)) return 0;
+    return plan_wino_wgrad(B, D, H, W, cin, cout).nsplit;
+}
+
 extern "C" int tmf_conv3d_wgrad_wino(const float* x, const float* dz, float* dw, void* workspace, size_t workspace_bytes,
                                      int B, int D, int H, int W, int cin, int cout, int dw_layout, void* stream) {
+    return tmf_conv3d_wgrad_wino_slabs(x, dz, dw, workspace, workspace_bytes, B, D, H, W, cin, cout, dw_layout, stream, nullptr);
+}
+
+int tmf_conv3d_wgrad_wino_slabs(const float* x, const float* dz, float* dw, void* workspace, size_t workspace_bytes, int B, int D,
+                                int H, int W, int cin, int cout, int dw_layout, void* stream, TmfSlabProblem* defer) {
     TMF_REQUIRE(dw_layout == TMF_DW_TAPMAJOR || dw_layout == TMF_DW_REFERENCE, TMF_E_ARG,
                 "tmf_conv3d_wgrad_wino: unknown dw_layout %d", dw_layout);
     TMF_REQUIRE_PTR(x); TMF_REQUIRE_PTR(dz); TMF_REQUIRE_PTR(dw); TMF_REQUIRE_PTR(workspace);
@@ -1761,9 +1771,14 @@
         if ((rc = tmf_launch_result("tmf_conv3d_wgrad_wino"))) return rc;
         const long nw = (long)27 * cin * cout;
         const bool ref = dw_layout == TMF_DW_REFERENCE;
+        if (defer != nullptr) {
+            *defer = TmfSlabProblem{partial, dw, nw, p.nsplit, ref ? cin : 0, ref ? cout : 0};
+            return TMF_OK;
+        }
         return tmf_reduce_slabs(partial, p.nsplit, nw, partial + (size_t)p.nsplit * nw, dw, s, "tmf_conv3d_wgrad_wino(reduce)",
                                 ref ? cin : 0, ref ? cout : 0);
     }
+    if (defer != nullptr) defer->partial = nullptr;
     auto k = conv3d_wino_wgrad_kernel;
     if ((rc = tmf_allow_lds(k, WG_LDS_BYTES, "tmf_conv3d_wgrad_wino"))) return rc;
     hipLaunchKernelGGL(k, dim3(p.nsplit, p.nblk), dim3(NTHR), WG_LDS_BYTES, s, x, dz, partial, D, H, W, cin, cout,
diff --git a/transmf_ad_amd/csrc/options.hip b/transmf_ad_amd/csrc/options.hip
--- a/transmf_ad_amd/csrc/options.hip
+++ b/transmf_ad_amd/csrc/options.hip
@@ -7,6 +7,7 @@
 constexpr int UNSET = INT_MIN;
 
 int nonzero(int v) { return v != 0; }
+int is_zero(int v) { return v == 0; }
 int clamp02(int v) { return v <= 0 ? 0 : (v >= 2 ? 2 : 1); }
 bool in02(int v) { return v >= 0 && v <= 2; }
 
@@ -33,6 +34,7 @@
     {TMF_OPT_POOL_RECOMPUTE, "pool_recompute", "TMF_POOL_RECOMPUTE", 0, "0, 1, 2 or 3", [](int v) { return v >= 0 && v <= 3; }, nullptr,
      [](int v) { return v >= 0 && v <= 3 ? v : 0; },
      {TMF_SNET_ALGO_POOL_REC_C1 | TMF_SNET_ALGO_POOL_REC_BN, TMF_SNET_ALGO_POOL_REC_C1, TMF_SNET_ALGO_POOL_REC_BN}},
+    {TMF_OPT_SLAB_PER_LAYER, "slab_multi", "TMF_SLAB_MULTI", 0, nullptr, nullptr, is_zero, is_zero, {TMF_SNET_ALGO_SLAB_PER_LAYER}},
     {TMF_OPT_WINO_CUS, "wino_cus", "TMF_WINO_CUS", 0, ">= 0", [](int v) { return v >= 0; }, [](int v) { return v ? v : UNSET; },
      nullptr, {}},
     {TMF_OPT_CONV_RT, "conv_rt", "TMF_CONV_RT", 0, "0, 1 or 2", in02, nullptr, [](int v) { return v == 1 || v == 2 ? v : 0; }, {}},
@@ -117,3 +119,4 @@
 extern "C" int tmf_wino_p_mode(void) { return tmf_opt(TMF_OPT_WINO_P); }
 extern "C" int tmf_wino_x_mode(void) { return tmf_opt(TMF_OPT_WINO_X); }
 extern "C" int tmf_c1_split_mode(void) { return tmf_opt(TMF_OPT_C1_SPLIT); }
+extern "C" int tmf_slab_multi_mode(void) { return tmf_opt(TMF_OPT_SLAB_PER_LAYER) ? 0 : 1; }
diff --git a/transmf_ad_amd/csrc/reduce.hip b/transmf_ad_amd/csrc/reduce.hip
--- a/transmf_ad_amd/csrc/reduce.hip
+++ b/transmf_ad_amd/csrc/reduce.hip
@@ -1,99 +1,164 @@
 #include "tmf_common.h"
+#include <algorithm>
 
 #define TMF_RED_LANES 16
-static __global__ __launch_bounds__(64 * TMF_RED_LANES) void tmf_slab_reduce_kernel(
-    const float* __restrict__ partial, float* __restrict__ out, int nsplit, long n, int slabs_per_group,
-    int tcin = 0, int tcout = 0) {
-    __shared__ double red[TMF_RED_LANES][64];
+#define TMF_RED_MAX_GROUPS 32
+
+template <int V> using slab_vec = float __attribute__((ext_vector_type(V)));
+
+template <int V, typename Load>
+static __device__ __forceinline__ void slab_lane_sum(double (&a)[V], int first, int s1, Load load) {
+    int s = first;
+    for (; s + 3 * TMF_RED_LANES < s1; s += 4 * TMF_RED_LANES) {
+        const slab_vec<V> v0 = load(s);
+        const slab_vec<V> v1 = load(s + TMF_RED_LANES);
+        const slab_vec<V> v2 = load(s + 2 * TMF_RED_LANES);
+        const slab_vec<V> v3 = load(s + 3 * TMF_RED_LANES);
+#pragma unroll
+        for (int c = 0; c < V; ++c) a[c] += ((double)v0[c] + (double)v1[c]) + ((double)v2[c] + (double)v3[c]);
+    }
+    for (; s < s1; s += TMF_RED_LANES) {
+        const slab_vec<V> v = load(s);
+#pragma unroll
+        for (int c = 0; c < V; ++c) a[c] += (double)v[c];
+    }
+}
+
+template <int V, typename Load>
+static __device__ __forceinline__ void slab_group_sum(double (&a)[V], double (*red)[64][V], int s0, int s1, bool live, int tx, int ty,
+                                                      Load load) {
+#pragma unroll
+    for (int c = 0; c < V; ++c) a[c] = 0.0;
+    if (live) slab_lane_sum<V>(a, s0 + ty, s1, load);
+#pragma unroll
+    for (int c = 0; c < V; ++c) red[ty][tx][c] = a[c];
+    __syncthreads();
+    if (ty == 0 && live) {
+#pragma unroll
+        for (int k = 1; k < TMF_RED_LANES; ++k)
+#pragma unroll
+            for (int c = 0; c < V; ++c) a[c] += red[k][tx][c];
+    }
+}
+
+template <int V>
+static __device__ __forceinline__ void slab_store(const double (&a)[V], float* __restrict__ out, long n, long e, size_t flat, int tcin,
+                                                  int tcout) {
+    if (tcin > 0) {
+        const int T = (int)(n / ((long)tcin * tcout));
+#pragma unroll
+        for (int c = 0; c < V; ++c) {
+            const long ec = e + c;
+            const int co = (int)(ec % tcout), ci = (int)((ec / tcout) % tcin), t = (int)(ec / ((long)tcout * tcin));
+            out[((size_t)co * tcin + ci) * T + t] = (float)a[c];
+        }
+    } else {
+        slab_vec<V> r;
+#pragma unroll
+        for (int c = 0; c < V; ++c) r[c] = (float)a[c];
+        *reinterpret_cast<slab_vec<V>*>(out + flat) = r;
+    }
+}
+
+template <int V>
+static __device__ __forceinline__ void slab_reduce_body(const float* __restrict__ partial, float* __restrict__ out, int nsplit, long n,
+                                                        int slabs_per_group, int tcin, int tcout) {
+    __shared__ double red[TMF_RED_LANES][64][V];
     const int tx = threadIdx.x & 63, ty = threadIdx.x >> 6;
-    const long e = (long)blockIdx.x * 64 + tx;
+    const long e = ((long)blockIdx.x * 64 + tx) * V;
     const int g = blockIdx.y;
     const int s0 = g * slabs_per_group;
     int s1 = s0 + slabs_per_group;
     if (s1 > nsplit) s1 = nsplit;
-    double a = 0.0;
-    if (e < n) {
-        int s = s0 + ty;
-        for (; s + 3 * TMF_RED_LANES < s1; s += 4 * TMF_RED_LANES) {
-            const float v0 = partial[(size_t)s * n + e];
-            const float v1 = partial[(size_t)(s + TMF_RED_LANES) * n + e];
-            const float v2 = partial[(size_t)(s + 2 * TMF_RED_LANES) * n + e];
-            const float v3 = partial[(size_t)(s + 3 * TMF_RED_LANES) * n + e];
-            a += ((double)v0 + (double)v1) + ((double)v2 + (double)v3);
-        }
-        for (; s < s1; s += TMF_RED_LANES) a += (double)partial[(size_t)s * n + e];
-    }
-    red[ty][tx] = a;
-    __syncthreads();
-    if (ty == 0 && e < n) {
-#pragma unroll
-        for (int k = 1; k < TMF_RED_LANES; ++k) a += red[k][tx];
-        size_t o = (size_t)g * n + e;
-        if (tcin > 0) {
-            const int co = (int)(e % tcout), ci = (int)((e / tcout) % tcin), t = (int)(e / ((long)tcout * tcin));
-            const int T = (int)(n / ((long)tcin * tcout));
-            o = ((size_t)co * tcin + ci) * T + t;
-        }
-        out[o] = (float)a;
-    }
-}
-
+    const bool live = e < n;
+    double a[V];
+    slab_group_sum<V>(a, red, s0, s1, live, tx, ty,
+                      [&](int s) { return *reinterpret_cast<const slab_vec<V>*>(partial + (size_t)s * n + e); });
+    if (ty == 0 && live) slab_store<V>(a, out, n, e, (size_t)g * n + e, tcin, tcout);
+}
+static __global__ __launch_bounds__(64 * TMF_RED_LANES) void tmf_slab_reduce_kernel(
+    const float* __restrict__ partial, float* __restrict__ out, int nsplit, long n, int slabs_per_group,
+    int tcin = 0, int tcout = 0) {
+    slab_reduce_body<1>(partial, out, nsplit, n, slabs_per_group, tcin, tcout);
+}
 static __global__ __launch_bounds__(64 * TMF_RED_LANES) void tmf_slab_reduce4_kernel(
     const float* __restrict__ partial, float* __restrict__ out, int nsplit, long n, int slabs_per_group,
     int tcin = 0, int tcout = 0) {
-    typedef float f4 __attribute__((ext_vector_type(4)));
-    __shared__ double red[TMF_RED_LANES][64][4];
+    slab_reduce_body<4>(partial, out, nsplit, n, slabs_per_group, tcin, tcout);
+}
+
+struct SlabItem {
+    const float* partial;
+    float* out;
+    long n;
+    int nsplit, tcin, tcout;
+    int groups;
+    int v4;
+    int first;
+};
+struct SlabTable {
+    SlabItem item[TMF_SLAB_MULTI_MAX];
+    int count, blocks;
+};
+static_assert(sizeof(SlabTable) <= 3584, "SlabTable travels in the kernel arguments (4 KiB)");
+
+template <int V>
+static __device__ __forceinline__ void slab_multi_body(const SlabItem& q, int block, double* red_raw, float* stage_raw) {
+    double (*red)[64][V] = reinterpret_cast<double (*)[64][V]>(red_raw);
+    float (*stage)[64][V] = reinterpret_cast<float (*)[64][V]>(stage_raw);
     const int tx = threadIdx.x & 63, ty = threadIdx.x >> 6;
-    const long e = ((long)blockIdx.x * 64 + tx) * 4;
-    const int g = blockIdx.y;
-    const int s0 = g * slabs_per_group;
-    int s1 = s0 + slabs_per_group;
-    if (s1 > nsplit) s1 = nsplit;
-    double a[4] = {0.0, 0.0, 0.0, 0.0};
-    if (e < n) {
-        int s = s0 + ty;
-        for (; s + 3 * TMF_RED_LANES < s1; s += 4 * TMF_RED_LANES) {
-            const f4 v0 = *reinterpret_cast<const f4*>(partial + (size_t)s * n + e);
-            const f4 v1 = *reinterpret_cast<const f4*>(partial + (size_t)(s + TMF_RED_LANES) * n + e);
-            const f4 v2 = *reinterpret_cast<const f4*>(partial + (size_t)(s + 2 * TMF_RED_LANES) * n + e);
-            const f4 v3 = *reinterpret_cast<const f4*>(partial + (size_t)(s + 3 * TMF_RED_LANES) * n + e);
-#pragma unroll
-            for (int c = 0; c < 4; ++c) a[c] += ((double)v0[c] + (double)v1[c]) + ((double)v2[c] + (double)v3[c]);
+    const float* __restrict__ partial = q.partial;
+    const long n = q.n;
+    const long e = ((long)block * 64 + tx) * V;
+    const bool live = e < n;
+    const int nsplit = q.nsplit, G = q.groups;
+    auto slab = [&](int s) { return *reinterpret_cast<const slab_vec<V>*>(partial + (size_t)s * n + e); };
+    double a[V];
+    if (G == 1) {
+        slab_group_sum<V>(a, red, 0, nsplit, live, tx, ty, slab);
+    } else {
+        const int spg = (nsplit + G - 1) / G;
+        for (int g = 0; g < G; ++g) {
+            const int s0 = g * spg;
+            int s1 = s0 + spg;
+            if (s1 > nsplit) s1 = nsplit;
+            slab_group_sum<V>(a, red, s0, s1, live, tx, ty, slab);
+            if (ty == 0 && live) {
+#pragma unroll
+                for (int c = 0; c < V; ++c) stage[g][tx][c] = (float)a[c];
+            }
+            __syncthreads();
         }
-        for (; s < s1; s += TMF_RED_LANES) {
-            const f4 v = *reinterpret_cast<const f4*>(partial + (size_t)s * n + e);
-#pragma unroll
-            for (int c = 0; c < 4; ++c) a[c] += (double)v[c];
-        }
-    }
-#pragma unroll
-    for (int c = 0; c < 4; ++c) red[ty][tx][c] = a[c];
-    __syncthreads();
-    if (ty == 0 && e < n) {
-#pragma unroll
-        for (int k = 1; k < TMF_RED_LANES; ++k)
-#pragma unroll
-            for (int c = 0; c < 4; ++c) a[c] += red[k][tx][c];
-        if (tcin > 0) {
-            const int T = (int)(n / ((long)tcin * tcout));
-#pragma unroll
-            for (int c = 0; c < 4; ++c) {
-                const long ec = e + c;
-                const int co = (int)(ec % tcout), ci = (int)((ec / tcout) % tcin), t = (int)(ec / ((long)tcout * tcin));
-                out[((size_t)co * tcin + ci) * T + t] = (float)a[c];
-            }
-        } else {
-            *reinterpret_cast<f4*>(out + (size_t)g * n + e) = f4{(float)a[0], (float)a[1], (float)a[2], (float)a[3]};
-        }
-    }
+        slab_group_sum<V>(a, red, 0, G, live, tx, ty, [&](int s) {
+            slab_vec<V> v;
+#pragma unroll
+            for (int c = 0; c < V; ++c) v[c] = stage[s][tx][c];
+            return v;
+        });
+    }
+    if (ty == 0 && live) slab_store<V>(a, q.out, n, e, (size_t)e, q.tcin, q.tcout);
+}
+
+static __global__ __launch_bounds__(64 * TMF_RED_LANES) void tmf_slab_reduce_multi_kernel(const SlabTable t) {
+    __shared__ double red_raw[TMF_RED_LANES * 64 * 4];
+    __shared__ float stage_raw[TMF_RED_MAX_GROUPS * 64 * 4];
+    const int b = blockIdx.x;
+    int q = 0;
+    while (q + 1 < t.count && b >= t.item[q + 1].first) ++q;
+    const SlabItem& it = t.item[q];
+    if (it.v4) slab_multi_body<4>(it, b - it.first, red_raw, stage_raw);
+    else       slab_multi_body<1>(it, b - it.first, red_raw, stage_raw);
+}
+
+static inline bool slab_v4(const float* partial, long n, const float* out, const float* scratch) {
+    return n % 4 == 0 && n >= 1024 && ((size_t)partial & 15) == 0 && ((size_t)out & 15) == 0 && ((size_t)scratch & 15) == 0;
 }
 
 int tmf_reduce_slabs(const float* partial, int nsplit, long n, float* scratch, float* out, hipStream_t s, const char* what,
                      int tcin, int tcout) {
     const int G = tmf_reduce_groups(nsplit);
     const dim3 block(64 * TMF_RED_LANES);
-    const bool v4 = n % 4 == 0 && n >= 1024 && ((size_t)partial & 15) == 0 && ((size_t)out & 15) == 0 &&
-                    (G == 1 || ((size_t)scratch & 15) == 0);
+    const bool v4 = slab_v4(partial, n, out, G == 1 ? nullptr : scratch);
     const int gx = v4 ? (int)((n / 4 + 63) / 64) : (int)((n + 63) / 64);
     auto k = v4 ? tmf_slab_reduce4_kernel : tmf_slab_reduce_kernel;
     if (G == 1) {
@@ -106,6 +171,70 @@
     if (rc) return rc;
     hipLaunchKernelGGL(k, dim3(gx, 1), block, 0, s, (const float*)scratch, out, G, n, G, tcin, tcout);
     return tmf_launch_result(what);
+}
+
+static int check_slab_problem(const char* fn, const float* partial, int nsplit, long long n, const float* out, int tcin, int tcout) {
+    TMF_REQUIRE_PTR_FN(fn, partial); TMF_REQUIRE_PTR_FN(fn, out);
+    TMF_REQUIRE(nsplit > 0 && n > 0 && n < (1LL << 31), TMF_E_SHAPE, "%s: nsplit=%d n=%lld", fn, nsplit, n);
+    TMF_REQUIRE(tcin >= 0 && tcout >= 0 && (tcin == 0 || (tcout > 0 && n % ((long long)tcin * tcout) == 0)), TMF_E_SHAPE,
+                "%s: n=%lld is not a tap-major weight gradient of tcin=%d tcout=%d", fn, n, tcin, tcout);
+    return TMF_OK;
+}
+
+extern "C" int tmf_reduce_slabs_groups(int nsplit) { return nsplit > 0 ? tmf_reduce_groups(nsplit) : 0; }
+
+extern "C" int tmf_reduce_slabs_plan(const float* partial, int nsplit, long long n, float* scratch, float* out, int tcin, int tcout,
+                                     void* stream) {
+    TMF_TRY(check_slab_problem("tmf_reduce_slabs_plan", partial, nsplit, n, out, tcin, tcout));
+    if (tmf_reduce_groups(nsplit) > 1) TMF_REQUIRE_PTR(scratch);
+    return tmf_reduce_slabs(partial, nsplit, (long)n, scratch, out, (hipStream_t)stream, "tmf_reduce_slabs_plan", tcin, tcout);
+}
+
+int tmf_reduce_slabs_multi(const TmfSlabProblem* table, int nproblems, hipStream_t stream) {
+    TMF_REQUIRE(nproblems >= 0, TMF_E_ARG, "tmf_reduce_slabs_multi: nproblems=%d", nproblems);
+    if (nproblems == 0) return TMF_OK;
+    TMF_REQUIRE_PTR(table);
+    for (int i = 0; i < nproblems; ++i) {
+        const TmfSlabProblem& p = table[i];
+        TMF_TRY(check_slab_problem("tmf_reduce_slabs_multi", p.partial, p.nsplit, p.n, p.out, p.tcin, p.tcout));
+        TMF_REQUIRE(tmf_reduce_groups(p.nsplit) <= TMF_RED_MAX_GROUPS, TMF_E_SHAPE, "tmf_reduce_slabs_multi: nsplit=%d", p.nsplit);
+    }
+    int order[TMF_SLAB_MULTI_MAX];
+    for (int base = 0; base < nproblems; base += TMF_SLAB_MULTI_MAX) {
+        SlabTable t;
+        t.count = std::min(nproblems - base, (int)TMF_SLAB_MULTI_MAX);
+        for (int i = 0; i < t.count; ++i) order[i] = base + i;
+        std::stable_sort(order, order + t.count, [&](int a, int b) { return table[a].nsplit > table[b].nsplit; });
+        long blocks = 0;
+        for (int i = 0; i < t.count; ++i) {
+            const TmfSlabProblem& p = table[order[i]];
+            SlabItem& it = t.item[i];
+            it.partial = p.partial; it.out = p.out; it.n = p.n;
+            it.nsplit = p.nsplit; it.tcin = p.tcin; it.tcout = p.tcout;
+            it.groups = tmf_reduce_groups(p.nsplit);
+            it.v4 = slab_v4(p.partial, it.n, p.out, nullptr) ? 1 : 0;
+            it.first = (int)blocks;
+            blocks += it.v4 ? (it.n / 4 + 63) / 64 : (it.n + 63) / 64;
+        }
+        TMF_REQUIRE(blocks < (1L << 31), TMF_E_SHAPE, "tmf_reduce_slabs_multi: %ld workgroups", blocks);
+        t.blocks = (int)blocks;
+        hipLaunchKernelGGL(tmf_slab_reduce_multi_kernel, dim3((unsigned)blocks), dim3(64 * TMF_RED_LANES), 0, stream, t);
+        TMF_TRY(tmf_launch_result("tmf_reduce_slabs_multi"));
+    }
+    return TMF_OK;
+}
+
+extern "C" int tmf_reduce_slabs_multi_ptrs(int nproblems, const float* const* partial, float* const* out, const long long* n,
+                                           const int* nsplit, const int* tcin, const int* tcout, void* stream) {
+    TMF_REQUIRE(nproblems >= 0 && nproblems <= 4096, TMF_E_ARG, "tmf_reduce_slabs_multi_ptrs: nproblems=%d (0 .. 4096)", nproblems);
+    if (nproblems == 0) return TMF_OK;
+    TMF_REQUIRE_PTR(partial); TMF_REQUIRE_PTR(out); TMF_REQUIRE_PTR(n); TMF_REQUIRE_PTR(nsplit); TMF_REQUIRE_PTR(tcin); TMF_REQUIRE_PTR(tcout);
+    TmfSlabProblem* table = (TmfSlabProblem*)malloc(sizeof(TmfSlabProblem) * nproblems);
+    TMF_REQUIRE(table != nullptr, TMF_E_ARG, "tmf_reduce_slabs_multi_ptrs: out of memory");
+    for (int i = 0; i < nproblems; ++i) table[i] = TmfSlabProblem{partial[i], out[i], (long)n[i], nsplit[i], tcin[i], tcout[i]};
+    const int rc = tmf_reduce_slabs_multi(table, nproblems, (hipStream_t)stream);
+    free(table);
+    return rc;
 }
 
 extern "C" int tmf_colsum_finalize(const float* partial, int nblk, int ncol, float* out, void* stream) {
diff --git a/transmf_ad_amd/csrc/snet_path.hip b/transmf_ad_amd/csrc/snet_path.hip
--- a/transmf_ad_amd/csrc/snet_path.hip
+++ b/transmf_ad_amd/csrc/snet_path.hip
@@ -15,6 +15,8 @@
     size_t off_zsel, off_arg;
     size_t x_bytes, z_bytes, out_bytes;
     int cpad;
+    bool defer;
+    size_t off_wgws, wgws_bytes;
 };
 
 struct Plan {
@@ -23,6 +25,7 @@
     size_t off_c1gram = 0, c1gram_bytes = 0;
     size_t saved_bytes;
     size_t off_bpart, off_coef, off_dz, off_gA, off_gB, off_ws, scratch_bytes, ws_bytes;
+    size_t scratch_multi_bytes;
     size_t off_dgws, dgws_bytes;
 };
 
@@ -108,17 +111,23 @@
 }
 
 int launch_wgrad(const tmf_snet_desc& d, const LayerPlan& L, const void* x, const void* dz, float* dw, void* ws, size_t ws_bytes,
-                 void* stream) {
+                 void* stream, TmfSlabProblem* defer) {
     switch (L.wgr) {
     case TMF_CONV_BF16:
         return tmf_conv3d_wgrad_bf16_t(x, dz, dw, ws, ws_bytes, d.B, L.D, L.H, L.W, L.cin, L.cout, L.x16 ? 1 : 0, TMF_DW_REFERENCE, stream);
     case TMF_CONV_WINO:
-        return tmf_conv3d_wgrad_wino((const float*)x, (const float*)dz, dw, ws, ws_bytes, d.B, L.D, L.H, L.W, L.cin, L.cout,
-                                     TMF_DW_REFERENCE, stream);
+        return tmf_conv3d_wgrad_wino_slabs((const float*)x, (const float*)dz, dw, ws, ws_bytes, d.B, L.D, L.H, L.W, L.cin, L.cout,
+                                           TMF_DW_REFERENCE, stream, defer);
     default:
-        return tmf_conv3d_wgrad((const float*)x, (const float*)dz, dw, ws, ws_bytes, d.B, L.D, L.H, L.W, L.cin, L.cout, L.k,
-                                TMF_DW_REFERENCE, stream);
-    }
+        return tmf_conv3d_wgrad_slabs((const float*)x, (const float*)dz, dw, ws, ws_bytes, d.B, L.D, L.H, L.W, L.cin, L.cout, L.k,
+                                      TMF_DW_REFERENCE, stream, defer);
+    }
+}
+
+bool wgrad_defers(const LayerPlan& L, int l, size_t c1gram_bytes) {
+    if (tmf_opt(TMF_OPT_SLAB_PER_LAYER)) return false;
+    if (l == 0) return c1gram_bytes == 0;
+    return L.wgr == TMF_CONV_DIRECT || (L.wgr == TMF_CONV_WINO && tmf_opt(TMF_OPT_WINO_P));
 }
 
 Plan make_plan(const tmf_snet_desc& d, bool train = true) {
@@ -183,6 +192,8 @@
         if (pb2 > bpart_max) bpart_max = pb2;
         if (L.z_bytes > z_max) z_max = L.z_bytes;
         if (l > 0 && L.x_bytes > x_max) x_max = L.x_bytes;
+        L.defer = train && wgrad_defers(L, l, p.c1gram_bytes);
+        L.wgws_bytes = ws;
         if (ws > ws_max) ws_max = ws;
     }
     p.off_part = off; off += up256(part_max);
@@ -199,6 +210,12 @@
     p.dgws_bytes = tmf_c1_bwd_dgrad_workspace_bytes(d.B, p.L[0].D, p.L[0].H, p.L[0].W, p.L[0].cout);
     p.off_dgws = so; so += up256(p.dgws_bytes);
     p.scratch_bytes = so;
+    for (int l = 0; l < NL; ++l) {
+        LayerPlan& L = p.L[l];
+        L.off_wgws = so;
+        if (L.defer) so += up256(L.wgws_bytes);
+    }
+    p.scratch_multi_bytes = so;
     return p;
 }
 
@@ -238,6 +255,12 @@
     if (check_desc("tmf_snet_bwd_scratch_bytes", d) != TMF_OK) return 0;
     const TmfAlgoScope algo_scope(d->flags);
     return make_plan(*d).scratch_bytes;
+}
+
+extern "C" size_t tmf_snet_bwd_scratch_bytes_multi(const tmf_snet_desc* d) {
+    if (check_desc("tmf_snet_bwd_scratch_bytes_multi", d) != TMF_OK) return 0;
+    const TmfAlgoScope algo_scope(d->flags);
+    return make_plan(*d).scratch_multi_bytes;
 }
 
 extern "C" int tmf_snet_train_fwd(const tmf_snet_desc* d, const float* vol, const tmf_snet_params* prm,
@@ -423,10 +446,21 @@
             bias_filled = true;
         }
     }
+    const bool multi = scratch_bytes >= p.scratch_multi_bytes;
+    TmfSlabProblem slabs[NL];
+    int nslabs = 0;
+    auto reduce_slabs = [&]() {
+        const int n = nslabs;
+        nslabs = 0;
+        return tmf_reduce_slabs_multi(slabs, n, s);
+    };
     const void* go = dout;
     for (int l = NL - 1; l >= 0; --l) {
         const LayerPlan& L = p.L[l];
         const Vecs v = vecs_of(base, L);
+        TmfSlabProblem* defer = multi && L.defer ? &slabs[nslabs] : nullptr;
+        void* wgws = defer ? sc + L.off_wgws : ws;
+        const size_t wgws_bytes = defer ? L.wgws_bytes : p.ws_bytes;
         const void* x = l == 0 ? (const void*)vol : (const void*)(base + p.L[l - 1].off_out);
         const void* wf = base + L.off_wf;
         const void* wd = base + L.off_wd;
@@ -468,12 +502,10 @@
                                                d->B, L.D, L.H, L.W, L.cout, d->slope[l], stream));
             TMF_TRY(tmf_bn_bwd_finalize(part, nblk, L.cout, count, g->dgamma[l], g->dbeta[l], coef, stream));
             if (g->dweight[l] != nullptr) {
-                if (b16) TMF_TRY(tmf_c1_bwd_wgrad_bf16(vol, (const float*)wf, v.scale, v.shift, v.mean, v.invstd, coef, go,
-                                                       g->dweight[l], ws, p.ws_bytes, d->B, L.D, L.H, L.W, L.cout, d->slope[l],
-                                                       L.o16 ? 1 : 0, TMF_DW_REFERENCE, stream));
-                else     TMF_TRY(tmf_c1_bwd_wgrad(vol, (const float*)wf, v.scale, v.shift, v.mean, v.invstd, coef,
-                                                  (const float*)go, g->dweight[l], ws, p.ws_bytes, d->B, L.D, L.H, L.W, L.cout,
-                                                  d->slope[l], TMF_DW_REFERENCE, stream));
+                TMF_TRY(tmf_c1_bwd_wgrad_slabs(b16, b16 && L.o16, vol, (const float*)wf, v.scale, v.shift, v.mean, v.invstd, coef, go,
+                                               g->dweight[l], wgws, wgws_bytes, d->B, L.D, L.H, L.W, L.cout, d->slope[l],
+                                               TMF_DW_REFERENCE, stream, defer));
+                if (defer != nullptr) ++nslabs;
             }
             if (dvol != nullptr)
                 TMF_TRY(tmf_c1_bwd_dgrad(vol, (const float*)wf, v.scale, v.shift, v.mean, v.invstd, coef, (const float*)go, dvol,
@@ -490,15 +522,19 @@
         TMF_TRY(tmf_bn_act_pool_bwd_apply_t(z, go, v.scale, v.shift, v.mean, v.invstd, coef, dz, d->B, L.D, L.H, L.W, L.cout,
                                             L.pool, d->slope[l], io, stream));
         void* dx = sc + ((l & 1) ? p.off_gA : p.off_gB);
-        if (g->dweight[l] != nullptr) TMF_TRY(launch_wgrad(*d, L, x, dz, g->dweight[l], ws, p.ws_bytes, stream));
+        if (g->dweight[l] != nullptr) {
+            TMF_TRY(launch_wgrad(*d, L, x, dz, g->dweight[l], wgws, wgws_bytes, stream, defer));
+            if (defer != nullptr && defer->partial != nullptr) ++nslabs;
+        }
         TMF_TRY(launch_dgrad(*d, L, dz, wd, dx, stream));
         go = dx;
         if (l == TMF_SNET_DEEP_FROM && g->deep_event != nullptr) {
+            TMF_TRY(reduce_slabs());
             hipError_t e = hipEventRecord((hipEvent_t)g->deep_event, s);
             TMF_REQUIRE(e == hipSuccess, (int)e, "tmf_snet_train_bwd: hipEventRecord failed: %s", hipGetErrorString(e));
         }
     }
-    return TMF_OK;
+    return reduce_slabs();
 }
 
 extern "C" int tmf_snet_train_bwd(const tmf_snet_desc* d, const float* vol, const void* saved, size_t saved_bytes,
diff --git a/transmf_ad_amd/csrc/tmf_common.h b/transmf_ad_amd/csrc/tmf_common.h
--- a/transmf_ad_amd/csrc/tmf_common.h
+++ b/transmf_ad_amd/csrc/tmf_common.h
@@ -83,6 +83,7 @@
 int tmf_conv3d_stat_blocks_mode(int B, int D, int H, int W, int cin, int cout, int ksize, int rt_min);
 enum TmfOpt {
     TMF_OPT_CONV_WINO, TMF_OPT_WINO_P, TMF_OPT_WINO_X, TMF_OPT_C1_GRAM, TMF_OPT_C1_SPLIT, TMF_OPT_POOL_RECOMPUTE,
+    TMF_OPT_SLAB_PER_LAYER,
     TMF_OPT_WINO_CUS, TMF_OPT_CONV_RT, TMF_OPT_CONV_WAVES, TMF_OPT_BF16_V2, TMF_OPT_BF16_DMA, TMF_OPT_WGRAD_TR, TMF_OPT_DEBUG,
     TMF_OPT_WINO_EVEN, TMF_OPT_WINOX_SWAP, TMF_OPT_BF_NT2, TMF_OPT_CONV_AUTO, TMF_OPT_C1_BLOCKS, TMF_OPT_C1_FWD_MULT,
     TMF_OPT_COUNT
@@ -192,6 +193,25 @@
 }
 int tmf_reduce_slabs(const float* partial, int nsplit, long n, float* scratch, float* out, hipStream_t s, const char* what,
                      int tcin = 0, int tcout = 0);
+struct TmfSlabProblem {
+    const float* partial;
+    float* out;
+    long n;
+    int nsplit, tcin, tcout;
+};
+TMF_INTERNAL
+int tmf_reduce_slabs_multi(const TmfSlabProblem* table, int nproblems, hipStream_t s);
+TMF_INTERNAL
+int tmf_conv3d_wgrad_slabs(const float* x, const float* dz, float* dw, void* workspace, size_t workspace_bytes, int B, int D, int H,
+                           int W, int cin, int cout, int ksize, int dw_layout, void* stream, TmfSlabProblem* defer);
+TMF_INTERNAL
+int tmf_conv3d_wgrad_wino_slabs(const float* x, const float* dz, float* dw, void* workspace, size_t workspace_bytes, int B, int D,
+                                int H, int W, int cin, int cout, int dw_layout, void* stream, TmfSlabProblem* defer);
+TMF_INTERNAL
+int tmf_c1_bwd_wgrad_slabs(bool bf16, bool pooled_bf16, const float* x, const float* w, const float* scale, const float* shift,
+                           const float* mean, const float* invstd, const float* coef, const void* dpool, float* dw, void* workspace,
+                           size_t workspace_bytes, int B, int D, int H, int W, int C, float slope, int dw_layout, void* stream,
+                           TmfSlabProblem* defer);
 
 #ifdef __HIPCC__
 __host__ __device__ __forceinline__ int xcd_contiguous(int bid, int n) {
diff --git a/transmf_ad_amd/ops.py b/transmf_ad_amd/ops.py
--- a/transmf_ad_amd/ops.py
+++ b/transmf_ad_amd/ops.py
@@ -602,7 +602,7 @@
 def snet_algo_flags(algo=None) -> int:
     f = _lib.query("tmf_snet_algo_flags")
     if algo:
-        bad = set(algo) - {"conv_wino", "wino_p", "wino_x", "c1_gram", "c1_split", "pool_recompute"}
+        bad = set(algo) - {"conv_wino", "wino_p", "wino_x", "c1_gram", "c1_split", "pool_recompute", "slab_multi"}
         if bad:
             raise ValueError(f"unknown algorithm option(s) {sorted(bad)}")
         if "conv_wino" in algo:
@@ -620,6 +620,8 @@
                 raise ValueError("pool_recompute must be 0, 1, 2 or 3")
             c1, bn = _lib.SNET_ALGO_POOL_REC_C1, _lib.SNET_ALGO_POOL_REC_BN
             f = (f & ~(c1 | bn)) | {0: 0, 1: c1 | bn, 2: c1, 3: bn}[int(algo["pool_recompute"])]
+        if "slab_multi" in algo:
+            f = (f & ~_lib.SNET_ALGO_SLAB_PER_LAYER) if algo["slab_multi"] else (f | _lib.SNET_ALGO_SLAB_PER_LAYER)
     return f
 
 
@@ -691,7 +693,9 @@
         prep = ctx.bwd if ctx.bwd is not None else SNetTrain._prepare_backward(ctx.shapes, ctx.needs_input_grad, vol.device)
         ctx.bwd = None
         flat, grads, g, ev, o_deep = prep
-        nscr = _lib.query("tmf_snet_bwd_scratch_bytes", C.byref(desc))
+        publish = bool(_FLAT_GRAD_CONSUMERS) and all(ctx.needs_input_grad[3 + i] for i, gr in enumerate(grads) if gr is not None)
+        g.deep_event = ev.cuda_event if publish else None
+        nscr = _lib.query("tmf_snet_bwd_scratch_bytes_multi", C.byref(desc))
         scratch = torch.empty(nscr, device=vol.device, dtype=torch.uint8)
         dvol = None
         if ctx.needs_input_grad[0]:
@@ -704,7 +708,7 @@
         out = [dvol, None, None]
         for i, gr in enumerate(grads):
             out.append(gr if (gr is not None and ctx.needs_input_grad[3 + i]) else None)
-        if _FLAT_GRAD_CONSUMERS and all(ctx.needs_input_grad[3 + i] for i, gr in enumerate(grads) if gr is not None):
+        if publish:
             _publish_flat_grads(flat, ctx.param_ptrs, grads, [(o_deep, flat.numel(), ev, "now"), (0, o_deep, None, "end")])
         return tuple(out)
 
```

After: 1096, median of 4. 1.03x the previous value.
